# Algomorph/LevelSetFusion-Python

Hardware: AMD Instinct MI355X
Metric: voxel-warp-updates/sec (higher is better)
Workload: dtype f32

## Files before the change

include/lsf_hip.h:

```cpp
#ifndef LSF_HIP_H
#define LSF_HIP_H

#include <stdint.h>

#ifdef __cplusplus
extern "C" {
#endif

#define LSF_ABI_VERSION 4
#define LSF_MAX_KERNEL_TAPS 31

#define LSF_ERR_BAD_ARGUMENT (-1)
#define LSF_ERR_BAD_DIMS (-2)
#define LSF_ERR_KERNEL_TOO_LONG (-3)
#define LSF_ERR_RCCL_UNAVAILABLE (-4)
#define LSF_ERR_RCCL_FAILED (-5)
#define LSF_ERR_NOT_RESIDENT (-6)

typedef struct lsf_grid {
    int32_t dims;
    int32_t nz, ny, nx;
    int32_t z_begin, z_end;
    int32_t z_global_offset;
    int32_t y_global_offset;
// ... 146 lines not shown
int lsf_state_prepare(const float *live, const float *canonical, float *state_a, float *state_b,
                      const lsf_grid *grid, int32_t *scratch, int64_t *counts_out, void *stream);
int lsf_state_pack(const float *live, const float *warp_planar, float *state_a, float *state_b,
                   const lsf_grid *grid, void *stream);
int lsf_state_unpack(const float *state, float *live_out, float *warp_planar_out, float *warp_interleaved_out,
                     const lsf_grid *grid, void *stream);
int64_t lsf_state_finalize_scratch_elements(const lsf_grid *grid);
int lsf_state_finalize(const float *state, const float *canonical, float *live_out, float *warp_planar_out,
                       float *warp_interleaved_out, const lsf_grid *grid, float lower_threshold,
                       double *statistics16, double *scratch, void *stream);
int lsf_planar_finalize(const float *live, const float *warp_planar, const float *canonical, float *live_out,
                        float *warp_interleaved_out, const lsf_grid *grid, float lower_threshold,
                        double *statistics16, double *scratch, void *stream);

int lsf_state_finalize_listed(const float *state, const float *canonical, float *live_out, float *warp_interleaved_out,
                              const lsf_grid *grid, const int32_t *const *band_lists, const int64_t *band_counts,
                              int32_t n_lists, int64_t opposite_count, int64_t first_opposite, float lower_threshold,
                              double *statistics16, double *scratch, const int32_t *skip_flag,
                              const lsf_iteration_record *guard_records, int32_t guard_count, float guard_limit,
                              void *stream);
int lsf_slavcheva_state_iteration(const float *state_in, const float *canonical, float *state_out,
                                  const lsf_grid *grid, const lsf_slavcheva_params *params, const lsf_gate *gate,
                                  lsf_iteration_record *record, const int32_t *band_list, int64_t band_count,
                                  int32_t band_subset, void *stream);

int lsf_cumulative_warp_compose(const float *state, const float *psi_in, float *psi_out, const lsf_grid *grid,
                                const lsf_gate *gate, const int32_t *band_list, int64_t band_count, void *stream);

typedef struct lsf_band_box {
    int32_t origin;
    int32_t reserved;
    uint64_t mask;
} lsf_band_box;
int64_t lsf_band_boxes_scratch_elements(const lsf_grid *grid);
int lsf_band_boxes_count(const lsf_grid *grid, int32_t subset, const int32_t *prepare_scratch, int32_t *box_scratch,
                         int64_t *count_out, void *stream);
int lsf_band_boxes_fill(const lsf_grid *grid, int32_t subset, const int32_t *prepare_scratch, const int32_t *box_scratch,
                        lsf_band_box *boxes, void *stream);
int lsf_band_boxes_canonical(const float *canonical, const lsf_grid *grid, const lsf_band_box *boxes, int64_t box_count,
                             float *canonical_boxed, void *stream);
int lsf_slavcheva_state_iteration_boxes(const float *state_in, const float *canonical_boxed, float *state_out,
                                        const lsf_grid *grid, const lsf_slavcheva_params *params, const lsf_gate *gate,
                                        lsf_iteration_record *record, const lsf_band_box *boxes, int64_t box_count,
                                        void *stream);

typedef struct lsf_run_loop {
    int32_t min_iterations;
    int32_t max_iterations;
    float lower_threshold, upper_threshold;
    int32_t check_interval;
    int32_t reserved;
} lsf_run_loop;
typedef struct lsf_state_run {
    const float *live;
    const float *canonical;
    float *state[2];
    int32_t *prepare_scratch;
    int64_t *totals_device;
    int64_t *totals_host;
    lsf_grid grid;
    int32_t sparse_reach;
    int32_t second_state_late;
    int32_t *box_scratch;
    int32_t box_all;
    int32_t reserved;
} lsf_state_run;
typedef struct lsf_state_run_result {
    float *max_value;
    int64_t *argmax;
    double *energies3;
    uint8_t *executed;
    int32_t final_state;
    int32_t n_lists;
    int32_t reach_exceeded;
    int32_t compact_faces;
} lsf_state_run_result;
int lsf_state_run_begin(const lsf_state_run *run, void *stream);
int lsf_state_run_finish(const lsf_state_run *run, const lsf_slavcheva_params *params, int32_t *list_interior,
                         int32_t *list_boundary, lsf_band_box *boxes, float *box_canonical, lsf_iteration_record *records,
                         int32_t iterations, const lsf_run_loop *loop ,
                         float *live_out,
                         float lower_threshold, double *statistics16, double *finalize_scratch, int64_t *words_device,
                         int64_t *words_host, lsf_state_run_result *result, void *stream);

int lsf_sobolev_run_finish(const lsf_state_run *run, const lsf_slavcheva_params *params, const double *taps_host,
                           int32_t n_taps, int32_t *list_interior, int32_t *list_boundary, int32_t *list_all,
                           lsf_band_box *boxes, float *g4_a, float *g4_b, lsf_iteration_record *records, int32_t iterations,
                           const lsf_run_loop *loop, float *live_out, float lower_threshold, double *statistics16,
                           double *finalize_scratch, int64_t *words_device, int64_t *words_host,
                           lsf_state_run_result *result, void *stream);

int lsf_sobolev_state_gradient(const float *state, const float *canonical, float *g_raw4, const lsf_grid *grid,
                               const lsf_slavcheva_params *params, const lsf_gate *gate, lsf_iteration_record *record,
                               const int32_t *band_list, int64_t band_count, void *stream);
int lsf_sobolev_state_gradient_x(const float *state, const float *canonical, float *out4, const lsf_grid *grid,
                                 const lsf_slavcheva_params *params, const double *taps_host, int32_t n_taps,
                                 const lsf_gate *gate, lsf_iteration_record *record, const int32_t *band_list,
                                 int64_t band_count, int32_t out_bricks, void *stream);
int lsf_zero_listed4(float *field4, const lsf_grid *grid, const int32_t *band_list, int64_t band_count, int32_t bricks,
                     void *stream);
int lsf_convolve_axis_listed4(const float *in4, float *out4, const float *zero_mask_source4, const lsf_grid *grid,
                              int32_t axis, const double *taps_host, int32_t n_taps, const lsf_gate *gate,
                              const int32_t *band_list, int64_t band_count, void *stream);
int lsf_band_list_strip_major(const int32_t *band_list, int64_t band_count, const lsf_grid *grid, int32_t strips,
                              int32_t *out, int32_t *scratch, void *stream);
int lsf_sobolev_state_update(const float *in4, const float *zero_mask_source4, const float *state_in, float *state_out,
                             float *g_out4, const lsf_grid *grid, const lsf_slavcheva_params *params, int32_t axis,
                             const double *taps_host, int32_t n_taps, const lsf_gate *gate,
                             lsf_iteration_record *record, const int32_t *band_list, int64_t band_count,
                             int32_t first_list, void *stream);
int lsf_sobolev_state_update_boxes(const float *in4, const float *state_in, float *state_out, float *g_out4,
                                   const lsf_grid *grid, const lsf_slavcheva_params *params, const double *taps_host,
                                   int32_t n_taps, const lsf_gate *gate, lsf_iteration_record *record,
                                   const lsf_band_box *boxes, int64_t box_count, void *stream);

#define LSF_SLAB_LAUNCH 0
#define LSF_SLAB_EXCHANGE 1
#define LSF_SLAB_EXCHANGE_DEFERRED 2
#define LSF_SLAB_RESUME 3
typedef struct lsf_slab_comm lsf_slab_comm;
typedef struct lsf_slab_layout {
    int32_t nz, ny, nx;
    int32_t z_begin, z_end;
    int32_t halo;
    int32_t lo_rank, hi_rank;
} lsf_slab_layout;
typedef struct lsf_slab_part {
    lsf_grid grid;
    const int32_t *band_list[2];
    int64_t band_count[2];
    int32_t band_subset[2];
    int32_t n_lists;
    int32_t reserved;
} lsf_slab_part;
typedef struct lsf_slab_faces {
    const int32_t *send_list[2], *recv_list[2];
    float *send_msg[2], *recv_msg[2];
    int64_t send_count[2], recv_count[2];
} lsf_slab_faces;
int lsf_merge_sorted_runs(const int32_t *const *a, const int64_t *n_a, const int32_t *const *b, const int64_t *n_b,
                          int32_t *const *out, int32_t pairs, void *stream);
int lsf_slab_unique_id(const char *rccl_library_path, uint8_t *id_out128);
int lsf_slab_comm_create(const char *rccl_library_path, const uint8_t *id128, int32_t rank, int32_t world,
                         lsf_slab_comm **out);
int lsf_slab_comm_destroy(lsf_slab_comm *comm);
int lsf_slab_comm_info(lsf_slab_comm *comm, int32_t *rank_out, int32_t *nranks_out);
int lsf_slab_face_counts_begin(lsf_slab_comm *comm, const int64_t *counts4);
int lsf_slab_face_counts_end(lsf_slab_comm *comm, int64_t *table);
int lsf_slab_state_iteration(lsf_slab_comm *comm, const float *state_in, const float *canonical, float *state_out,
                             const lsf_slab_layout *layout, const lsf_slab_part *boundary_parts, int32_t n_boundary,
                             const lsf_slab_part *interior_parts, int32_t n_interior,
                             const lsf_slavcheva_params *params, const lsf_gate *gate, lsf_iteration_record *record,
                             int32_t exchange ,
                             const lsf_slab_faces *faces , void *stream);

#define LSF_SLAB_MAX_CUTS 72
typedef struct lsf_slab_run {
    lsf_state_run base;
    lsf_slab_layout layout;
    int32_t exchange_interval;
    int32_t n_cuts;
    int32_t cut_slices[LSF_SLAB_MAX_CUTS];
    int64_t cut_entries[2][LSF_SLAB_MAX_CUTS];
    int64_t out_index_entries;
    int64_t out_face_entries;
} lsf_slab_run;
// ... 483 lines not shown
```

levelsetfusion-python_amd/_lib.py:

```python
import ctypes
import os

import torch

from ._build import LIB_PATH

c_float_p = ctypes.c_void_p

MAX_KERNEL_TAPS = 31
ABI_VERSION = 4
HEADER_ABI_HASH = "88f9a6300475259d"

ERRORS = {-1: "LSF_ERR_BAD_ARGUMENT", -2: "LSF_ERR_BAD_DIMS", -3: "LSF_ERR_KERNEL_TOO_LONG",
          -4: "LSF_ERR_RCCL_UNAVAILABLE", -5: "LSF_ERR_RCCL_FAILED", -6: "LSF_ERR_NOT_RESIDENT"}

SMOOTHING_TIKHONOV, SMOOTHING_KILLING = 0, 1
DATA_BASIC, DATA_THRESHOLDED_FDM = 0, 2
ENERGY_NONE, ENERGY_DIRECT, ENERGY_VECTORIZED = 0, 1, 2
GATE_HIERARCHICAL, GATE_SLAVCHEVA, GATE_OPEN = 0, 1, 2


class Grid(ctypes.Structure):
    _fields_ = [("dims", ctypes.c_int32), ("nz", ctypes.c_int32), ("ny", ctypes.c_int32), ("nx", ctypes.c_int32),
                ("z_begin", ctypes.c_int32), ("z_end", ctypes.c_int32), ("z_global_offset", ctypes.c_int32),
                ("y_global_offset", ctypes.c_int32), ("energy_z_begin", ctypes.c_int32), ("energy_z_end", ctypes.c_int32),
                ("ny_global", ctypes.c_int32), ("energy_y_begin", ctypes.c_int32), ("energy_y_end", ctypes.c_int32)]


BAND_ALL, BAND_INTERIOR, BAND_BOUNDARY = 0, 1, 2
RECORD_SLOTS = 8


class RecordSlot(ctypes.Structure):
    _fields_ = [("max_packed", ctypes.c_uint64), ("data_energy", ctypes.c_double),
                ("smoothing_energy", ctypes.c_double), ("level_set_energy", ctypes.c_double),
                ("pad", ctypes.c_uint64 * 508)]


class IterationRecord(ctypes.Structure):
    _fields_ = [("slot", RecordSlot * RECORD_SLOTS)]


RECORD_BYTES = ctypes.sizeof(IterationRecord)
SLOT_WORDS = ctypes.sizeof(RecordSlot) // 8


class Gate(ctypes.Structure):
    _fields_ = [("prev_record", ctypes.c_void_p), ("mode", ctypes.c_int32), ("a", ctypes.c_float),
                ("b", ctypes.c_float)]


SLAB_LAUNCH, SLAB_EXCHANGE, SLAB_EXCHANGE_DEFERRED, SLAB_RESUME = 0, 1, 2, 3


class SlabLayoutC(ctypes.Structure):
    _fields_ = [("nz", ctypes.c_int32), ("ny", ctypes.c_int32), ("nx", ctypes.c_int32), ("z_begin", ctypes.c_int32),
                ("z_end", ctypes.c_int32), ("halo", ctypes.c_int32), ("lo_rank", ctypes.c_int32),
                ("hi_rank", ctypes.c_int32)]


class SlabPart(ctypes.Structure):
    _fields_ = [("grid", Grid), ("band_list", ctypes.c_void_p * 2), ("band_count", ctypes.c_int64 * 2),
                ("band_subset", ctypes.c_int32 * 2), ("n_lists", ctypes.c_int32), ("reserved", ctypes.c_int32)]


class SlabFaces(ctypes.Structure):
    _fields_ = [("send_list", ctypes.c_void_p * 2), ("recv_list", ctypes.c_void_p * 2),
                ("send_msg", ctypes.c_void_p * 2), ("recv_msg", ctypes.c_void_p * 2),
                ("send_count", ctypes.c_int64 * 2), ("recv_count", ctypes.c_int64 * 2)]


class BandBox(ctypes.Structure):
    _fields_ = [("origin", ctypes.c_int32), ("reserved", ctypes.c_int32), ("mask", ctypes.c_uint64)]


class StateRun(ctypes.Structure):
    _fields_ = [("live", ctypes.c_void_p), ("canonical", ctypes.c_void_p), ("state", ctypes.c_void_p * 2),
                ("prepare_scratch", ctypes.c_void_p), ("totals_device", ctypes.c_void_p),
                ("totals_host", ctypes.c_void_p), ("grid", Grid), ("sparse_reach", ctypes.c_int32),
                ("second_state_late", ctypes.c_int32), ("box_scratch", ctypes.c_void_p), ("box_all", ctypes.c_int32),
                ("reserved", ctypes.c_int32)]


TERM_DATA_BASIC, TERM_DATA_THRESHOLDED_FDM, TERM_TIKHONOV, TERM_TIKHONOV_LOCAL, TERM_KILLING, TERM_LEVEL_SET = range(6)
TERM_COPY_IF_ZERO, TERM_IGNORE_IF_ZERO, TERM_INTERLEAVED = 1, 2, 4
SELECT_ALL, SELECT_BAND, SELECT_LIST = 0, 1, 2
TERM_ENERGY_LOCAL, TERM_ENERGY_NP_GRADIENT = 0, 1


class TermParams(ctypes.Structure):
    _fields_ = [("isomorphic_enforcement_factor_f64", ctypes.c_double), ("isomorphic_enforcement_factor", ctypes.c_float),
                ("epsilon", ctypes.c_float), ("scaling_factor", ctypes.c_float), ("term", ctypes.c_int32),
                ("flags", ctypes.c_int32), ("reserved", ctypes.c_int32)]

# ... 218 lines not shown

class PointSdfParams(ctypes.Structure):
    _fields_ = [(n, ctypes.c_double) for n in ("fx", "fy", "cx", "cy", "depth_unit_ratio", "max_distance", "voxel_size",
                                               "offset_x", "offset_y", "offset_z", "narrow_band_width_voxels",
                                               "scale")] + \
               [(n, ctypes.c_int32) for n in ("depth", "height", "width", "image_height", "image_width", "depth_dtype",
                                              "levels")] + \
               [("iterations", ctypes.c_int32 * ICP_MAX_LEVELS), ("strides", ctypes.c_int32 * ICP_MAX_LEVELS),
                ("loss", ctypes.c_int32)]


POINT_SDF_COLOUR_SCRATCH_BYTES = 2 * ICP_MAX_BLOCKS * 35 * 8
_POINT_SDF_COLOUR_FIELDS = [(n, ctypes.c_double) for n in ("photometric_weight", "max_intensity_difference",
                                                           "intensity_scale")]


class PointSdfPhotometricParams(ctypes.Structure):
    _fields_ = PointSdfParams._fields_ + _POINT_SDF_COLOUR_FIELDS


class PointSdfPyramidParams(ctypes.Structure):
    _fields_ = PointSdfPhotometricParams._fields_ + [("pyramid_levels", ctypes.c_int32), ("reserved", ctypes.c_int32)]


class EwaParams(ctypes.Structure):
    _fields_ = [("covariance_camera_space", ctypes.c_double * 9), ("squared_radius_threshold", ctypes.c_double),
                ("intrinsic_matrix", ctypes.c_float * 9), ("method", ctypes.c_int32)]


_P = ctypes.POINTER
_vp, _i32, _i64, _f32 = ctypes.c_void_p, ctypes.c_int32, ctypes.c_int64, ctypes.c_float

PROTOTYPES = {
    "lsf_abi_version": (ctypes.c_int, []),
    "lsf_target_arch": (ctypes.c_char_p, []),
    "lsf_build_id": (ctypes.c_char_p, []),
    "lsf_abi_hash": (ctypes.c_char_p, []),
    "lsf_deinterleave": (ctypes.c_int, [_vp, _vp, _i64, _i32, _vp]),
    "lsf_interleave": (ctypes.c_int, [_vp, _vp, _i64, _i32, _vp]),
    "lsf_halo_copy": (ctypes.c_int, [_vp, _vp, _vp, _vp, _P(Grid), _i32, _i32, _i32, _i32, _i32, _vp]),
    "lsf_warp_field": (ctypes.c_int, [_vp, _vp, _vp, _P(Grid), _f32, _vp]),
    "lsf_warp_field_advanced": (ctypes.c_int, [_vp, _vp, _vp, _vp, _vp, _P(Grid), _i32, _vp]),
    "lsf_pack_live_gradient": (ctypes.c_int, [_vp, _vp, _P(Grid), _vp]),
    "lsf_restrict_mean": (ctypes.c_int, [_vp, _vp, _P(Grid), _i32, _vp]),
    "lsf_prolong_repeat": (ctypes.c_int, [_vp, _vp, _P(Grid), _vp]),
    "lsf_upsample2x_linear": (ctypes.c_int, [_vp, _vp, _P(Grid), _i32, _vp]),
    "lsf_downsample2x_linear": (ctypes.c_int, [_vp, _vp, _P(Grid), _i32, _vp]),
    "lsf_convolve_axis": (ctypes.c_int, [_vp, _vp, _vp, _P(Grid), _i32, _i32, _P(ctypes.c_double), _i32,
                                         _P(Gate), _vp]),
    "lsf_convolve_xy": (ctypes.c_int, [_vp, _vp, _P(Grid), _i32, _P(ctypes.c_double), _i32, _P(Gate), _vp]),
    "lsf_convolve_axis_update": (ctypes.c_int, [_vp, _vp, _vp, ctypes.c_float, _P(Grid), _i32, _i32, _P(ctypes.c_double),
                                                _i32, _P(Gate), _vp]),
    "lsf_convolve_xyz": (ctypes.c_int, [_vp, _vp, _vp, _f32, _P(Grid), _i32, _P(ctypes.c_double), _i32, _P(Gate),
                                        _vp]),
    "lsf_hier_iteration": (ctypes.c_int, [_vp, _vp, _vp, _vp, _vp, _P(Grid), _P(HierParams), _P(Gate), _vp, _vp]),
    "lsf_hier_update": (ctypes.c_int, [_vp, _vp, _P(Grid), _f32, _P(Gate), _vp, _vp]),
    "lsf_hier_level_run_2d": (ctypes.c_int, [_vp, _vp, _vp, _vp, _vp, _vp, _P(Grid), _P(HierParams), _P(ctypes.c_double),
                                            _i32, _vp, _i32, _i32, ctypes.c_float, _vp]),
    "lsf_slavcheva_gradient": (ctypes.c_int, [_vp, _vp, _vp, _vp, _P(Grid), _P(SlavchevaParams), _P(Gate), _vp,
                                              _vp, _i64, _vp]),
    "lsf_convolve_axis_listed": (ctypes.c_int, [_vp, _vp, _vp, _P(Grid), _i32, _i32, _P(ctypes.c_double), _i32,
                                                _P(Gate), _vp, _i64, _vp]),
    "lsf_state_prepare_scratch_elements": (ctypes.c_int64, [_P(Grid)]),
    "lsf_band_list_fill_prepared": (ctypes.c_int, [_P(Grid), _i32, _vp, _vp, _vp]),
    "lsf_state_prepare": (ctypes.c_int, [_vp, _vp, _vp, _vp, _P(Grid), _vp, _vp, _vp]),
    "lsf_state_pack": (ctypes.c_int, [_vp, _vp, _vp, _vp, _P(Grid), _vp]),
    "lsf_state_pack_needed": (ctypes.c_int, [_vp, _vp, _vp, _P(Grid), _vp, _i32, _i32, _vp]),
    "lsf_state_unpack": (ctypes.c_int, [_vp, _vp, _vp, _vp, _P(Grid), _vp]),
    "lsf_state_finalize_scratch_elements": (ctypes.c_int64, [_P(Grid)]),
    "lsf_state_finalize": (ctypes.c_int, [_vp, _vp, _vp, _vp, _vp, _P(Grid), _f32, _vp, _vp, _vp]),
    "lsf_planar_finalize": (ctypes.c_int, [_vp, _vp, _vp, _vp, _vp, _P(Grid), _f32, _vp, _vp, _vp]),
    "lsf_state_finalize_listed": (ctypes.c_int, [_vp, _vp, _vp, _vp, _P(Grid), _P(ctypes.c_void_p), _P(_i64), _i32,
                                                 _i64, _i64, _f32, _vp, _vp, _vp, _vp, _i32, _f32, _vp]),
    "lsf_slavcheva_state_iteration": (ctypes.c_int, [_vp, _vp, _vp, _P(Grid), _P(SlavchevaParams), _P(Gate), _vp,
                                                     _vp, _i64, _i32, _vp]),
    "lsf_cumulative_warp_compose": (ctypes.c_int, [_vp, _vp, _vp, _P(Grid), _P(Gate), _vp, _i64, _vp]),
    "lsf_band_boxes_scratch_elements": (ctypes.c_int64, [_P(Grid)]),
    "lsf_band_boxes_count": (ctypes.c_int, [_P(Grid), ctypes.c_int32, _vp, _vp, _vp, _vp]),
    "lsf_band_boxes_fill": (ctypes.c_int, [_P(Grid), ctypes.c_int32, _vp, _vp, _vp, _vp]),
    "lsf_band_boxes_canonical": (ctypes.c_int, [_vp, _P(Grid), _vp, ctypes.c_int64, _vp, _vp]),
    "lsf_slavcheva_state_iteration_boxes": (ctypes.c_int, [_vp, _vp, _vp, _P(Grid), _P(SlavchevaParams), _P(Gate), _vp, _vp,
                                                           _i64, _vp]),
    "lsf_state_run_begin": (ctypes.c_int, [_P(StateRun), _vp]),
    "lsf_state_run_finish": (ctypes.c_int, [_P(StateRun), _P(SlavchevaParams), _vp, _vp, _vp, _vp, _vp, _i32, _P(RunLoop), _vp,
                                            _f32, _vp, _vp, _vp, _vp, _P(StateRunResult), _vp]),
    "lsf_sobolev_run_finish": (ctypes.c_int, [_P(StateRun), _P(SlavchevaParams), _P(ctypes.c_double), _i32, _vp, _vp, _vp, _vp,
                                              _vp, _vp, _vp, _i32, _P(RunLoop), _vp, _f32, _vp, _vp, _vp, _vp,
                                              _P(StateRunResult), _vp]),
    "lsf_slab_run_begin": (ctypes.c_int, [_P(SlabRun), _vp]),
    "lsf_slab_run_finish": (ctypes.c_int, [_P(SlabRun), _vp, _P(SlavchevaParams), _vp, _vp, _vp, _vp, _vp, _i32, _vp, _vp, _vp,
                                           _P(StateRunResult), _vp]),
    "lsf_band_scratch_elements": (ctypes.c_int64, [_P(Grid)]),
    "lsf_band_count": (ctypes.c_int, [_vp, _vp, _P(Grid), _i32, _vp, _vp, _vp]),
    "lsf_band_list_fill": (ctypes.c_int, [_vp, _vp, _P(Grid), _i32, _vp, _vp, _vp]),
    "lsf_records_decode": (ctypes.c_int, [_vp, _i32, _i32, _i32, _vp, _vp, _vp, _vp]),
    "lsf_merge_sorted_runs": (ctypes.c_int, [_P(_vp), _P(_i64), _P(_vp), _P(_i64), _P(_vp), _i32, _vp]),
    "lsf_slab_unique_id": (ctypes.c_int, [ctypes.c_char_p, _vp]),
    "lsf_slab_comm_create": (ctypes.c_int, [ctypes.c_char_p, _vp, _i32, _i32, _P(_vp)]),
    "lsf_slab_comm_destroy": (ctypes.c_int, [_vp]),
    "lsf_slab_comm_info": (ctypes.c_int, [_vp, _P(_i32), _P(_i32)]),
    "lsf_slab_face_counts_begin": (ctypes.c_int, [_vp, _P(_i64)]),
    "lsf_slab_face_counts_end": (ctypes.c_int, [_vp, _P(_i64)]),
    "lsf_slab_state_iteration": (ctypes.c_int, [_vp, _vp, _vp, _vp, _P(SlabLayoutC), _P(SlabPart), _i32, _P(SlabPart),
                                                _i32, _P(SlavchevaParams), _P(Gate), _vp, _i32, _P(SlabFaces), _vp]),
    "lsf_slavcheva_filter_update_rewarp": (ctypes.c_int, [_vp, _vp, _vp, _vp, _vp, _vp, _P(Grid), _P(SlavchevaParams),
                                                          _i32, _P(ctypes.c_double), _i32, _P(Gate), _vp, _vp, _i64,
                                                          _vp]),
    "lsf_sobolev_state_gradient": (ctypes.c_int, [_vp, _vp, _vp, _P(Grid), _P(SlavchevaParams), _P(Gate), _vp, _vp, _i64,
                                                  _vp]),
    "lsf_band_list_strip_major": (ctypes.c_int, [_vp, _i64, _P(Grid), _i32, _vp, _vp, _vp]),
    "lsf_sobolev_state_gradient_x": (ctypes.c_int, [_vp, _vp, _vp, _P(Grid), _P(SlavchevaParams), _P(ctypes.c_double), _i32,
                                                    _P(Gate), _vp, _vp, _i64, _i32, _vp]),
    "lsf_zero_listed4": (ctypes.c_int, [_vp, _P(Grid), _vp, _i64, _i32, _vp]),
    "lsf_convolve_axis_listed4": (ctypes.c_int, [_vp, _vp, _vp, _P(Grid), _i32, _P(ctypes.c_double), _i32, _P(Gate), _vp,
                                                 _i64, _vp]),
    "lsf_sobolev_state_update": (ctypes.c_int, [_vp, _vp, _vp, _vp, _vp, _P(Grid), _P(SlavchevaParams), _i32,
                                                _P(ctypes.c_double), _i32, _P(Gate), _vp, _vp, _i64, _i32, _vp]),
    "lsf_sobolev_state_update_boxes": (ctypes.c_int, [_vp, _vp, _vp, _vp, _P(Grid), _P(SlavchevaParams),
                                                      _P(ctypes.c_double), _i32, _P(Gate), _vp, _vp, _i64, _vp]),
    "lsf_slavcheva_update_rewarp": (ctypes.c_int, [_vp, _vp, _vp, _vp, _vp, _P(Grid), _P(SlavchevaParams),
                                                   _P(Gate), _vp, _vp, _i64, _vp]),
    "lsf_term_gradient": (ctypes.c_int, [_vp, _vp, _vp, _vp, _vp, _vp, _vp, _vp, _vp, _P(Grid), _P(TermParams), _i32, _i32,
                                         _vp, _i64, _vp]),
    "lsf_warp_statistics": (ctypes.c_int, [_vp, _vp, _vp, _P(Grid), _f32, _vp, _vp]),
    "lsf_tsdf_difference_statistics": (ctypes.c_int, [_vp, _vp, _P(Grid), _vp, _vp]),
    "lsf_tsdf_generate_nearest": (ctypes.c_int, [_vp, _vp, _P(Grid), _P(TsdfParams), _vp]),
    "lsf_tsdf_generate_bilinear": (ctypes.c_int, [_vp, _vp, _P(Grid), _P(TsdfParams), _i32, _vp]),
    "lsf_tsdf_generate_ewa": (ctypes.c_int, [_vp, _vp, _P(Grid), _P(TsdfParams), _P(EwaParams), _vp]),
    "lsf_tsdf_generate_nearest_typed": (ctypes.c_int, [_vp, _i32, _vp, _P(Grid), _P(TsdfParams), _P(ctypes.c_double),
                                                       _P(ctypes.c_double), _vp]),
    "lsf_rigid_gradient": (ctypes.c_int, [_vp, _vp, _P(RigidParams), _vp]),
    "lsf_rigid_run": (ctypes.c_int, [_vp, _vp, _vp, _vp, _vp, _P(RigidParams), _vp]),
    "lsf_rigid3d_gradient": (ctypes.c_int, [_vp, _vp, _vp, _vp, _P(Rigid3dParams), _vp]),
    "lsf_rigid3d_run": (ctypes.c_int, [_vp, _vp, _vp, _vp, _vp, _P(Rigid3dParams), _vp]),
    "lsf_fusion_integrate_volume": (ctypes.c_int, [_vp, _vp, _vp, _vp, _vp, _P(FusionParams), _vp]),
    "lsf_fusion_integrate_depth": (ctypes.c_int, [_vp, _vp, _vp, _vp, _vp, _P(FusionParams), _vp]),
    "lsf_fusion_integrate_depth_weighted": (ctypes.c_int, [_vp, _vp, _vp, _vp, _vp, _vp, _P(FusionWeightedParams),
                                                           _vp]),
    "lsf_fusion_integrate_depth_colour": (ctypes.c_int, [_vp, _vp, _vp, _vp, _vp, _vp, _vp, _vp,
                                                         _P(FusionColourParams), _vp]),
    "lsf_fusion_integrate_depth_warped": (ctypes.c_int, [_vp, _vp, _vp, _vp, _vp, _vp, _vp, _vp, _vp,
                                                         _P(FusionWarpedParams), _vp]),
    "lsf_depth_confidence": (ctypes.c_int, [_vp, _vp, _vp, _P(DepthConfidenceParams), _vp]),
    "lsf_raycast": (ctypes.c_int, [_vp, _vp, _vp, _vp, _vp, _vp, _P(RaycastParams), _vp]),
    "lsf_raycast_colour": (ctypes.c_int, [_vp, _vp, _vp, _vp, _vp, _vp, _vp, _vp, _P(RaycastParams), _vp]),
    "lsf_mesh_count": (ctypes.c_int, [_vp, _vp, _vp, _vp, _vp, _vp, _P(MeshParams), _vp]),
    "lsf_mesh_emit": (ctypes.c_int, [_vp, _vp, _vp, _vp, _vp, _vp, _vp, _vp, _vp, _i64, _i64, _P(MeshParams), _vp]),
    "lsf_mesh_vertex_colours": (ctypes.c_int, [_vp, _vp, _vp, _vp, _vp, _i64, ctypes.c_int32, ctypes.c_int32,
                                               ctypes.c_int32, _P(MeshParams), _vp]),
    "lsf_volume_shift": (ctypes.c_int, [_vp, _vp, _vp, _vp, _vp, _vp, _P(VolumeShiftParams), _vp]),
    "lsf_icp_run": (ctypes.c_int, [_vp, _vp, _vp, _vp, _vp, _vp, _vp, _P(IcpParams), _vp]),
    "lsf_depth_pyramid": (ctypes.c_int, [_vp, _vp, _vp, _P(DepthPyramidParams), _vp]),
    "lsf_icp_run_pyramid": (ctypes.c_int, [_vp, _vp, _vp, _vp, _vp, _vp, _vp, _vp, _P(IcpPyramidParams), _vp]),
    "lsf_icp_run_photometric": (ctypes.c_int, [_vp, _vp, _vp, _vp, _vp, _vp, _vp, _vp, _vp, _vp,
                                               _P(IcpPhotometricParams), _vp]),
    "lsf_intensity_pyramid": (ctypes.c_int, [_vp, _vp, _P(IntensityPyramidParams), _vp]),
    "lsf_icp_run_pyramid_photometric": (ctypes.c_int, [_vp, _vp, _vp, _vp, _vp, _vp, _vp, _vp, _vp, _vp, _vp,
                                                       _P(IcpPyramidPhotometricParams), _vp]),
    "lsf_icp_run_robust": (ctypes.c_int, [_vp, _vp, _vp, _vp, _vp, _vp, _vp, _vp, _vp, _vp, _vp, _P(IcpRobustParams),
                                          _vp]),
    "lsf_icp_run_pyramid_robust": (ctypes.c_int, [_vp, _vp, _vp, _vp, _vp, _vp, _vp, _vp, _vp, _vp, _vp, _vp,
                                                  _P(IcpPyramidRobustParams), _vp]),
    "lsf_point_sdf_run": (ctypes.c_int, [_vp, _vp, _vp, _vp, _vp, _vp, _vp, _vp, _P(PointSdfParams), _vp]),
    "lsf_point_sdf_run_photometric": (ctypes.c_int, [_vp] * 11 + [_P(PointSdfPhotometricParams), _vp]),
    "lsf_point_sdf_run_pyramid": (ctypes.c_int, [_vp] * 11 + [_P(PointSdfPyramidParams), _vp]),
}
# ... 40 lines not shown
```

levelsetfusion-python_amd/csrc/lsf_device.h:

```cpp
#pragma once

#include <hip/hip_runtime.h>
#include <cstdlib>
#include <stdint.h>

#include "../../include/lsf_hip.h"

namespace lsf {

constexpr int kWave = 64;
constexpr int kBlock = 256;
constexpr int kCuBlock = 1024;
constexpr int kMaxBlockWaves = kCuBlock / kWave;

struct FastDiv {
    unsigned d, m, l;
};

__host__ inline FastDiv make_fast_div(unsigned d) {
    FastDiv f;
    f.d = d;
    f.l = 0;
    while ((1ull << f.l) < d) ++f.l;
    f.m = (unsigned)(((1ull << 32) * ((1ull << f.l) - d)) / d + 1ull);
// ... 203 lines not shown
        return x_begin + (g * cus + q) * group + (n - g * group);
    }
};

__device__ inline WaveWalk wave_list_walk(unsigned count, unsigned group) {
    const unsigned units = (count + kWave - 1) / kWave;
    const unsigned nb = gridDim.x, bid = blockIdx.x;
    WaveWalk w;
    w.group = group;
    if (nb % kXcds == 0) {
        const unsigned per_xcd = (units + kXcds - 1) / kXcds, xcd = bid % kXcds;
        w.cus = nb / kXcds;
        w.q = bid / kXcds;
        w.x_begin = xcd * per_xcd;
        w.x_end = w.x_begin + per_xcd < units ? w.x_begin + per_xcd : units;
    } else {
        w.cus = nb;
        w.q = bid;
        w.x_begin = 0u;
        w.x_end = units;
    }
    return w;
}

__host__ inline unsigned cu_list_blocks(unsigned count, unsigned cus) {
    const unsigned units = (count + kWave - 1) / kWave;
    unsigned blocks = (units + kMaxBlockWaves - 1) / kMaxBlockWaves;
    if (blocks < 1) blocks = 1;
    if (blocks > cus) blocks = cus;
    if (blocks > kXcds) blocks -= blocks % kXcds;
    return blocks;
}

template <class F>
__device__ inline void for_each_listed_voxel(const Grid& g, const int* __restrict__ list, unsigned count, F&& f) {
    const bool listed = list != nullptr;
    const Tiling t = make_tiling(g);
    const TileWalk w = tile_walk(t.total, g);
    const int lx = threadIdx.x & (kTileX - 1), ly = threadIdx.x / kTileX;
    unsigned first = w.q, step = w.step, end = w.count;
    if (listed) {
        const unsigned units = (count + kBlock - 1) / kBlock;
        const unsigned nb = gridDim.x, bid = blockIdx.x;
        if (nb % kXcds == 0) {
            const unsigned per_xcd = (units + kXcds - 1) / kXcds, xcd = bid % kXcds;
            first = xcd * per_xcd + bid / kXcds;
            step = nb / kXcds;
            end = (xcd + 1) * per_xcd < units ? (xcd + 1) * per_xcd : units;
        } else {
            first = bid; step = nb; end = units;
        }
    }
    for (unsigned u = first; u < end; u += step) {
        int x, y, z;
        bool inside;
        if (listed) {
            const unsigned k = u * kBlock + threadIdx.x;
            inside = k < count;
            const unsigned i = inside ? (unsigned)list[k] : 0u;
            const unsigned zy = fast_div(i, g.div_nx);
            x = (int)(i - zy * (unsigned)g.nx);
            z = (int)fast_div(zy, g.div_ny);
            y = (int)zy - z * g.ny;
        } else {
            const unsigned tile = tile_of(w, u);
            const unsigned rest = fast_div(tile, g.div_tiles_x);
            const int tx = (int)(tile - rest * (unsigned)t.tiles_x);
            const int tz = (int)fast_div(rest, g.div_tiles_y);
            const int ty = (int)rest - tz * t.tiles_y;
            x = tx * kTileX + lx; y = ty * g.tile_y + ly; z = g.z_begin + tz;
            inside = x < g.nx && y < g.ny;
        }
        if (inside) f(x, y, z);
    }
}

__host__ inline unsigned band_list_blocks(unsigned count, unsigned default_per_xcd = 256u) {
    const unsigned units = (count + kBlock - 1) / kBlock;
    if (units <= kXcds) return units < 1 ? 1 : units;
    const unsigned per_xcd = (units + kXcds - 1) / kXcds;
    const unsigned cap = default_per_xcd;
    const unsigned rounds = (per_xcd + cap - 1) / cap;
    return kXcds * ((per_xcd + rounds - 1) / rounds);
}


__device__ inline void decode_voxel(const Grid& g, unsigned i, int& x, int& y, int& z) {
    if (g.shift_x >= 0) {
        x = (int)(i & ((1u << g.shift_x) - 1u));
        const unsigned zy = i >> g.shift_x;
        y = (int)(zy & ((1u << g.shift_y) - 1u));
        z = (int)(zy >> g.shift_y);
    } else {
        const unsigned zy = fast_div(i, g.div_nx);
        x = (int)(i - zy * (unsigned)g.nx);
        z = (int)fast_div(zy, g.div_ny);
        y = (int)zy - z * g.ny;
    }
}

__device__ inline unsigned linear_index(const Grid& g, int x, int y, int z) {
    return (unsigned)(((long long)(z + g.z_global_offset) * g.ny_global + (y + g.y_global_offset)) * g.nx + x);
}

__device__ inline int vidx(const Grid& g, int x, int y, int z) {
    return (z * g.ny + y) * g.nx + x;
}

__device__ inline bool inside(const Grid& g, int x, int y, int z) {
    return (unsigned)x < (unsigned)g.nx && (unsigned)y < (unsigned)g.ny && (unsigned)z < (unsigned)g.nz;
}

__device__ inline float read_oob(const float* __restrict__ f, const Grid& g, int x, int y, int z, float oob) {
    return inside(g, x, y, z) ? f[vidx(g, x, y, z)] : oob;
}

__device__ inline float read_clamp(const float* __restrict__ f, const Grid& g, int x, int y, int z) {
    x = min(max(x, 0), g.nx - 1);
    y = min(max(y, 0), g.ny - 1);
    z = min(max(z, 0), g.nz - 1);
    return f[vidx(g, x, y, z)];
}

struct AxisTaps {
    int c0, c1;
    bool v0, v1;
    float r, i;
};

__device__ inline AxisTaps axis_taps(float p, int n, int global_offset) {
    AxisTaps t;
    const float f = floorf(p);
    t.r = p - f;
    t.i = 1.0f - t.r;
    const int b = (int)fminf(fmaxf(f - (float)global_offset, -2.0f), (float)n + 1.0f);
    t.v0 = (unsigned)b < (unsigned)n;
    t.v1 = (unsigned)(b + 1) < (unsigned)n;
    t.c0 = min(max(b, 0), n - 1);
    t.c1 = min(max(b + 1, 0), n - 1);
    return t;
}

template <int D>
__device__ inline float sample_linear_taps(const float* __restrict__ f, const Grid& g, const AxisTaps& ax,
                                           const AxisTaps& ay, const AxisTaps& az, float oob) {
    const int row0 = ay.c0 * g.nx, row1 = ay.c1 * g.nx;
    if (D == 2) {
        float v00 = f[row0 + ax.c0], v01 = f[row1 + ax.c0], v10 = f[row0 + ax.c1], v11 = f[row1 + ax.c1];
        v00 = (ax.v0 && ay.v0) ? v00 : oob;
        v01 = (ax.v0 && ay.v1) ? v01 : oob;
        v10 = (ax.v1 && ay.v0) ? v10 : oob;
        v11 = (ax.v1 && ay.v1) ? v11 : oob;
        const float i0 = v00 * ay.i + v01 * ay.r;
        const float i1 = v10 * ay.i + v11 * ay.r;
        return i0 * ax.i + i1 * ax.r;
    } else {
        const int slice = g.nx * g.ny;
        const int s0 = az.c0 * slice, s1 = az.c1 * slice;
        float c[2][2];
#pragma unroll
        for (int ox = 0; ox < 2; ++ox)
#pragma unroll
            for (int oy = 0; oy < 2; ++oy) {
                const int xy = (oy ? row1 : row0) + (ox ? ax.c1 : ax.c0);
                const bool vxy = (ox ? ax.v1 : ax.v0) && (oy ? ay.v1 : ay.v0);
                float a = f[s0 + xy], b = f[s1 + xy];
// ... 26 lines not shown
__device__ inline double shfl_down_f64(double v, int delta) {
    return __longlong_as_double((long long)shfl_down_u64((unsigned long long)__double_as_longlong(v), delta));
}

template <int CTRL>
__device__ inline unsigned long long dpp_u64(unsigned long long v) {
    const unsigned lo = (unsigned)__builtin_amdgcn_update_dpp(0, (int)(unsigned)v, CTRL, 0xf, 0xf, false);
    const unsigned hi = (unsigned)__builtin_amdgcn_update_dpp(0, (int)(unsigned)(v >> 32), CTRL, 0xf, 0xf, false);
    return ((unsigned long long)hi << 32) | lo;
}

__device__ inline unsigned long long broadcast_lane63_u64(unsigned long long v) {
    const unsigned lo = (unsigned)__builtin_amdgcn_readlane((int)(unsigned)v, 63);
    const unsigned hi = (unsigned)__builtin_amdgcn_readlane((int)(unsigned)(v >> 32), 63);
    return ((unsigned long long)hi << 32) | lo;
}

__device__ inline unsigned long long wave_max_u64(unsigned long long v) {
#define LSF_STEP(CTRL)                                   \
    {                                                    \
        const unsigned long long o = dpp_u64<CTRL>(v);   \
        v = o > v ? o : v;                               \
    }
    LSF_STEP(0xb1)
    LSF_STEP(0x4e)
    LSF_STEP(0x124)
    LSF_STEP(0x128)
    LSF_STEP(0x142)
    LSF_STEP(0x143)
#undef LSF_STEP
    return broadcast_lane63_u64(v);
}

__device__ inline double wave_sum_f64(double v) {
#define LSF_STEP(CTRL)                                                                                               \
    v += __longlong_as_double((long long)dpp_u64<CTRL>((unsigned long long)__double_as_longlong(v)));
    LSF_STEP(0xb1)
    LSF_STEP(0x4e)
    LSF_STEP(0x124)
    LSF_STEP(0x128)
    LSF_STEP(0x142)
    LSF_STEP(0x143)
#undef LSF_STEP
    return __longlong_as_double((long long)broadcast_lane63_u64((unsigned long long)__double_as_longlong(v)));
}

__device__ inline unsigned long long pack_max(float length, unsigned linear_index) {
    return ((unsigned long long)__float_as_uint(length) << 32) | (unsigned long long)(~linear_index);
}

__device__ inline float unpack_max_value(unsigned long long packed) { return __uint_as_float((unsigned)(packed >> 32)); }

template <int NS>
__device__ inline void block_reduce_commit(unsigned long long packed, const double (&sums)[NS > 0 ? NS : 1],
                                           unsigned long long* dst_max, double* const (&dst_sum)[NS > 0 ? NS : 1]) {
    __shared__ unsigned long long s_max[kMaxBlockWaves];
    __shared__ double s_sum[(NS > 0 ? NS : 1)][kMaxBlockWaves];
    const int lane = threadIdx.x & (kWave - 1), wave = threadIdx.x / kWave;
    const int n_waves = blockDim.x / kWave;
    unsigned long long m = wave_max_u64(packed);
    double s[NS > 0 ? NS : 1];
#pragma unroll
    for (int i = 0; i < NS; ++i) s[i] = wave_sum_f64(sums[i]);
    if (lane == 0) {
        s_max[wave] = m;
#pragma unroll
        for (int i = 0; i < NS; ++i) s_sum[i][wave] = s[i];
    }
    __syncthreads();
    if (wave == 0) {
        const unsigned long long mm = wave_max_u64(lane < n_waves ? s_max[lane] : 0ull);
        double t[NS > 0 ? NS : 1];
#pragma unroll
        for (int i = 0; i < NS; ++i) t[i] = wave_sum_f64(lane < n_waves ? s_sum[i][lane] : 0.0);
        if (lane == 0) {
            if (dst_max && mm != 0ull) atomicMax(dst_max, mm);
#pragma unroll
            for (int i = 0; i < NS; ++i)
                if (dst_sum[i] && t[i] != 0.0) atomicAdd(dst_sum[i], t[i]);
        }
    }
}

template <int NT>
struct TapsN {
    double k[NT];
};

template <bool FMA>
__device__ inline double mac(double acc, double k, double v) {
    return FMA ? __builtin_fma(k, v, acc) : acc + k * v;
}

static inline bool taps_are_float32(const double* taps, int n) {
    for (int j = 0; j < n; ++j)
        if (!((double)(float)taps[j] == taps[j])) return false;
    return true;
}

template <int D>
__device__ inline float vec_length(const float (&v)[3]) {
    float s = v[0] * v[0] + v[1] * v[1];
    if (D == 3) s = s + v[2] * v[2];
    return sqrtf(s);
}

__device__ inline float second_difference_f64(float am, float a0, float ap) {
    return (float)__builtin_fma(-2.0, (double)a0, (double)ap + (double)am);
}

__device__ inline bool gate_closed(const lsf_gate& gate) {
    if (!gate.prev_record || gate.mode == LSF_GATE_OPEN) return false;
    unsigned long long p = 0ull;
#pragma unroll
    for (int k = 0; k < LSF_RECORD_SLOTS; ++k) {
        const unsigned long long q = gate.prev_record->slot[k].max_packed;
        p = q > p ? q : p;
    }
    if (p == 0ull) return true;
    float m = unpack_max_value(p);
    if (gate.mode == LSF_GATE_HIERARCHICAL) return m < gate.a;
    return !(gate.a < m && m < gate.b);
}

__device__ inline lsf_record_slot* record_slot(lsf_iteration_record* r) {
    return &r->slot[blockIdx.x % LSF_RECORD_SLOTS];
}

__device__ inline unsigned long long* record_max(lsf_iteration_record* r) {
    return reinterpret_cast<unsigned long long*>(&record_slot(r)->max_packed);
}

__host__ inline lsf_gate gate_or_open(const lsf_gate* gate) {
    return gate ? *gate : lsf_gate{nullptr, 0, 0.0f, 0.0f};
}

inline bool overlaps(const void* a, size_t na, const void* b, size_t nb) {
    if (!a || !b || !na || !nb) return false;
    const uintptr_t x = (uintptr_t)a, y = (uintptr_t)b;
    return x < y + nb && y < x + na;
}

inline hipStream_t as_stream(void* s) { return reinterpret_cast<hipStream_t>(s); }

inline int launch_status() { return (int)hipGetLastError(); }

}
```

levelsetfusion-python_amd/csrc/lsf_slavcheva.hip:

```cpp
#include "lsf_device.h"

using namespace lsf;

#include "lsf_slavcheva_terms.h"

using namespace lsf::slav;

namespace {


template <int D, int SMOOTH, bool LEVELSET, int DATA, int ENERGY>
__device__ inline void voxel_gradient(const float* __restrict__ live, const float* __restrict__ canonical,
                                      const float* __restrict__ warp_prev, const Grid& g, const Params& p, int x,
                                      int y, int z, int i, float (&gv)[3], double (&en)[3]) {
    gv[0] = gv[1] = gv[2] = 0.0f;
    const float l = live[i], cn = canonical[i];
    if (fabsf(l) == 1.0f && fabsf(cn) == 1.0f) return;
    const bool interior = x > 0 && x < g.nx - 1 && y > 0 && y < g.ny - 1 && (D == 2 || (z > 0 && z < g.nz - 1));
    if (g.fast_ok && __all(interior)) {
        const NbhFast<D> n(live, warp_prev, g, x, y, z);
        band_voxel_gradient<D, SMOOTH, LEVELSET, DATA, ENERGY>(n, p, l, cn, gv, en);
    } else {
        const Nbh<D> n(live, warp_prev, g, x, y, z);
        band_voxel_gradient<D, SMOOTH, LEVELSET, DATA, ENERGY>(n, p, l, cn, gv, en);
// ... 300 lines not shown
    if (blockIdx.x >= arrays) {
        reduce_opposite(opposite, n, totals);
        return;
    }
    __shared__ int wave_total[1024 / kWave];
    int* __restrict__ sums = sums_base + (size_t)blockIdx.x * stride;
    const unsigned t = threadIdx.x, lane = t & (kWave - 1), wave = t / kWave;
    int carry = 0;
    for (unsigned base = 0; base < n; base += 4096u) {
        const unsigned i = base + 4u * t;
        int v[4];
#pragma unroll
        for (int k = 0; k < 4; ++k) v[k] = i + k < n ? sums[i + k] : 0;
        const int mine = v[0] + v[1] + v[2] + v[3];
        int inclusive = mine;
#pragma unroll
        for (int d = 1; d < kWave; d <<= 1) {
            const int up = __shfl_up(inclusive, d, kWave);
            if ((int)lane >= d) inclusive += up;
        }
        if (lane == kWave - 1) wave_total[wave] = inclusive;
        __syncthreads();
        int before = 0, tile = 0;
#pragma unroll
        for (int w = 0; w < 1024 / kWave; ++w) {
            const int x = wave_total[w];
            before += w < (int)wave ? x : 0;
            tile += x;
        }
        int run = carry + before + inclusive - mine;
#pragma unroll
        for (int k = 0; k < 4; ++k) {
            if (i + k < n) sums[i + k] = run;
            run += v[k];
        }
        carry += tile;
        __syncthreads();
    }
    if (t == 0) totals[blockIdx.x] = carry;
}

constexpr unsigned kScanTile = 4096u;

__global__ __launch_bounds__(1024) void band_tile_totals_kernel(const int* __restrict__ sums_base, unsigned n,
                                                                unsigned stride, const int* __restrict__ opposite,
                                                                int* __restrict__ tile_out, unsigned tiles) {
    __shared__ int s_sum[1024 / kWave], s_first[1024 / kWave];
    const unsigned tile = blockIdx.x, a = blockIdx.y, t = threadIdx.x;
    const unsigned i = tile * kScanTile + 4u * t;
    int sum = 0, first = 0x7fffffff;
    if (a < 2u) {
        const int* __restrict__ sums = sums_base + (size_t)a * stride;
#pragma unroll
        for (unsigned k = 0; k < 4u; ++k) sum += i + k < n ? sums[i + k] : 0;
    } else {
#pragma unroll
        for (unsigned k = 0; k < 4u; ++k)
            if (i + k < n) {
                sum += opposite[2 * (i + k)];
                first = min(first, opposite[2 * (i + k) + 1]);
            }
    }
    for (int d = kWave / 2; d > 0; d >>= 1) {
        sum += __shfl_down(sum, d, kWave);
        first = min(first, __shfl_down(first, d, kWave));
    }
    if ((t & (kWave - 1)) == 0) {
        s_sum[t / kWave] = sum;
        s_first[t / kWave] = first;
    }
    __syncthreads();
    if (t == 0) {
        for (int k = 1; k < 1024 / kWave; ++k) {
            sum += s_sum[k];
            first = min(first, s_first[k]);
        }
        tile_out[(size_t)a * tiles + tile] = sum;
        if (a == 2u) tile_out[(size_t)3 * tiles + tile] = first;
    }
}

__global__ __launch_bounds__(1024) void band_scan_tiles_kernel(int* __restrict__ sums_base, unsigned n, unsigned stride,
                                                               const int* __restrict__ tile_out, unsigned tiles,
                                                               long long* __restrict__ totals) {
    const unsigned tile = blockIdx.x, a = blockIdx.y, t = threadIdx.x, lane = t & (kWave - 1), wave = t / kWave;
    if (a == 2u) {
        if (tile == 0u && t == 0u) {
            long long sum = 0;
            int first = 0x7fffffff;
            for (unsigned k = 0; k < tiles; ++k) {
                sum += tile_out[(size_t)2 * tiles + k];
                first = min(first, tile_out[(size_t)3 * tiles + k]);
            }
            totals[2] = sum;
            totals[3] = first == 0x7fffffff ? -1 : first;
        }
        return;
    }
    __shared__ int wave_total[1024 / kWave];
    int* __restrict__ sums = sums_base + (size_t)a * stride;
    int carry = 0;
    for (unsigned k = 0; k < tile; ++k) carry += tile_out[(size_t)a * tiles + k];
    const unsigned i = tile * kScanTile + 4u * t;
    int v[4];
#pragma unroll
    for (int k = 0; k < 4; ++k) v[k] = i + k < n ? sums[i + k] : 0;
    const int mine = v[0] + v[1] + v[2] + v[3];
    int inclusive = mine;
#pragma unroll
    for (int d = 1; d < kWave; d <<= 1) {
        const int up = __shfl_up(inclusive, d, kWave);
        if ((int)lane >= d) inclusive += up;
    }
    if (lane == kWave - 1) wave_total[wave] = inclusive;
    __syncthreads();
    int before = 0, whole = 0;
#pragma unroll
    for (int w = 0; w < 1024 / kWave; ++w) {
        const int x = wave_total[w];
        before += w < (int)wave ? x : 0;
        whole += x;
    }
    int run = carry + before + inclusive - mine;
#pragma unroll
    for (int k = 0; k < 4; ++k) {
        if (i + k < n) sums[i + k] = run;
        run += v[k];
    }
    if (tile == tiles - 1u && t == 0u) totals[a] = (long long)carry + whole;
}

typedef float vf4 __attribute__((ext_vector_type(4)));

__global__ __launch_bounds__(kBlock) void state_prepare_kernel(const float* __restrict__ live,
                                                               const float* __restrict__ canonical,
                                                               vf4* __restrict__ a, vf4* __restrict__ b, unsigned n,
                                                               Grid g, int dims, int* __restrict__ sums_interior,
                                                               int* __restrict__ sums_boundary,
                                                               unsigned long long* __restrict__ masks,
                                                               int* __restrict__ opposite, int* __restrict__ nonempty) {
    __shared__ int part[4][16];
    const int t = threadIdx.x, wave = t / kWave, lane = t % kWave;
#pragma unroll
    for (int j = 0; j < 4; ++j) {
        const unsigned v = blockIdx.x * kBandChunk + j * kBlock + t;
        bool in_band = false, interior = false, opposed = false;
        if (v < n) {
            const float l = live[v], cn = canonical[v];
            in_band = !(fabsf(l) == 1.0f && fabsf(cn) == 1.0f);
            opposed = !in_band && l != cn;
            vf4 o;
            o.x = l; o.y = 0.0f; o.z = 0.0f; o.w = 0.0f;
            if (a) a[v] = o;
            if (b) b[v] = o;
            const unsigned zy = fast_div(v, g.div_nx);
            const int x = (int)(v - zy * (unsigned)g.nx);
            const int z = (int)fast_div(zy, g.div_ny);
            const int y = (int)zy - z * g.ny;
            interior = x > 0 && x < g.nx - 1 && y > 0 && y < g.ny - 1 && (dims == 2 || (z > 0 && z < g.nz - 1));
        }
        const unsigned long long mi = __ballot(in_band && interior), mb = __ballot(in_band && !interior);
        const unsigned long long mo = __ballot(opposed);
        if (lane == 0) {
            part[0][j * 4 + wave] = __popcll(mi);
            part[1][j * 4 + wave] = __popcll(mb);
            part[2][j * 4 + wave] = __popcll(mo);
            part[3][j * 4 + wave] = mo ? (int)(blockIdx.x * kBandChunk + j * kBlock + wave * kWave) + __ffsll((long long)mo) - 1
                                       : 0x7fffffff;
            masks[((size_t)blockIdx.x * 16 + j * 4 + wave) * 2 + 0] = mi;
            masks[((size_t)blockIdx.x * 16 + j * 4 + wave) * 2 + 1] = mb;
// ... 31 lines not shown
    return ((unsigned long long)hi << 32) | lo;
}

__global__ __launch_bounds__(kBlock) void state_prepare4_kernel(const vf4* __restrict__ live4,
                                                                const vf4* __restrict__ canonical4,
                                                                vf4* __restrict__ a, vf4* __restrict__ b, unsigned n,
                                                                unsigned chunks, Grid g, int dims,
                                                                int* __restrict__ sums_interior,
                                                                int* __restrict__ sums_boundary,
                                                                unsigned long long* __restrict__ masks,
                                                                int* __restrict__ opposite, int* __restrict__ nonempty) {
    __shared__ int part[kPrepareChunksPerBlock][4][16];
    const int t = threadIdx.x, wave = t / kWave, lane = t % kWave;
    const unsigned chunk0 = blockIdx.x * kPrepareChunksPerBlock;
    vf4 l[kPrepareChunksPerBlock], c[kPrepareChunksPerBlock];
#pragma unroll
    for (int k = 0; k < kPrepareChunksPerBlock; ++k) {
        const unsigned v = (chunk0 + k) * kBandChunk + 4u * t;
        const vf4 one = {1.0f, 1.0f, 1.0f, 1.0f};
        l[k] = v < n ? live4[v / 4] : one;
        c[k] = v < n ? canonical4[v / 4] : one;
    }
#pragma unroll
    for (int k = 0; k < kPrepareChunksPerBlock; ++k) {
        const unsigned chunk = chunk0 + k, v = chunk * kBandChunk + 4u * t;
        unsigned ni = 0u, nb = 0u, no = 0u;
        if (v < n) {
            const unsigned zy = fast_div(v, g.div_nx);
            const int x0 = (int)(v - zy * (unsigned)g.nx);
            const int z = (int)fast_div(zy, g.div_ny);
            const int y = (int)zy - z * g.ny;
            const bool row_inside = y > 0 && y < g.ny - 1 && (dims == 2 || (z > 0 && z < g.nz - 1));
            const float lv[4] = {l[k].x, l[k].y, l[k].z, l[k].w}, cv[4] = {c[k].x, c[k].y, c[k].z, c[k].w};
#pragma unroll
            for (int j = 0; j < 4; ++j) {
                const bool in_band = !(fabsf(lv[j]) == 1.0f && fabsf(cv[j]) == 1.0f);
                const bool interior = row_inside && x0 + j > 0 && x0 + j < g.nx - 1;
                ni |= (in_band && interior ? 1u : 0u) << j;
                nb |= (in_band && !interior ? 1u : 0u) << j;
                no |= (!in_band && lv[j] != cv[j] ? 1u : 0u) << j;
                vf4 o;
                o.x = lv[j]; o.y = 0.0f; o.z = 0.0f; o.w = 0.0f;
                if (a) a[v + j] = o;
                if (b) b[v + j] = o;
            }
        }
        const unsigned long long mi = row16_or(ni, lane), mb = row16_or(nb, lane), mo = row16_or(no, lane);
        if ((lane & 15) == 0 && chunk < chunks) {
            const int word = wave * 4 + lane / 16;
            part[k][0][word] = __popcll(mi);
            part[k][1][word] = __popcll(mb);
            part[k][2][word] = __popcll(mo);
            part[k][3][word] = mo ? (int)(chunk * kBandChunk + word * kWave) + __ffsll((long long)mo) - 1 : 0x7fffffff;
            masks[((size_t)chunk * 16 + word) * 2 + 0] = mi;
            masks[((size_t)chunk * 16 + word) * 2 + 1] = mb;
        }
    }
    __syncthreads();
    if (t < 4 * kPrepareChunksPerBlock) {
        const int k = t / 4, what = t % 4;
        const unsigned chunk = chunk0 + k;
        if (chunk < chunks) {
            if (what < 2) {
                int sum = 0;
                for (int w = 0; w < 16; ++w) sum += part[k][what][w];
                (what == 0 ? sums_interior : sums_boundary)[chunk] = sum;
            } else if (what == 2) {
                int sum = 0, first = 0x7fffffff;
                for (int w = 0; w < 16; ++w) {
                    sum += part[k][2][w];
                    first = min(first, part[k][3][w]);
                }
                opposite[2 * chunk] = sum;
                opposite[2 * chunk + 1] = first;
            } else {
                int any = 0;
                for (int w = 0; w < 16; ++w) any |= part[k][0][w] | part[k][1][w];
                nonempty[chunk] = any != 0;
            }
        }
    }
}

__global__ __launch_bounds__(kBlock) void chunk_needed_kernel(unsigned chunks, long long row, long long slice, int dims,
                                                              int reach, const int* __restrict__ nonempty,
                                                              int* __restrict__ needed) {
    const unsigned c = blockIdx.x * (kBlock / kWave) + threadIdx.x / kWave;
    if (c >= chunks) return;
    const int lane = threadIdx.x % kWave;
    const long long c0 = (long long)c * kBandChunk;
    const int span = 2 * reach + 1, zs = dims == 3 ? span : 1;
    bool hit = false;
    for (int k = lane; k < zs * span; k += kWave) {
        const int dy = k % span - reach, dz = dims == 3 ? k / span - reach : 0;
        const long long lo = c0 + dz * slice + dy * row - reach, hi = c0 + (long long)kBandChunk - 1 + dz * slice + dy * row + reach;
        long long first = lo >= 0 ? lo / kBandChunk : -((-lo + kBandChunk - 1) / kBandChunk);
        long long last = hi >= 0 ? hi / kBandChunk : -((-hi + kBandChunk - 1) / kBandChunk);
        first = first < 0 ? 0 : first;
        last = last >= (long long)chunks ? (long long)chunks - 1 : last;
        for (long long cand = first; cand <= last; ++cand) hit |= nonempty[cand] != 0;
    }
    const bool any = __any(hit);
    if (lane == 0) needed[c] = any ? 1 : 0;
}

constexpr int kPackChunks = 1;
__global__ __launch_bounds__(kBlock) void state_pack_needed_kernel(const float* __restrict__ live, vf4* __restrict__ a,
                                                                   vf4* __restrict__ b, unsigned n, unsigned chunks,
                                                                   const int* __restrict__ needed, int want) {
    const int t = threadIdx.x;
    int verdict[kPackChunks];
#pragma unroll
    for (int k = 0; k < kPackChunks; ++k) {
        const unsigned c = blockIdx.x * kPackChunks + k;
        verdict[k] = c < chunks ? needed[c] : -1;
    }
#pragma unroll
    for (int k = 0; k < kPackChunks; ++k) {
        if (verdict[k] != want) continue;
        const unsigned c = blockIdx.x * kPackChunks + k;
#pragma unroll
        for (int j = 0; j < 4; ++j) {
            const unsigned v = c * kBandChunk + j * kBlock + t;
            if (v < n) {
                vf4 o;
                o.x = live[v]; o.y = 0.0f; o.z = 0.0f; o.w = 0.0f;
                if (a) a[v] = o;
                if (b) b[v] = o;
            }
        }
    }
}



__global__ __launch_bounds__(kBlock) void band_fill_from_masks_kernel(const unsigned long long* __restrict__ masks,
                                                                      const int* __restrict__ block_sums, int which,
                                                                      int* __restrict__ list, unsigned chunks) {
    const int lane = threadIdx.x % kWave;
    const unsigned chunk = blockIdx.x * (kBlock / kWave) + threadIdx.x / kWave;
    if (chunk >= chunks) return;
    const unsigned long long mine = lane < 16 ? masks[((size_t)chunk * 16 + lane) * 2 + which] : 0ull;
    if (__ballot(mine != 0ull) == 0ull) return;
    int at = block_sums[chunk];
#pragma unroll
    for (int w = 0; w < 16; ++w) {
        const unsigned lo = (unsigned)__shfl((int)(unsigned)mine, w, kWave);
        const unsigned hi = (unsigned)__shfl((int)(unsigned)(mine >> 32), w, kWave);
        const unsigned long long m = ((unsigned long long)hi << 32) | lo;
        if ((m >> lane) & 1ull)
            list[at + __popcll(m & ((1ull << lane) - 1ull))] = (int)(chunk * kBandChunk + w * kWave + lane);
        at += __popcll(m);
    }
}

}

static inline bool band_subset_ok(int32_t subset) {
    return subset == LSF_BAND_ALL || subset == LSF_BAND_INTERIOR || subset == LSF_BAND_BOUNDARY;
}

extern "C" int lsf_slavcheva_gradient(const float* live, const float* canonical, const float* warp_prev_planar,
                                      float* g_out_planar, const lsf_grid* grid, const lsf_slavcheva_params* params,
                                      const lsf_gate* gate, lsf_iteration_record* record, const int32_t* band_list,
                                      int64_t band_count, void* stream) {
    if (int e = check_grid(grid)) return e;
    if (!live || !canonical || !warp_prev_planar || !params || !record || !g_out_planar ||
        g_out_planar == warp_prev_planar || (band_list && (band_count < 0 || band_count > 0x7fffffffll)))
        return LSF_ERR_BAD_ARGUMENT;
    Grid g = make_grid(grid);
    Tiling t = make_tiling(g);
    if (t.total == 0) return 0;
    LaunchArgs a{band_list ? band_list_blocks((unsigned)band_count) : launch_blocks(t.total), as_stream(stream), live,
                 canonical, warp_prev_planar, g_out_planar, g, make_params(params), gate_or_open(gate), record, band_list,
                 (unsigned)band_count};
    if (grid->dims == 2) pick_terms<2>(params, a);
    else pick_terms<3>(params, a);
    return launch_status();
}

extern "C" int lsf_slavcheva_update_rewarp(const float* live, const float* canonical, float* g_planar,
                                           float* warp_out_planar, float* live_out, const lsf_grid* grid,
                                           const lsf_slavcheva_params* params, const lsf_gate* gate,
                                           lsf_iteration_record* record, const int32_t* band_list, int64_t band_count,
                                           void* stream) {
    (void)canonical;
    if (int e = check_grid(grid)) return e;
    if (!live || !g_planar || !warp_out_planar || !live_out || live_out == live || !params || !record ||
        (band_list && (band_count < 0 || band_count > 0x7fffffffll)))
        return LSF_ERR_BAD_ARGUMENT;
    Grid g = make_grid(grid);
    Tiling t = make_tiling(g);
    if (t.total == 0) return 0;
    Params p = make_params(params);
    lsf_gate gt = gate_or_open(gate);
    const unsigned blocks = band_list ? band_list_blocks((unsigned)band_count) : launch_blocks(t.total);
    if (grid->dims == 2)
        hipLaunchKernelGGL(slavcheva_update_rewarp_kernel<2>, dim3(blocks), dim3(kBlock), 0, as_stream(stream), live,
// ... 137 lines not shown
        }
    return m;
}

template <bool FILL>
__global__ __launch_bounds__(kBlock) void band_boxes_kernel(const unsigned long long* __restrict__ masks, unsigned n_boxes,
                                                            int nbx, int nby, int nx, int ny, bool all,
                                                            int* __restrict__ group_sums, lsf_band_box* __restrict__ boxes) {
    __shared__ int wave_count[kBlock / kWave];
    const unsigned box = blockIdx.x * kBoxGroup + threadIdx.x;
    const int lane = threadIdx.x % kWave, wave = threadIdx.x / kWave;
    const unsigned long long m = box < n_boxes ? box_mask_of(masks, box, nbx, nby, nx, ny, all) : 0ull;
    const unsigned long long any = __ballot(m != 0ull);
    if (lane == 0) wave_count[wave] = __popcll(any);
    __syncthreads();
    if (!FILL) {
        if (threadIdx.x == 0) {
            int sum = 0;
            for (int k = 0; k < kBlock / kWave; ++k) sum += wave_count[k];
            group_sums[blockIdx.x] = sum;
        }
        return;
    }
    if (m == 0ull) return;
    int at = group_sums[blockIdx.x];
    for (int k = 0; k < wave; ++k) at += wave_count[k];
    at += __popcll(any & ((1ull << lane) - 1ull));
    const int bx = (int)(box % (unsigned)nbx), by = (int)((box / (unsigned)nbx) % (unsigned)nby);
    const int bz = (int)(box / ((unsigned)nbx * (unsigned)nby));
    lsf_band_box b;
    b.origin = ((4 * bz) * ny + 4 * by) * nx + 4 * bx;
    b.reserved = 0;
    b.mask = m;
    boxes[at] = b;
}

inline bool boxes_ok(const lsf_grid* g) {
    return g->dims == 3 && g->nx % 4 == 0 && g->ny % 4 == 0 && g->nz % 4 == 0 && g->z_begin == 0 && g->z_end == g->nz &&
           (long long)g->nx * g->ny * g->nz <= 0x0fffffffll;
}
}

extern "C" int64_t lsf_band_boxes_scratch_elements(const lsf_grid* grid) {
    if (check_grid(grid) || !boxes_ok(grid)) return 0;
    const long long n_boxes = (long long)grid->nx * grid->ny * grid->nz / 64;
    return (n_boxes + kBoxGroup - 1) / kBoxGroup + 1;
}

extern "C" int lsf_band_boxes_count(const lsf_grid* grid, int32_t subset, const int32_t* prepare_scratch,
                                    int32_t* box_scratch, int64_t* count_out, void* stream) {
    if (int e = check_grid(grid)) return e;
    if (!boxes_ok(grid)) return LSF_ERR_BAD_DIMS;
    if (!prepare_scratch || !box_scratch || !count_out || (subset != LSF_BAND_INTERIOR && subset != LSF_BAND_ALL))
        return LSF_ERR_BAD_ARGUMENT;
    unsigned first, n, chunks;
    band_range(grid, first, n, chunks);
    const unsigned n_boxes = n / 64, groups = (n_boxes + kBoxGroup - 1) / kBoxGroup;
    hipStream_t s = as_stream(stream);
    hipLaunchKernelGGL(band_boxes_kernel<false>, dim3(groups), dim3(kBlock), 0, s,
                       prepare_masks(const_cast<int32_t*>(prepare_scratch), chunks), n_boxes, grid->nx / 4, grid->ny / 4,
                       grid->nx, grid->ny, subset == LSF_BAND_ALL, box_scratch, (lsf_band_box*)nullptr);
    hipLaunchKernelGGL(band_scan_kernel, dim3(1), dim3(1024), 0, s, box_scratch, groups, 0u, 1u, (long long*)count_out,
                       (const int*)nullptr);
    return launch_status();
}

extern "C" int lsf_band_boxes_fill(const lsf_grid* grid, int32_t subset, const int32_t* prepare_scratch,
                                   const int32_t* box_scratch, lsf_band_box* boxes, void* stream) {
    if (int e = check_grid(grid)) return e;
    if (!boxes_ok(grid)) return LSF_ERR_BAD_DIMS;
    if (!prepare_scratch || !box_scratch || !boxes || (subset != LSF_BAND_INTERIOR && subset != LSF_BAND_ALL))
        return LSF_ERR_BAD_ARGUMENT;
    unsigned first, n, chunks;
    band_range(grid, first, n, chunks);
    const unsigned n_boxes = n / 64, groups = (n_boxes + kBoxGroup - 1) / kBoxGroup;
    hipLaunchKernelGGL(band_boxes_kernel<true>, dim3(groups), dim3(kBlock), 0, as_stream(stream),
                       prepare_masks(const_cast<int32_t*>(prepare_scratch), chunks), n_boxes, grid->nx / 4, grid->ny / 4,
                       grid->nx, grid->ny, subset == LSF_BAND_ALL, const_cast<int32_t*>(box_scratch), boxes);
    return launch_status();
}

extern "C" int lsf_state_prepare(const float* live, const float* canonical, float* state_a, float* state_b,
                                 const lsf_grid* grid, int32_t* scratch, int64_t* counts_out, void* stream) {
    if (int e = check_grid(grid, true)) return e;
    if (!live || !canonical || (!state_a && state_b) || !scratch || !counts_out) return LSF_ERR_BAD_ARGUMENT;
    if (grid->z_begin != 0 || grid->z_end != grid->nz) return LSF_ERR_BAD_ARGUMENT;
    unsigned first, n, chunks;
    band_range(grid, first, n, chunks);
    hipStream_t s = as_stream(stream);
    int* sums_interior = scratch;
    int* sums_boundary = scratch + (chunks + 1);
    const bool wide = grid->nx % 4 == 0 && ((uintptr_t)live | (uintptr_t)canonical) % 16 == 0;
    if (wide)
        hipLaunchKernelGGL(state_prepare4_kernel, dim3((chunks + kPrepareChunksPerBlock - 1) / kPrepareChunksPerBlock),
                           dim3(kBlock), 0, s, reinterpret_cast<const vf4*>(live), reinterpret_cast<const vf4*>(canonical),
                           reinterpret_cast<vf4*>(state_a), reinterpret_cast<vf4*>(state_b), n, chunks, make_grid(grid),
                           grid->dims, sums_interior, sums_boundary, prepare_masks(scratch, chunks),
                           prepare_opposite(scratch, chunks), prepare_nonempty(scratch, chunks));
    else
        hipLaunchKernelGGL(state_prepare_kernel, dim3(chunks), dim3(kBlock), 0, s, live, canonical,
                           reinterpret_cast<vf4*>(state_a), reinterpret_cast<vf4*>(state_b), n, make_grid(grid), grid->dims,
                           sums_interior, sums_boundary, prepare_masks(scratch, chunks), prepare_opposite(scratch, chunks),
                           prepare_nonempty(scratch, chunks));
    const unsigned tiles = prepare_scan_tiles(chunks) > 0u ? prepare_scan_tiles(chunks) : 1u;
    hipLaunchKernelGGL(band_tile_totals_kernel, dim3(tiles, 3), dim3(1024), 0, s, scratch, chunks, chunks + 1,
                       (const int*)prepare_opposite(scratch, chunks), prepare_tile_totals(scratch, chunks), tiles);
    hipLaunchKernelGGL(band_scan_tiles_kernel, dim3(tiles, 3), dim3(1024), 0, s, scratch, chunks, chunks + 1,
                       (const int*)prepare_tile_totals(scratch, chunks), tiles, (long long*)counts_out);
    return launch_status();
}

extern "C" int lsf_state_pack_needed(const float* live, float* state_a, float* state_b, const lsf_grid* grid,
                                     int32_t* scratch, int32_t reach, int32_t invert, void* stream) {
    if (int e = check_grid(grid, true)) return e;
    if (!live || (!state_a && !state_b) || !scratch || reach < 1 || reach > 8) return LSF_ERR_BAD_ARGUMENT;
    if (grid->z_begin != 0 || grid->z_end != grid->nz) return LSF_ERR_BAD_ARGUMENT;
    unsigned first, n, chunks;
    band_range(grid, first, n, chunks);
    if (!invert)
        hipLaunchKernelGGL(chunk_needed_kernel, dim3((chunks + kBlock / kWave - 1) / (kBlock / kWave)), dim3(kBlock), 0, as_stream(stream),
                           chunks, (long long)grid->nx, (long long)grid->nx * grid->ny, grid->dims, reach,
                           prepare_nonempty(scratch, chunks), prepare_needed(scratch, chunks));
    hipLaunchKernelGGL(state_pack_needed_kernel, dim3((chunks + kPackChunks - 1) / kPackChunks), dim3(kBlock), 0,
                       as_stream(stream), live, reinterpret_cast<vf4*>(state_a), reinterpret_cast<vf4*>(state_b), n, chunks,
                       prepare_needed(scratch, chunks), invert ? 0 : 1);
    return launch_status();
}

extern "C" int lsf_band_list_fill(const float* live, const float* canonical, const lsf_grid* grid, int32_t subset,
                                  const int32_t* scratch, int32_t* list, void* stream) {
    if (int e = check_grid(grid)) return e;
    if (!live || !canonical || !scratch || !list || !band_subset_ok(subset)) return LSF_ERR_BAD_ARGUMENT;
    unsigned first, n, chunks;
    if (!band_range(grid, first, n, chunks)) return 0;
    hipLaunchKernelGGL(band_list_kernel<true>, dim3(chunks), dim3(kBlock), 0, as_stream(stream), live, canonical, first, n,
                       make_grid(grid), grid->dims, subset, const_cast<int32_t*>(scratch), list);
    return launch_status();
}
```

levelsetfusion-python_amd/csrc/lsf_slavcheva_box.hip:

```cpp
#include "lsf_slavcheva_state_taps.h"

using namespace lsf;
using namespace lsf::slav;

namespace {

constexpr int kBoxEdge = 4, kShellEdge = kBoxEdge + 2, kShell = kShellEdge * kShellEdge * kShellEdge;
constexpr int kShellLoads = (kShell + kWave - 1) / kWave;
#ifndef LSF_BOX_WAVES
#define LSF_BOX_WAVES 12
#endif
constexpr int kBoxWaves = LSF_BOX_WAVES, kBoxThreads = kBoxWaves * kWave;
constexpr int kImage = kShellLoads * kWave + kWave / 4;

struct NbhStateLds : TapsBase<3> {
    __device__ inline void load(const vf4* __restrict__ image, int centre) {
#pragma unroll
        for (int dz = -1; dz <= 1; ++dz)
#pragma unroll
            for (int dy = -1; dy <= 1; ++dy)
#pragma unroll
                for (int dx = -1; dx <= 1; ++dx) {
                    if ((dx != 0) + (dy != 0) + (dz != 0) > 2) continue;
                    this->t[dz + 1][dy + 1][dx + 1] = image[centre + (dz * kShellEdge + dy) * kShellEdge + dx];
                }
    }
};

__device__ inline bool rewarp_from_image(const TapsBase<3>& n, const vf4* __restrict__ image, int centre, const Grid& g,
                                         int x, int y, int z, const float (&wv)[3], bool active, Rewarp& rw) {
    const NearFar ax((float)x, wv[0]), ay((float)(y + g.y_global_offset), wv[1]), az((float)(z + g.z_global_offset), wv[2]);
    const unsigned lowest = min(min((unsigned)x, (unsigned)y), (unsigned)z);
    if (!__all(!active || (ax.near && ay.near && az.near && lowest >= 2u))) return false;
    const int ci = centre + (ax.below ? -1 : 1) + (ay.below ? -kShellEdge : kShellEdge) +
                   (az.below ? -kShellEdge * kShellEdge : kShellEdge * kShellEdge);
    rw.corner = image[ci].x;
    auto L = [&](int dz, int dy, int dx) { return n.t[dz + 1][dy + 1][dx + 1].x; };
    auto pick2 = [&](bool b, float m, float p) { return b ? m : p; };
    const float t000 = L(0, 0, 0);
    const float t100 = pick2(az.below, L(-1, 0, 0), L(1, 0, 0));
    const float t010 = pick2(ay.below, L(0, -1, 0), L(0, 1, 0));
    const float t001 = pick2(ax.below, L(0, 0, -1), L(0, 0, 1));
    const float t110 = pick2(az.below, pick2(ay.below, L(-1, -1, 0), L(-1, 1, 0)), pick2(ay.below, L(1, -1, 0), L(1, 1, 0)));
    const float t101 = pick2(az.below, pick2(ax.below, L(-1, 0, -1), L(-1, 0, 1)), pick2(ax.below, L(1, 0, -1), L(1, 0, 1)));
    const float t011 = pick2(ay.below, pick2(ax.below, L(0, -1, -1), L(0, -1, 1)), pick2(ax.below, L(0, 1, -1), L(0, 1, 1)));
    const float c00 = t000 * az.wn + t100 * az.wf;
    const float c10 = t010 * az.wn + t110 * az.wf;
    const float c01 = t001 * az.wn + t101 * az.wf;
    const float iy0 = c00 * ay.wn + c10 * ay.wf;
    rw.P = t011 * az.wn;
    rw.Q = c01 * ay.wn;
    rw.R = iy0 * ax.wn;
    rw.wfz = az.wf;
    rw.wfy = ay.wf;
    rw.wfx = ax.wf;
    rw.lerp = true;
    return true;
}

template <int SMOOTH, bool LEVELSET, int DATA, int ENERGY>
__global__ __launch_bounds__(kBoxThreads) __attribute__((amdgpu_waves_per_eu(kBoxWaves / 4, kBoxWaves / 4)))
void slavcheva_state_box_kernel(const vf4* __restrict__ state_in, const float* __restrict__ canonical_boxed,
                                vf4* __restrict__ state_out, Grid g, Params p, lsf_gate gate, lsf_iteration_record* record,
                                const lsf_band_box* __restrict__ boxes, unsigned box_count) {
    g.y_global_offset = 0;
    g.ny_global = g.ny;
    g.y_cut = 0;
    if (gate_closed(gate)) return;
    extern __shared__ vf4 lds[];
    __shared__ unsigned s_next_unit;
    __shared__ int s_goff[kWave][kShellLoads];
    const unsigned waves = blockDim.x / kWave, wave = threadIdx.x / kWave, lane = threadIdx.x & (kWave - 1);
    vf4* const images = lds + wave * (2 * kImage);
    const int sy = g.nx, sz = g.nx * g.ny;
    const int last_voxel = g.nz * sz - 1;
    if (wave == 0) {
#pragma unroll
        for (int j = 0; j < kShellLoads; ++j) {
            int k = (int)lane + kWave * j;
            k = k < kShell ? k : kShell - 1;
            s_goff[lane][j] = (k / (kShellEdge * kShellEdge)) * sz + ((k / kShellEdge) % kShellEdge) * sy + k % kShellEdge;
        }
    }
    const int lx = lane & 3, ly = (lane >> 2) & 3, lz = lane >> 4;
    const int centre = ((lz + 1) * kShellEdge + ly + 1) * kShellEdge + lx + 1;
    const int voxel_off = lz * sz + ly * sy + lx;

    unsigned long long best = 0ull;
    double en[3] = {0.0, 0.0, 0.0};
    const WaveWalk w = wave_list_walk(box_count * kWave, g.list_group);
    if (threadIdx.x == 0) s_next_unit = 2u * waves;
    __syncthreads();
    auto grab = [&]() {
        unsigned v = 0u;
        if (lane == 0) v = atomicAdd(&s_next_unit, 1u);
        return w.unit((unsigned)__builtin_amdgcn_readfirstlane((int)v));
    };
    auto header = [&](unsigned unit, bool& listed) {
        listed = unit < w.x_end && unit < box_count;
        return boxes[unit < box_count ? unit : box_count - 1u];
    };
    auto stage = [&](int origin, unsigned unit, vf4* image) {
        __builtin_amdgcn_global_load_lds((const __attribute__((address_space(1))) void*)(
                                             canonical_boxed + (size_t)(unit < box_count ? unit : box_count - 1u) * kWave + lane),
                                         (__attribute__((address_space(3))) void*)(image + kShellLoads * kWave), 4, 0, 0);
        const int corner = origin - 1 - sy - sz;
        int goff[kShellLoads];
#pragma unroll
        for (int j = 0; j < kShellLoads; ++j) goff[j] = s_goff[lane][j];
#pragma unroll
        for (int j = 0; j < kShellLoads; ++j) {
            int v = corner + goff[j];
            v = v < 0 ? 0 : (v > last_voxel ? last_voxel : v);
            __builtin_amdgcn_global_load_lds((const __attribute__((address_space(1))) void*)(state_in + v),
                                             (__attribute__((address_space(3))) void*)(image + j * kWave), 16, 0, 0);
        }
    };
    auto new_state = [&](const Deferred& d) {
        float v = d.rw.value();
        float wv[3] = {d.wv[0], d.wv[1], d.wv[2]};
        if (1.0f - fabsf(v) < 1e-6f) {
            v = v > 0.0f ? 1.0f : (v < 0.0f ? -1.0f : v);
            wv[0] = wv[1] = wv[2] = 0.0f;
        }
        vf4 o;
        o.x = v; o.y = wv[0]; o.z = wv[1]; o.w = wv[2];
        return o;
    };
    const __amdgpu_buffer_rsrc_t out_rsrc = __builtin_amdgcn_make_buffer_rsrc(
        state_out, 0, (int)((unsigned)(last_voxel + 1) * 16u), 0x00020000);
    auto store = [&](const vf4& o, int i) {
        const int offset = i < 0 ? (int)0xfffffff0u : i * 16;
        if (g.list_store_nt) __builtin_amdgcn_raw_buffer_store_b128(__builtin_bit_cast(vu4, o), out_rsrc, offset, 0, 2);
        else __builtin_amdgcn_raw_buffer_store_b128(__builtin_bit_cast(vu4, o), out_rsrc, offset, 0, 0);
    };

    unsigned u = box_count ? w.unit(wave) : w.x_end, u1 = w.unit(wave + waves);
    bool in0 = false, in1 = false, in2 = false;
    lsf_band_box b0 = {0, 0, 0ull}, b1 = b0;
    int parity = 0;
    if (u < w.x_end) {
        b0 = header(u, in0);
        b1 = header(u1, in1);
        stage(b0.origin, u, images);
    }
    while (u < w.x_end) {
        asm volatile("s_waitcnt vmcnt(0)" ::: "memory");
        const unsigned u2 = grab();
        const lsf_band_box b2 = header(u2, in2);
        const vf4* image = images + parity * kImage;
        const float cn = reinterpret_cast<const float*>(image + kShellLoads * kWave)[lane];
        stage(b1.origin, u1, images + (parity ^ 1) * kImage);
        __builtin_amdgcn_sched_barrier(0);
        NbhStateLds n;
        n.load(image, centre);
        const unsigned i = (unsigned)(b0.origin + voxel_off);
        const bool listed = in0 && ((b0.mask >> lane) & 1ull);
        int x0, y0, z0;
        decode_voxel(g, (unsigned)b0.origin, x0, y0, z0);
        const int x = x0 + lx, y = y0 + ly, z = z0 + lz;
        Deferred d;
        d.i = listed ? (int)i : -1;
        const float l = n.t[1][1][1].x;
        const bool in_band = listed && !(fabsf(l) == 1.0f && fabsf(cn) == 1.0f);
        float gv[3] = {0.0f, 0.0f, 0.0f};
        double e[3] = {0.0, 0.0, 0.0};
        band_voxel_gradient_taps<SMOOTH, LEVELSET, DATA, ENERGY>(n, p, l, cn, gv, e);
        const bool counted = in_band && z >= g.e_begin && z < g.e_end;
#pragma unroll
        for (int c = 0; c < 3; ++c) {
            d.wv[c] = in_band ? (-gv[c]) * p.rate : 0.0f;
            en[c] += counted ? e[c] : 0.0;
        }
        const float len = vec_length<3>(d.wv);
        const bool moved = !(d.wv[0] == 0.0f && d.wv[1] == 0.0f && d.wv[2] == 0.0f);
        if (!rewarp_from_image(n, image, centre, g, x, y, z, d.wv, listed, d.rw)) {
            d.rw.lerp = false;
            d.rw.R = state_gather<3>(state_in, g, (float)x + d.wv[0], (float)y + d.wv[1], (float)(z + g.z_global_offset) + d.wv[2]);
        }
        if (!moved) {
            d.rw.lerp = false;
            d.rw.R = l;
        }
        const unsigned long long q = listed ? pack_max(len, i + g.index_offset) : 0ull;
        best = q > best ? q : best;
        store(new_state(d), d.i);
        u = u1; u1 = u2;
        b0 = b1; b1 = b2;
        in0 = in1; in1 = in2;
        parity ^= 1;
    }
    asm volatile("s_waitcnt vmcnt(0)" ::: "memory");
    if (blockIdx.x == 0 && threadIdx.x == 0) {
        const unsigned long long q = pack_max(0.0f, linear_index(g, 0, 0, g.z_begin));
        best = q > best ? q : best;
    }
    double* dst[3] = {ENERGY != LSF_ENERGY_NONE ? &record_slot(record)->data_energy : nullptr,
                      ENERGY != LSF_ENERGY_NONE ? &record_slot(record)->smoothing_energy : nullptr,
                      ENERGY != LSF_ENERGY_NONE ? &record_slot(record)->level_set_energy : nullptr};
    block_reduce_commit<3>(best, en, record_max(record), dst);
}

struct BoxLaunch {
    unsigned blocks;
    hipStream_t s;
    const vf4* state_in;
    const float* canonical;
    vf4* state_out;
    Grid g;
    Params p;
    lsf_gate gate;
    lsf_iteration_record* record;
    const lsf_band_box* boxes;
    unsigned box_count;
};

constexpr size_t kBoxLdsBytes = (size_t)kBoxWaves * 2 * kImage * sizeof(vf4);

template <int SMOOTH, bool LEVELSET, int DATA, int ENERGY>
int launch_box(const BoxLaunch& a) {
    auto kernel = slavcheva_state_box_kernel<SMOOTH, LEVELSET, DATA, ENERGY>;
    static bool configured[64] = {false};
    int dev = 0;
    if (hipGetDevice(&dev) != hipSuccess || dev < 0 || dev >= 64) return (int)hipGetLastError();
    if (!configured[dev]) {
        if (hipFuncSetAttribute(reinterpret_cast<const void*>(kernel), hipFuncAttributeMaxDynamicSharedMemorySize,
                                (int)kBoxLdsBytes) != hipSuccess)
            return (int)hipGetLastError();
        configured[dev] = true;
    }
    hipLaunchKernelGGL(kernel, dim3(a.blocks), dim3(kBoxThreads), kBoxLdsBytes, a.s, a.state_in, a.canonical, a.state_out, a.g,
                       a.p, a.gate, a.record, a.boxes, a.box_count);
    return 0;
}

template <int SMOOTH, bool LEVELSET, int DATA>
int pick_box_energy(int energy, const BoxLaunch& a) {
    switch (energy) {
        case LSF_ENERGY_DIRECT: return launch_box<SMOOTH, LEVELSET, DATA, LSF_ENERGY_DIRECT>(a);
        case LSF_ENERGY_VECTORIZED: return launch_box<SMOOTH, LEVELSET, DATA, LSF_ENERGY_VECTORIZED>(a);
        default: return launch_box<SMOOTH, LEVELSET, DATA, LSF_ENERGY_NONE>(a);
    }
}

Params box_params(const lsf_slavcheva_params* q) {
    Params p;
    p.lambda64 = q->isomorphic_enforcement_factor_f64;
    p.rate = q->rate;
    p.w_data = q->data_term_weight;
    p.w_smooth = q->smoothing_term_weight;
    p.w_level_set = q->level_set_term_weight;
    p.lambda32 = q->isomorphic_enforcement_factor;
    p.killing_c1 = q->killing_c1;
    p.zero_gradient_on_snap = q->zero_gradient_on_snap;
    return p;
}

inline unsigned box_compute_units() {
    static int cached[64] = {0};
    int dev = 0;
    if (hipGetDevice(&dev) != hipSuccess || dev < 0 || dev >= 64) return 256u;
    if (!cached[dev]) {
        int n = 0;
        if (hipDeviceGetAttribute(&n, hipDeviceAttributeMultiprocessorCount, dev) != hipSuccess || n <= 0) n = 256;
        cached[dev] = n;
    }
    return (unsigned)cached[dev];
}

}

__global__ __launch_bounds__(kBlock) void box_canonical_kernel(const float* __restrict__ canonical,
                                                               const lsf_band_box* __restrict__ boxes, unsigned box_count,
                                                               int sy, int sz, float* __restrict__ out) {
    const unsigned b = blockIdx.x * (kBlock / kWave) + threadIdx.x / kWave, lane = threadIdx.x & (kWave - 1);
    if (b >= box_count) return;
    const int lx = lane & 3, ly = (lane >> 2) & 3, lz = lane >> 4;
    out[(size_t)b * kWave + lane] = canonical[boxes[b].origin + lz * sz + ly * sy + lx];
}

extern "C" int lsf_band_boxes_canonical(const float* canonical, const lsf_grid* grid, const lsf_band_box* boxes,
                                        int64_t box_count, float* canonical_boxed, void* stream) {
    if (int e = check_grid(grid)) return e;
    if (!canonical || !boxes || !canonical_boxed || box_count < 0 || box_count > 0x3ffffffll) return LSF_ERR_BAD_ARGUMENT;
    if (grid->dims != 3 || grid->nx % kBoxEdge || grid->ny % kBoxEdge || grid->nz % kBoxEdge ||
        (long long)grid->nx * grid->ny * grid->nz > 0x0fffffffll)
        return LSF_ERR_BAD_DIMS;
    if (box_count == 0) return 0;
    hipLaunchKernelGGL(box_canonical_kernel, dim3((unsigned)((box_count + kBlock / kWave - 1) / (kBlock / kWave))), dim3(kBlock),
                       0, as_stream(stream), canonical, boxes, (unsigned)box_count, grid->nx, grid->nx * grid->ny, canonical_boxed);
    return launch_status();
}

extern "C" int lsf_slavcheva_state_iteration_boxes(const float* state_in, const float* canonical_boxed, float* state_out,
                                                   const lsf_grid* grid, const lsf_slavcheva_params* params,
                                                   const lsf_gate* gate, lsf_iteration_record* record,
                                                   const lsf_band_box* boxes, int64_t box_count, void* stream) {
    if (int e = check_grid(grid)) return e;
    if (!state_in || !canonical_boxed || !state_out || state_out == state_in || !params || !record || !boxes || box_count < 0 ||
        box_count > 0x3ffffffll)
        return LSF_ERR_BAD_ARGUMENT;
    if (grid->dims != 3 || grid->nx % kBoxEdge || grid->ny % kBoxEdge || grid->nz % kBoxEdge ||
        (long long)grid->nx * grid->ny * grid->nz > 0x0fffffffll)
        return LSF_ERR_BAD_DIMS;
    if (box_count == 0) return 0;
    Grid g = make_grid(grid, 4);
    g.list_store_nt = box_count * 64ll * 32ll > 200ll * 1000 * 1000 * 5 / 4;
    BoxLaunch a{cu_list_blocks((unsigned)box_count * kWave, box_compute_units()), as_stream(stream),
                reinterpret_cast<const vf4*>(state_in), canonical_boxed, reinterpret_cast<vf4*>(state_out), g, box_params(params),
                gate_or_open(gate), record, boxes, (unsigned)box_count};
    const bool killing = params->smoothing_method == LSF_SMOOTHING_KILLING;
    const bool ls = params->level_set_enabled != 0;
    const bool fdm = params->data_method == LSF_DATA_THRESHOLDED_FDM;
    const int e = params->energy_mode;
    int status;
#define LSF_BOX(S, L, DM) status = pick_box_energy<S, L, DM>(e, a)
    if (killing) {
        if (ls) { if (fdm) LSF_BOX(LSF_SMOOTHING_KILLING, true, LSF_DATA_THRESHOLDED_FDM); else LSF_BOX(LSF_SMOOTHING_KILLING, true, LSF_DATA_BASIC); }
        else    { if (fdm) LSF_BOX(LSF_SMOOTHING_KILLING, false, LSF_DATA_THRESHOLDED_FDM); else LSF_BOX(LSF_SMOOTHING_KILLING, false, LSF_DATA_BASIC); }
    } else {
        if (ls) { if (fdm) LSF_BOX(LSF_SMOOTHING_TIKHONOV, true, LSF_DATA_THRESHOLDED_FDM); else LSF_BOX(LSF_SMOOTHING_TIKHONOV, true, LSF_DATA_BASIC); }
        else    { if (fdm) LSF_BOX(LSF_SMOOTHING_TIKHONOV, false, LSF_DATA_THRESHOLDED_FDM); else LSF_BOX(LSF_SMOOTHING_TIKHONOV, false, LSF_DATA_BASIC); }
    }
#undef LSF_BOX
    return status ? status : launch_status();
}
```

levelsetfusion-python_amd/csrc/lsf_slavcheva_run.hip:

```cpp
#include "lsf_device.h"

#include <cstring>

using namespace lsf;

namespace {

__global__ __launch_bounds__(kBlock) void records_used_words_kernel(const long long* __restrict__ records,
                                                                    const long long* __restrict__ statistics16,
                                                                    long long* __restrict__ out, int n_slots, int tail) {
    const int k = blockIdx.x * kBlock + threadIdx.x;
    if (k < n_slots * 4) out[k] = records[(long long)(k >> 2) * (sizeof(lsf_record_slot) / 8) + (k & 3)];
    else if (tail && k < n_slots * 4 + 16) out[k] = statistics16 ? statistics16[k - n_slots * 4] : 0ll;
}

inline hipEvent_t thread_event() {
    thread_local hipEvent_t events[64] = {};
    int dev = 0;
    if (hipGetDevice(&dev) != hipSuccess || dev < 0 || dev >= 64) return nullptr;
    if (!events[dev] && hipEventCreateWithFlags(&events[dev], hipEventDisableTiming) != hipSuccess) events[dev] = nullptr;
    return events[dev];
}

inline bool run_ok(const lsf_state_run* r) {
    return r && r->live && r->canonical && r->state[0] && r->state[1] && r->state[0] != r->state[1] && r->prepare_scratch &&
           r->totals_device && r->totals_host && r->sparse_reach >= 0 && r->sparse_reach <= 8;
}

}

extern "C" int lsf_state_run_begin(const lsf_state_run* run, void* stream) {
    if (!run_ok(run)) return LSF_ERR_BAD_ARGUMENT;
    const lsf_grid* g = &run->grid;
    if (int e = check_grid(g)) return e;
    if (g->z_begin != 0 || g->z_end != g->nz) return LSF_ERR_BAD_ARGUMENT;
    hipStream_t s = as_stream(stream);
    const bool sparse = run->sparse_reach > 0;
    float* b_in_pass = (sparse || run->second_state_late) ? nullptr : run->state[1];
    if (int e = lsf_state_prepare(run->live, run->canonical, sparse ? nullptr : run->state[0], b_in_pass, g,
                                  run->prepare_scratch, run->totals_device, stream))
        return e;
    if (run->box_scratch) {
        if (int e = lsf_band_boxes_count(g, run->box_all ? LSF_BAND_ALL : LSF_BAND_INTERIOR, run->prepare_scratch, run->box_scratch,
                                         run->totals_device + 4, stream))
            return e;
    } else if (hipMemsetAsync(run->totals_device + 4, 0, sizeof(int64_t), s) != hipSuccess) {
        return (int)hipGetLastError();
    }
    if (hipMemcpyAsync(run->totals_host, run->totals_device, 5 * sizeof(int64_t), hipMemcpyDeviceToHost, s) != hipSuccess)
        return (int)hipGetLastError();
    hipEvent_t sizes = thread_event();
    if (!sizes) return (int)hipGetLastError();
    int status = 0;
    if (hipEventRecord(sizes, s) != hipSuccess) status = (int)hipGetLastError();
    if (!status && sparse)
        status = lsf_state_pack_needed(run->live, run->state[0], run->state[1], g, run->prepare_scratch, run->sparse_reach, 0,
                                       stream);
    else if (!status && run->second_state_late)
        status = lsf_state_pack(run->live, nullptr, run->state[1], nullptr, g, stream);
    if (!status && hipEventSynchronize(sizes) != hipSuccess) status = (int)hipGetLastError();
    return status;
}

extern "C" int lsf_state_run_finish(const lsf_state_run* run, const lsf_slavcheva_params* params, int32_t* list_interior,
                                    int32_t* list_boundary, lsf_band_box* boxes, float* box_canonical,
                                    lsf_iteration_record* records, int32_t iterations, const lsf_run_loop* loop,
                                    float* live_out, float lower_threshold, double* statistics16,
                                    double* finalize_scratch, int64_t* words_device, int64_t* words_host,
                                    lsf_state_run_result* result, void* stream) {
    if (!run_ok(run) || !params || !records || iterations < 1 || !live_out || !words_device || !words_host || !result ||
        (statistics16 && !finalize_scratch) || !result->max_value || !result->argmax ||
        !result->energies3 || !result->executed)
        return LSF_ERR_BAD_ARGUMENT;
    if (loop && (loop->min_iterations < 1 || loop->check_interval < 1 ||
                 (loop->max_iterations > loop->min_iterations ? loop->max_iterations : loop->min_iterations) != iterations))
        return LSF_ERR_BAD_ARGUMENT;
    if (run->box_all && boxes) return LSF_ERR_BAD_ARGUMENT;
    const lsf_grid* g = &run->grid;
    if (int e = check_grid(g)) return e;
    const int64_t n_interior = run->totals_host[0], n_boundary = run->totals_host[1];
    if (n_interior < 0 || n_boundary < 0 || n_interior > 0x7fffffffll || n_boundary > 0x7fffffffll ||
        (n_interior && !list_interior) || (n_boundary && !list_boundary))
        return LSF_ERR_BAD_ARGUMENT;
    hipStream_t s = as_stream(stream);
    const int32_t* lists[2];
    int64_t counts[2];
    int32_t subsets[2];
    int n_lists = 0;
    if (n_interior) {
        if (int e = lsf_band_list_fill_prepared(g, LSF_BAND_INTERIOR, run->prepare_scratch, list_interior, stream)) return e;
        lists[n_lists] = list_interior; counts[n_lists] = n_interior; subsets[n_lists++] = LSF_BAND_INTERIOR;
    }
    if (n_boundary || !n_lists) {
        if (n_boundary)
            if (int e = lsf_band_list_fill_prepared(g, LSF_BAND_BOUNDARY, run->prepare_scratch, list_boundary, stream)) return e;
        lists[n_lists] = n_boundary ? list_boundary : reinterpret_cast<const int32_t*>(run->prepare_scratch);
        counts[n_lists] = n_boundary; subsets[n_lists++] = LSF_BAND_BOUNDARY;
    }
    const int64_t n_boxes = boxes && run->box_scratch ? run->totals_host[4] : 0;
    if (n_boxes > 0) {
        if (!box_canonical) return LSF_ERR_BAD_ARGUMENT;
        if (int e = lsf_band_boxes_fill(g, LSF_BAND_INTERIOR, run->prepare_scratch, run->box_scratch, boxes, stream)) return e;
        if (int e = lsf_band_boxes_canonical(run->canonical, g, boxes, n_boxes, box_canonical, stream)) return e;
    }
    const bool sparse = run->sparse_reach > 0;
    const int n_slots = iterations * LSF_RECORD_SLOTS;
    const bool fixed = !loop || loop->min_iterations >= iterations;
    int32_t it = 0, n_exec = fixed ? iterations : 0;
    while (it < iterations) {
        const int32_t batch = fixed ? iterations : (loop->check_interval < iterations - it ? loop->check_interval : iterations - it);
        for (int32_t i = it; i < it + batch; ++i) {
            lsf_gate gate_i{records + (i > 0 ? i - 1 : 0), LSF_GATE_SLAVCHEVA, loop ? loop->lower_threshold : 0.0f,
                            loop ? loop->upper_threshold : 0.0f};
            const lsf_gate* gate = (fixed || i < loop->min_iterations) ? nullptr : &gate_i;
            for (int k = 0; k < n_lists; ++k) {
                int e;
                if (n_boxes > 0 && subsets[k] == LSF_BAND_INTERIOR)
                    e = lsf_slavcheva_state_iteration_boxes(run->state[i % 2], box_canonical, run->state[(i + 1) % 2], g, params,
                                                            gate, records + i, boxes, n_boxes, stream);
                else
                    e = lsf_slavcheva_state_iteration(run->state[i % 2], run->canonical, run->state[(i + 1) % 2], g, params,
                                                      gate, records + i, lists[k], counts[k], subsets[k], stream);
                if (e) return e;
            }
        }
        it += batch;
        if (fixed) break;
        const int first_slot = (it - batch) * LSF_RECORD_SLOTS, batch_slots = batch * LSF_RECORD_SLOTS;
        hipLaunchKernelGGL(records_used_words_kernel, dim3((batch_slots * 4 + kBlock - 1) / kBlock), dim3(kBlock), 0, s,
                           reinterpret_cast<const long long*>(records + (it - batch)), nullptr,
                           reinterpret_cast<long long*>(words_device) + (size_t)first_slot * 4, batch_slots, 0);
        if (int e = launch_status()) return e;
        if (hipMemcpyAsync(words_host + (size_t)first_slot * 4, words_device + (size_t)first_slot * 4,
                           (size_t)batch_slots * 4 * sizeof(int64_t), hipMemcpyDeviceToHost, s) != hipSuccess)
            return (int)hipGetLastError();
        if (hipStreamSynchronize(s) != hipSuccess) return (int)hipGetLastError();
        if (int e = lsf_records_decode(words_host, it, LSF_RECORD_SLOTS, 4, result->max_value, result->argmax,
                                       result->energies3, result->executed))
            return e;
        n_exec = 0;
        while (n_exec < it && result->executed[n_exec]) ++n_exec;
        if (n_exec < it) break;
        const float m = result->max_value[n_exec - 1];
        if (n_exec >= loop->min_iterations && !(loop->lower_threshold < m && m < loop->upper_threshold)) break;
    }
    const float* final_state = run->state[n_exec % 2];
    int64_t listed_counts[2] = {0, 0};
    const int32_t* listed[2] = {nullptr, nullptr};
    int n_listed = 0;
    for (int k = 0; k < n_lists; ++k)
        if (counts[k]) { listed[n_listed] = lists[k]; listed_counts[n_listed++] = counts[k]; }
    if (int e = lsf_state_finalize_listed(final_state, run->canonical, live_out, nullptr, g, listed, listed_counts, n_listed,
                                          run->totals_host[2], run->totals_host[3], lower_threshold, statistics16,
                                          finalize_scratch, nullptr, sparse ? records : nullptr, sparse ? iterations : 0,
                                          (float)run->sparse_reach, stream))
        return e;
    hipLaunchKernelGGL(records_used_words_kernel, dim3((n_slots * 4 + 16 + kBlock - 1) / kBlock), dim3(kBlock), 0, s,
                       reinterpret_cast<const long long*>(records), reinterpret_cast<const long long*>(statistics16),
                       reinterpret_cast<long long*>(words_device), n_slots, 1);
    if (int e = launch_status()) return e;
    if (hipMemcpyAsync(words_host, words_device, ((size_t)n_slots * 4 + 16) * sizeof(int64_t), hipMemcpyDeviceToHost, s) !=
        hipSuccess)
        return (int)hipGetLastError();
    if (hipStreamSynchronize(s) != hipSuccess) return (int)hipGetLastError();
    if (int e = lsf_records_decode(words_host, iterations, LSF_RECORD_SLOTS, 4, result->max_value, result->argmax,
                                   result->energies3, result->executed))
        return e;
    result->final_state = n_exec % 2;
    result->n_lists = n_lists;
    result->reach_exceeded = 0;
    result->compact_faces = -1;
    for (int32_t i = 0; i < iterations && sparse; ++i)
        if (result->executed[i] && !(result->max_value[i] < (float)run->sparse_reach)) result->reach_exceeded = 1;
    return 0;
}

extern "C" int lsf_sobolev_run_finish(const lsf_state_run* run, const lsf_slavcheva_params* params, const double* taps_host,
                                      int32_t n_taps, int32_t* list_interior, int32_t* list_boundary, int32_t* list_all,
                                      lsf_band_box* boxes, float* g4_a, float* g4_b, lsf_iteration_record* records,
                                      int32_t iterations, const lsf_run_loop* loop, float* live_out, float lower_threshold,
                                      double* statistics16, double* finalize_scratch, int64_t* words_device,
                                      int64_t* words_host, lsf_state_run_result* result, void* stream) {
    if (!run_ok(run) || !run->box_scratch || !run->box_all || !params || !taps_host || !boxes || !g4_a || !g4_b ||
        g4_a == g4_b || !records || iterations < 1 || !live_out || !words_device || !words_host || !result ||
        (statistics16 && !finalize_scratch) || !result->max_value || !result->argmax || !result->energies3 ||
        !result->executed)
        return LSF_ERR_BAD_ARGUMENT;
    if (loop && (loop->min_iterations < 1 || loop->check_interval < 1 ||
                 (loop->max_iterations > loop->min_iterations ? loop->max_iterations : loop->min_iterations) != iterations))
        return LSF_ERR_BAD_ARGUMENT;
    const lsf_grid* g = &run->grid;
    if (int e = check_grid(g)) return e;
    if (g->dims != 3) return LSF_ERR_BAD_DIMS;
    const int64_t n_interior = run->totals_host[0], n_boundary = run->totals_host[1], n_boxes = run->totals_host[4];
    if (n_interior < 0 || n_boundary < 0 || n_boxes < 0 || n_interior + n_boundary > 0x7fffffffll ||
        (n_interior && !list_interior) || (n_boundary && !list_boundary) || (n_interior && n_boundary && !list_all))
        return LSF_ERR_BAD_ARGUMENT;
    hipStream_t s = as_stream(stream);
    if (n_interior)
        if (int e = lsf_band_list_fill_prepared(g, LSF_BAND_INTERIOR, run->prepare_scratch, list_interior, stream)) return e;
    if (n_boundary)
        if (int e = lsf_band_list_fill_prepared(g, LSF_BAND_BOUNDARY, run->prepare_scratch, list_boundary, stream)) return e;
    const int32_t* all = n_interior ? list_interior : list_boundary;
    const int64_t n_all = n_interior + n_boundary;
    if (n_interior && n_boundary) {
        const int32_t* a[1] = {list_interior};
        const int32_t* b[1] = {list_boundary};
        int32_t* out[1] = {list_all};
        const int64_t na[1] = {n_interior}, nb[1] = {n_boundary};
        if (int e = lsf_merge_sorted_runs(a, na, b, nb, out, 1, stream)) return e;
        all = list_all;
    }
    if (n_boxes > 0)
        if (int e = lsf_band_boxes_fill(g, LSF_BAND_ALL, run->prepare_scratch, run->box_scratch, boxes, stream)) return e;
    const bool sparse = run->sparse_reach > 0;
    const int n_slots = iterations * LSF_RECORD_SLOTS;
    const bool fixed = !loop || loop->min_iterations >= iterations;
    int32_t it = 0, n_exec = fixed ? iterations : 0;
    while (it < iterations) {
        const int32_t batch = fixed ? iterations : (loop->check_interval < iterations - it ? loop->check_interval : iterations - it);
        for (int32_t i = it; i < it + batch; ++i) {
            lsf_gate gate_i{records + (i > 0 ? i - 1 : 0), LSF_GATE_SLAVCHEVA, loop ? loop->lower_threshold : 0.0f,
                            loop ? loop->upper_threshold : 0.0f};
            const lsf_gate* gate = (fixed || i < loop->min_iterations) ? nullptr : &gate_i;
            const float* s_in = run->state[i % 2];
            float* s_out = run->state[(i + 1) % 2];
            if (n_all)
                if (int e = lsf_sobolev_state_gradient_x(s_in, run->canonical, g4_a, g, params, taps_host, n_taps, gate,
                                                         records + i, all, n_all, 1, stream))
                    return e;
            float* g_out = (!fixed || i == iterations - 1) ? g4_b : nullptr;
            if (int e = lsf_sobolev_state_update_boxes(g4_a, s_in, s_out, g_out, g, params, taps_host, n_taps, gate, records + i,
                                                       boxes, n_boxes, stream))
                return e;
        }
        it += batch;
        if (fixed) break;
        const int first_slot = (it - batch) * LSF_RECORD_SLOTS, batch_slots = batch * LSF_RECORD_SLOTS;
        hipLaunchKernelGGL(records_used_words_kernel, dim3((batch_slots * 4 + kBlock - 1) / kBlock), dim3(kBlock), 0, s,
                           reinterpret_cast<const long long*>(records + (it - batch)), nullptr,
                           reinterpret_cast<long long*>(words_device) + (size_t)first_slot * 4, batch_slots, 0);
        if (int e = launch_status()) return e;
        if (hipMemcpyAsync(words_host + (size_t)first_slot * 4, words_device + (size_t)first_slot * 4,
                           (size_t)batch_slots * 4 * sizeof(int64_t), hipMemcpyDeviceToHost, s) != hipSuccess)
            return (int)hipGetLastError();
        if (hipStreamSynchronize(s) != hipSuccess) return (int)hipGetLastError();
        if (int e = lsf_records_decode(words_host, it, LSF_RECORD_SLOTS, 4, result->max_value, result->argmax,
                                       result->energies3, result->executed))
            return e;
        n_exec = 0;
        while (n_exec < it && result->executed[n_exec]) ++n_exec;
        if (n_exec < it) break;
        const float m = result->max_value[n_exec - 1];
        if (n_exec >= loop->min_iterations && !(loop->lower_threshold < m && m < loop->upper_threshold)) break;
    }
    const int32_t* listed[2] = {nullptr, nullptr};
    int64_t listed_counts[2] = {0, 0};
    int n_listed = 0;
    if (n_interior) { listed[n_listed] = list_interior; listed_counts[n_listed++] = n_interior; }
    if (n_boundary) { listed[n_listed] = list_boundary; listed_counts[n_listed++] = n_boundary; }
    if (int e = lsf_state_finalize_listed(run->state[n_exec % 2], run->canonical, live_out, nullptr, g, listed, listed_counts,
                                          n_listed, run->totals_host[2], run->totals_host[3], lower_threshold, statistics16,
                                          finalize_scratch, nullptr, sparse ? records : nullptr, sparse ? iterations : 0,
                                          (float)run->sparse_reach, stream))
        return e;
    hipLaunchKernelGGL(records_used_words_kernel, dim3((n_slots * 4 + 16 + kBlock - 1) / kBlock), dim3(kBlock), 0, s,
                       reinterpret_cast<const long long*>(records), reinterpret_cast<const long long*>(statistics16),
                       reinterpret_cast<long long*>(words_device), n_slots, 1);
    if (int e = launch_status()) return e;
    if (hipMemcpyAsync(words_host, words_device, ((size_t)n_slots * 4 + 16) * sizeof(int64_t), hipMemcpyDeviceToHost, s) !=
        hipSuccess)
        return (int)hipGetLastError();
    if (hipStreamSynchronize(s) != hipSuccess) return (int)hipGetLastError();
    if (int e = lsf_records_decode(words_host, iterations, LSF_RECORD_SLOTS, 4, result->max_value, result->argmax,
                                   result->energies3, result->executed))
        return e;
    result->final_state = n_exec % 2;
    result->n_lists = n_listed;
    result->reach_exceeded = 0;
    result->compact_faces = -1;
    for (int32_t i = 0; i < iterations && sparse; ++i)
        if (result->executed[i] && !(result->max_value[i] < (float)run->sparse_reach)) result->reach_exceeded = 1;
    return 0;
}
```

levelsetfusion-python_amd/csrc/lsf_slavcheva_state.hip:

```cpp
#include "lsf_slavcheva_state_taps.h"

using namespace lsf;
using namespace lsf::slav;

namespace {

#ifdef LSF_STATE_TRACE
__device__ unsigned long long* g_state_trace = nullptr;
__device__ unsigned long long* g_state_waves = nullptr;
constexpr unsigned kTraceBlocks = 64, kTraceUnits = 16, kTraceStamps = 8;
#define LSF_TRACE(slot)                                                                                               \
    do {                                                                                                              \
        if (trace_row && (threadIdx.x & 63) == 0) trace_row[slot] = __builtin_readcyclecounter();                     \
    } while (0)
#else
#define LSF_TRACE(slot) do {} while (0)
#endif

constexpr int kWalkDense = 0, kWalkList = 1, kWalkListInterior = 2, kWalkListYCut = 3, kWalkListInteriorYCut = 4;
constexpr int walk_of(int walk_code) {
    return walk_code == kWalkListYCut ? kWalkList : (walk_code == kWalkListInteriorYCut ? kWalkListInterior : walk_code);
}

template <int D, int SMOOTH, bool LEVELSET, int DATA, int ENERGY, int WALK_CODE>
__global__ __launch_bounds__(walk_of(WALK_CODE) == kWalkListInterior ? kCuBlock : kBlock)
__attribute__((amdgpu_waves_per_eu(walk_of(WALK_CODE) == kWalkList ? 3 : 4, 4)))
void slavcheva_state_kernel(const vf4* __restrict__ state_in,
                                                                 const float* __restrict__ canonical,
                                                                 vf4* __restrict__ state_out, Grid g, Params p,
                                                                 lsf_gate gate, lsf_iteration_record* record,
                                                                 const int* __restrict__ band_list,
                                                                 unsigned band_count) {
    constexpr int WALK = walk_of(WALK_CODE);
    if (WALK_CODE == WALK) {
        g.y_global_offset = 0;
        g.ny_global = g.ny;
        g.ey_begin = -0x7fffffff - 1;
        g.ey_end = 0x7fffffff;
        g.y_cut = 0;
    }
#ifdef LSF_STATE_TRACE
    unsigned long long* wave_row = (g_state_waves && WALK == kWalkListInterior)
                                       ? g_state_waves + ((unsigned long long)blockIdx.x * kMaxBlockWaves + threadIdx.x / 64) * 8 : nullptr;
    if (wave_row && (threadIdx.x & 63) == 0) wave_row[0] = __builtin_amdgcn_s_memrealtime();
#endif
    if (gate_closed(gate)) return;
    unsigned long long best = 0ull;
    double en[3] = {0.0, 0.0, 0.0};
    auto finish = [&](const Deferred& d) {
        if (d.i < 0) return;
        float v = d.rw.value();
        float wv[3] = {d.wv[0], d.wv[1], d.wv[2]};
        if (1.0f - fabsf(v) < 1e-6f) {
            v = v > 0.0f ? 1.0f : (v < 0.0f ? -1.0f : v);
            wv[0] = wv[1] = wv[2] = 0.0f;
        }
        vf4 o;
        o.x = v; o.y = wv[0]; o.z = wv[1]; o.w = wv[2];
        if (WALK == kWalkDense) __builtin_nontemporal_store(o, &state_out[d.i]);
        else if (g.list_store_nt) __builtin_nontemporal_store(o, &state_out[d.i]);
        else state_out[d.i] = o;
    };
    auto voxel = [&](int x, int y, int z, int i, const vf4& sc, float cn) {
        Deferred d;
        d.i = i;
        const float l = sc.x;
        float gv[3] = {0.0f, 0.0f, 0.0f};
        const bool in_band = !(fabsf(l) == 1.0f && fabsf(cn) == 1.0f);
        d.rw.lerp = false;
        d.rw.R = l;
        d.rw.P = d.rw.Q = d.rw.wfz = d.rw.wfy = d.rw.wfx = d.rw.corner = 0.0f;
        bool from_taps = false;
        if (in_band) {
            double e[3] = {0.0, 0.0, 0.0};
            const bool interior = x > 0 && x < g.nx - 1 && y > 0 && y < g.ny - 1 && (D == 2 || (z > 0 && z < g.nz - 1));
            if (g.wide_ok && __all(interior) && wave_span_ok(g, i)) {
                NbhStateFast<D> n;
                n.load(state_in, g, (unsigned)i, sc, !g.fast_ok);
                band_voxel_gradient<D, SMOOTH, LEVELSET, DATA, ENERGY>(n, p, l, cn, gv, e);
                float w_now[3] = {0.0f, 0.0f, 0.0f};
#pragma unroll
                for (int c = 0; c < D; ++c) w_now[c] = (-gv[c]) * p.rate;
                if (g.fast_ok) from_taps = rewarp_from_taps<D, true>(n, state_in, g, i, x, y, z, w_now, d.rw);
                else from_taps = rewarp_from_taps<D, false>(n, state_in, g, i, x, y, z, w_now, d.rw);
            } else {
                const NbhState<D> n(state_in, g, x, y, z, sc);
                band_voxel_gradient<D, SMOOTH, LEVELSET, DATA, ENERGY>(n, p, l, cn, gv, e);
            }
            if (z >= g.e_begin && z < g.e_end && y >= g.ey_begin && y < g.ey_end) {
                en[0] += e[0];
                en[1] += e[1];
                en[2] += e[2];
            }
        }
#pragma unroll
        for (int c = 0; c < 3; ++c) d.wv[c] = c < D ? (-gv[c]) * p.rate : 0.0f;
        const float len = vec_length<D>(d.wv);
        const bool moved = !(d.wv[0] == 0.0f && d.wv[1] == 0.0f && d.wv[2] == 0.0f);
        if (!moved) {
            d.rw.lerp = false;
            d.rw.R = l;
        } else if (!from_taps) {
            const float px = (float)x + d.wv[0], py = (float)(y + g.y_global_offset) + d.wv[1];
            const float pz = D == 3 ? (float)(z + g.z_global_offset) + d.wv[2] : 0.0f;
            d.rw.lerp = false;
            d.rw.R = state_gather<D>(state_in, g, px, py, pz);
        }
        const unsigned long long q = pack_max(len, linear_index(g, x, y, z));
        best = q > best ? q : best;
        return d;
    };
#ifdef LSF_STATE_TRACE
    unsigned long long* trace_row = nullptr;
    unsigned trace_unit = 0u;
#endif
// ... 57 lines not shown
            return (unsigned)band_list[k < band_count ? k : band_count - 1u];
        };
        __shared__ unsigned s_next_unit;
        if (WALK == kWalkListInterior) {
            if (threadIdx.x == 0) s_next_unit = 2u * waves;
            __syncthreads();
        }
        unsigned n_last = wave + waves;
        auto grab = [&]() {
            if (WALK != kWalkListInterior) return w.unit(n_last += waves);
            unsigned v = 0u;
            if ((threadIdx.x & (kWave - 1)) == 0) v = atomicAdd(&s_next_unit, 1u);
            return w.unit((unsigned)__builtin_amdgcn_readfirstlane((int)v));
        };
        unsigned u = band_count ? w.unit(wave) : w.x_end, u1 = w.unit(wave + waves), u2 = 0u;
        bool in0 = false, in1 = false, in2 = false;
        unsigned i0 = 0u, i1 = 0u;
        vf4 s0 = {0.0f, 0.0f, 0.0f, 0.0f};
        float c0 = 0.0f;
        if (u < w.x_end) {
            i0 = entry(u, in0);
            i1 = entry(u1, in1);
            s0 = state_in[i0];
            c0 = canonical[i0];
        }
        Deferred pending = nothing;
#ifdef LSF_STATE_TRACE
        if (wave_row && (threadIdx.x & 63) == 0) {
            wave_row[1] = __builtin_amdgcn_s_memrealtime();
            wave_row[4] = __builtin_readcyclecounter();
        }
#endif
        while (u < w.x_end) {
            u2 = grab();
            const vf4 s1 = state_in[i1];
            const float c1 = canonical[i1];
            const unsigned i2 = entry(u2, in2);
            if (WALK == kWalkListInterior) {
#ifdef LSF_STATE_TRACE
                const unsigned nth = trace_unit++;
                trace_row = (g_state_trace && blockIdx.x < kTraceBlocks && nth < kTraceUnits)
                                ? g_state_trace + ((((unsigned long long)blockIdx.x * kMaxBlockWaves + threadIdx.x / 64) * kTraceUnits + nth) * kTraceStamps)
                                : nullptr;
                if (trace_row && (threadIdx.x & 63) == 0) {
                    trace_row[6] = __builtin_amdgcn_s_getreg((4 << 0) | (0 << 6) | (31 << 11));
                    trace_row[7] = __builtin_amdgcn_s_getreg((20 << 0) | (0 << 6) | (31 << 11));
                }
#endif
                pending = interior_voxel(i0, s0, c0, in0, pending);
                LSF_TRACE(5);
#ifdef LSF_STATE_NO_DEFER
                finish(pending);
                pending = nothing;
#endif
            } else if (in0) {
                const unsigned zy = fast_div(i0, g.div_nx);
                const int x = (int)(i0 - zy * (unsigned)g.nx);
                const int z = (int)fast_div(zy, g.div_ny);
                const int y = (int)zy - z * g.ny;
                finish(voxel(x, y, z, (int)i0, s0, c0));
            }
            u = u1;
            u1 = u2;
            i0 = i1; in0 = in1; s0 = s1; c0 = c1;
            i1 = i2; in1 = in2;
        }
        finish(pending);
#ifdef LSF_STATE_TRACE
        if (wave_row && (threadIdx.x & 63) == 0) {
            wave_row[2] = __builtin_amdgcn_s_memrealtime();
            wave_row[5] = __builtin_readcyclecounter();
            wave_row[6] = __builtin_amdgcn_s_getreg((4 << 0) | (0 << 6) | (31 << 11));
            wave_row[7] = __builtin_amdgcn_s_getreg((20 << 0) | (0 << 6) | (31 << 11));
        }
#endif
        if (blockIdx.x == 0 && threadIdx.x == 0) {
            const unsigned long long q = pack_max(0.0f, linear_index(g, 0, 0, g.z_begin));
            best = q > best ? q : best;
        }
    }
    double* dst[3] = {ENERGY != LSF_ENERGY_NONE ? &record_slot(record)->data_energy : nullptr,
                      ENERGY != LSF_ENERGY_NONE ? &record_slot(record)->smoothing_energy : nullptr,
                      ENERGY != LSF_ENERGY_NONE ? &record_slot(record)->level_set_energy : nullptr};
    block_reduce_commit<3>(best, en, record_max(record), dst);
#ifdef LSF_STATE_TRACE
    if (wave_row && (threadIdx.x & 63) == 0) wave_row[3] = __builtin_amdgcn_s_memrealtime();
#endif
}

__global__ __launch_bounds__(kBlock) void state_pack_kernel(const float* __restrict__ live,
                                                            const float* __restrict__ warp, vf4* __restrict__ a,
                                                            vf4* __restrict__ b, long long first, long long n,
                                                            long long plane, int dims) {
    for (long long k = blockIdx.x * (long long)kBlock + threadIdx.x; k < n; k += (long long)gridDim.x * kBlock) {
        const long long i = first + k;
        vf4 o;
        o.x = live[i];
        o.y = warp ? warp[i] : 0.0f;
        o.z = warp ? warp[plane + i] : 0.0f;
        o.w = (warp && dims == 3) ? warp[2 * plane + i] : 0.0f;
        a[i] = o;
        if (b) b[i] = o;
    }
}

__global__ __launch_bounds__(kBlock) void state_unpack_kernel(const vf4* __restrict__ s, float* __restrict__ live,
                                                              float* __restrict__ planar,
                                                              float* __restrict__ interleaved, long long first,
                                                              long long n, long long plane, int dims) {
    for (long long k = blockIdx.x * (long long)kBlock + threadIdx.x; k < n; k += (long long)gridDim.x * kBlock) {
        const long long i = first + k;
        const vf4 v = s[i];
        if (live) live[i] = v.x;
        if (planar) {
            planar[i] = v.y;
            planar[plane + i] = v.z;
            if (dims == 3) planar[2 * plane + i] = v.w;
        }
        if (interleaved) {
            interleaved[i * dims] = v.y;
            interleaved[i * dims + 1] = v.z;
            if (dims == 3) interleaved[i * dims + 2] = v.w;
        }
    }
}

constexpr int kFinalizeWords = 12;

struct FinalizeAccumulator {
    unsigned long long best_w = 0ull, best_d = 0ull;
    double sums[6] = {0.0, 0.0, 0.0, 0.0, 0.0, 0.0};
    double mn = __longlong_as_double(0x7ff0000000000000ll);

    __device__ inline void add(const vf4& v, float cn, unsigned lin, int dims, float lo) {
        if (!(fabsf(v.x) == 1.0f && fabsf(cn) == 1.0f)) {
            const float wv[3] = {v.y, v.z, v.w};
            const float len = dims == 3 ? vec_length<3>(wv) : vec_length<2>(wv);
            const unsigned long long p = pack_max(len, lin);
            best_w = p > best_w ? p : best_w;
            sums[0] += 1.0;
            sums[1] += len > lo ? 1.0 : 0.0;
            sums[2] += (double)len;
            sums[3] += (double)len * (double)len;
        }
        const double d = fabs((double)cn - (double)v.x);
        const unsigned long long q = pack_max((float)d, lin);
        best_d = q > best_d ? q : best_d;
        sums[4] += d;
        sums[5] += d * d;
        mn = fmin(mn, d);
    }

    __device__ inline void store_row(double* __restrict__ row) {
        __shared__ unsigned long long s_w[kBlock / kWave], s_d[kBlock / kWave];
        __shared__ double s_mn[kBlock / kWave], s_sum[6][kBlock / kWave];
        const int lane = threadIdx.x & (kWave - 1), wave = threadIdx.x / kWave;
        best_w = wave_max_u64(best_w);
        best_d = wave_max_u64(best_d);
        for (int dl = kWave / 2; dl > 0; dl >>= 1) mn = fmin(mn, shfl_down_f64(mn, dl));
#pragma unroll
        for (int j = 0; j < 6; ++j) sums[j] = wave_sum_f64(sums[j]);
        if (lane == 0) {
            s_w[wave] = best_w; s_d[wave] = best_d; s_mn[wave] = mn;
#pragma unroll
            for (int j = 0; j < 6; ++j) s_sum[j][wave] = sums[j];
        }
        __syncthreads();
// ... 13 lines not shown
                double t = 0.0;
                for (int k = 0; k < kBlock / kWave; ++k) t += s_sum[j][k];
                row[3 + j] = t;
            }
        }
    }
};

__global__ __launch_bounds__(kBlock) void state_finalize_kernel(const vf4* __restrict__ s,
                                                                const float* __restrict__ src_live,
                                                                const float* __restrict__ src_warp,
                                                                const float* __restrict__ canonical,
                                                                float* __restrict__ live, float* __restrict__ planar,
                                                                float* __restrict__ interleaved, long long first,
                                                                long long n, long long plane, int dims,
                                                                long long index_offset, float lo,
                                                                double* __restrict__ scratch) {
    FinalizeAccumulator acc;
    for (long long k = blockIdx.x * (long long)kBlock + threadIdx.x; k < n; k += (long long)gridDim.x * kBlock) {
        const long long i = first + k;
        vf4 v;
        if (s) {
            v = s[i];
        } else {
            v.x = src_live[i];
            v.y = src_warp[i];
            v.z = src_warp[plane + i];
            v.w = dims == 3 ? src_warp[2 * plane + i] : 0.0f;
        }
        if (live) live[i] = v.x;
        if (planar) {
            planar[i] = v.y;
            planar[plane + i] = v.z;
            if (dims == 3) planar[2 * plane + i] = v.w;
        }
        if (interleaved) {
            interleaved[i * dims] = v.y;
            interleaved[i * dims + 1] = v.z;
            if (dims == 3) interleaved[i * dims + 2] = v.w;
        }
        if (scratch) acc.add(v, canonical[i], (unsigned)(i + index_offset), dims, lo);
    }
    if (scratch) acc.store_row(scratch + (long long)blockIdx.x * kFinalizeWords);
}

__global__ __launch_bounds__(kBlock) void state_finalize_list_kernel(const vf4* __restrict__ s,
                                                                     const float* __restrict__ canonical,
                                                                     float* __restrict__ live,
                                                                     float* __restrict__ interleaved,
                                                                     const int* __restrict__ list, unsigned count,
                                                                     int dims, long long index_offset, float lo,
                                                                     double* __restrict__ scratch,
                                                                     const int* __restrict__ skip_flag,
                                                                     const lsf_iteration_record* __restrict__ guard_records,
                                                                     unsigned guard_count, float guard_limit) {
    if (skip_flag && *skip_flag != 0) return;
    if (guard_records) {
        bool bad = false;
        for (unsigned k = threadIdx.x; k < guard_count * LSF_RECORD_SLOTS; k += kBlock) {
            const unsigned long long p = guard_records[k / LSF_RECORD_SLOTS].slot[k % LSF_RECORD_SLOTS].max_packed;
            if (p != 0ull) bad |= !(unpack_max_value(p) < guard_limit);
        }
        if (__syncthreads_or(bad)) return;
    }
    FinalizeAccumulator acc;
    for (unsigned k = blockIdx.x * kBlock + threadIdx.x; k < count; k += gridDim.x * kBlock) {
        const long long i = list[k];
        const vf4 v = s[i];
        if (live) live[i] = v.x;
        if (interleaved) {
            interleaved[i * dims] = v.y;
            interleaved[i * dims + 1] = v.z;
            if (dims == 3) interleaved[i * dims + 2] = v.w;
        }
        if (scratch) acc.add(v, canonical[i], (unsigned)(i + index_offset), dims, lo);
    }
    if (scratch) acc.store_row(scratch + (long long)blockIdx.x * kFinalizeWords);
}

__global__ __launch_bounds__(kBlock) void state_finalize_combine_kernel(const double* __restrict__ scratch,
                                                                        unsigned rows, double voxels,
                                                                        double* __restrict__ out16, double unlisted,
                                                                        double opposite, long long first_opposite,
                                                                        long long first_voxel) {
    unsigned long long best_w = 0ull, best_d = 0ull;
    double sums[6] = {0.0, 0.0, 0.0, 0.0, 0.0, 0.0};
    double mn = __longlong_as_double(0x7ff0000000000000ll);
    for (unsigned r = threadIdx.x; r < rows; r += kBlock) {
        const double* row = scratch + (long long)r * kFinalizeWords;
        const unsigned long long w = (unsigned long long)__double_as_longlong(row[0]);
        const unsigned long long d = (unsigned long long)__double_as_longlong(row[1]);
        best_w = w > best_w ? w : best_w;
        best_d = d > best_d ? d : best_d;
        mn = fmin(mn, row[2]);
#pragma unroll
        for (int j = 0; j < 6; ++j) sums[j] += row[3 + j];
    }
    __shared__ unsigned long long s_w[kBlock / kWave], s_d[kBlock / kWave];
    __shared__ double s_mn[kBlock / kWave], s_sum[6][kBlock / kWave];
    const int lane = threadIdx.x & (kWave - 1), wave = threadIdx.x / kWave;
    best_w = wave_max_u64(best_w);
    best_d = wave_max_u64(best_d);
    for (int dl = kWave / 2; dl > 0; dl >>= 1) mn = fmin(mn, shfl_down_f64(mn, dl));
#pragma unroll
    for (int j = 0; j < 6; ++j) sums[j] = wave_sum_f64(sums[j]);
    if (lane == 0) {
        s_w[wave] = best_w; s_d[wave] = best_d; s_mn[wave] = mn;
#pragma unroll
        for (int j = 0; j < 6; ++j) s_sum[j][wave] = sums[j];
    }
    __syncthreads();
    if (threadIdx.x != 0) return;
    unsigned long long w = 0ull, d = 0ull;
    double m = s_mn[0], t[6] = {0.0, 0.0, 0.0, 0.0, 0.0, 0.0};
    for (int k = 0; k < kBlock / kWave; ++k) {
        w = s_w[k] > w ? s_w[k] : w;
        d = s_d[k] > d ? s_d[k] : d;
        m = fmin(m, s_mn[k]);
#pragma unroll
        for (int j = 0; j < 6; ++j) t[j] += s_sum[j][k];
    }
    if (unlisted > opposite) m = fmin(m, 0.0);
    if (opposite > 0.0) {
        m = fmin(m, 2.0);
        const unsigned long long q = pack_max(2.0f, (unsigned)first_opposite);
        d = q > d ? q : d;
        t[4] += 2.0 * opposite;
        t[5] += 4.0 * opposite;
    }
    if (unlisted > 0.0 && (d >> 32) == 0ull) d = pack_max(0.0f, (unsigned)first_voxel);
    out16[0] = t[0]; out16[1] = t[1];
    out16[2] = w ? (double)unpack_max_value(w) : 0.0;
    out16[3] = t[2]; out16[4] = t[3];
    out16[5] = w ? (double)(~(unsigned)w) : -1.0;
    out16[6] = 0.0; out16[7] = 0.0;
    out16[8] = voxels; out16[9] = m;
    out16[10] = d ? (double)unpack_max_value(d) : 0.0;
    out16[11] = t[4]; out16[12] = t[5];
    out16[13] = d ? (double)(~(unsigned)d) : -1.0;
    out16[14] = 0.0; out16[15] = 0.0;
}

struct LaunchArgs {
    unsigned blocks, threads;
    hipStream_t s;
    const vf4* state_in;
    const float* canonical;
    vf4* state_out;
    Grid g;
    Params p;
    lsf_gate gate;
    lsf_iteration_record* record;
    const int* band_list;
    unsigned band_count;
};

template <int D, int SMOOTH, bool LEVELSET, int DATA, int ENERGY, int WALK>
void launch_one(const LaunchArgs& a) {
    if constexpr (D == 3 && (WALK == kWalkList || WALK == kWalkListInterior)) {
        if (a.g.y_cut) {
            hipLaunchKernelGGL((slavcheva_state_kernel<D, SMOOTH, LEVELSET, DATA, ENERGY,
                                                       WALK == kWalkList ? kWalkListYCut : kWalkListInteriorYCut>),
                               dim3(a.blocks), dim3(a.threads), 0, a.s, a.state_in, a.canonical, a.state_out, a.g, a.p, a.gate,
                               a.record, a.band_list, a.band_count);
            return;
        }
    }
    hipLaunchKernelGGL((slavcheva_state_kernel<D, SMOOTH, LEVELSET, DATA, ENERGY, WALK>), dim3(a.blocks),
                       dim3(a.threads), 0, a.s, a.state_in, a.canonical, a.state_out, a.g, a.p, a.gate,
                       a.record, a.band_list, a.band_count);
}

template <int D, int SMOOTH, bool LEVELSET, int DATA, int WALK>
void pick_energy(int energy, const LaunchArgs& a) {
    switch (energy) {
        case LSF_ENERGY_DIRECT: launch_one<D, SMOOTH, LEVELSET, DATA, LSF_ENERGY_DIRECT, WALK>(a); break;
        case LSF_ENERGY_VECTORIZED: launch_one<D, SMOOTH, LEVELSET, DATA, LSF_ENERGY_VECTORIZED, WALK>(a); break;
        default: launch_one<D, SMOOTH, LEVELSET, DATA, LSF_ENERGY_NONE, WALK>(a); break;
    }
}

template <int D, int WALK>
void pick_terms(const lsf_slavcheva_params* q, const LaunchArgs& a) {
    const bool killing = q->smoothing_method == LSF_SMOOTHING_KILLING;
    const bool ls = q->level_set_enabled != 0;
    const bool fdm = q->data_method == LSF_DATA_THRESHOLDED_FDM;
    const int e = q->energy_mode;
#define LSF_PICK(S, L, DM) pick_energy<D, S, L, DM, WALK>(e, a)
    if (killing) {
        if (ls) { if (fdm) LSF_PICK(LSF_SMOOTHING_KILLING, true, LSF_DATA_THRESHOLDED_FDM); else LSF_PICK(LSF_SMOOTHING_KILLING, true, LSF_DATA_BASIC); }
        else    { if (fdm) LSF_PICK(LSF_SMOOTHING_KILLING, false, LSF_DATA_THRESHOLDED_FDM); else LSF_PICK(LSF_SMOOTHING_KILLING, false, LSF_DATA_BASIC); }
    } else {
        if (ls) { if (fdm) LSF_PICK(LSF_SMOOTHING_TIKHONOV, true, LSF_DATA_THRESHOLDED_FDM); else LSF_PICK(LSF_SMOOTHING_TIKHONOV, true, LSF_DATA_BASIC); }
        else    { if (fdm) LSF_PICK(LSF_SMOOTHING_TIKHONOV, false, LSF_DATA_THRESHOLDED_FDM); else LSF_PICK(LSF_SMOOTHING_TIKHONOV, false, LSF_DATA_BASIC); }
    }
#undef LSF_PICK
}

Params make_params(const lsf_slavcheva_params* q) {
    Params p;
    p.lambda64 = q->isomorphic_enforcement_factor_f64;
    p.rate = q->rate;
    p.w_data = q->data_term_weight;
    p.w_smooth = q->smoothing_term_weight;
    p.w_level_set = q->level_set_term_weight;
    p.lambda32 = q->isomorphic_enforcement_factor;
    p.killing_c1 = q->killing_c1;
    p.zero_gradient_on_snap = q->zero_gradient_on_snap;
    return p;
}

inline unsigned compute_units() {
    static int cached[64] = {0};
    int dev = 0;
    if (hipGetDevice(&dev) != hipSuccess || dev < 0 || dev >= 64) return 256u;
    if (!cached[dev]) {
        int n = 0;
        if (hipDeviceGetAttribute(&n, hipDeviceAttributeMultiprocessorCount, dev) != hipSuccess || n <= 0) n = 256;
        cached[dev] = n;
    }
    return (unsigned)cached[dev];
}

inline bool range_of(const lsf_grid* grid, long long& first, long long& n) {
    const long long slice = (long long)grid->ny * grid->nx;
    first = slice * grid->z_begin;
    n = slice * (grid->z_end - grid->z_begin);
    return n > 0;
}

inline unsigned stream_blocks(long long n, long long cap = 8192) {
    const long long want = (n + kBlock - 1) / kBlock;
    return (unsigned)(want < cap ? want : cap);
}

inline unsigned finalize_blocks(long long n) { return stream_blocks(n, 2048); }

}

#ifdef LSF_STATE_TRACE
extern "C" int lsf_debug_set_state_trace(void* units, void* waves) {
    if (int e = (int)hipMemcpyToSymbol(HIP_SYMBOL(g_state_trace), &units, sizeof(units))) return e;
    return (int)hipMemcpyToSymbol(HIP_SYMBOL(g_state_waves), &waves, sizeof(waves));
}
#endif

extern "C" int lsf_state_pack(const float* live, const float* warp_planar, float* state_a, float* state_b,
                              const lsf_grid* grid, void* stream) {
    if (int e = check_grid(grid, true)) return e;
    if (!live || !state_a) return LSF_ERR_BAD_ARGUMENT;
    long long first, n;
    if (!range_of(grid, first, n)) return 0;
    hipLaunchKernelGGL(state_pack_kernel, dim3(stream_blocks(n)), dim3(kBlock), 0, as_stream(stream), live, warp_planar,
                       reinterpret_cast<vf4*>(state_a), reinterpret_cast<vf4*>(state_b), first, n,
                       (long long)grid->nz * grid->ny * grid->nx, grid->dims);
    return launch_status();
}

extern "C" int lsf_state_unpack(const float* state, float* live_out, float* warp_planar_out,
                                float* warp_interleaved_out, const lsf_grid* grid, void* stream) {
    if (int e = check_grid(grid, true)) return e;
    if (!state) return LSF_ERR_BAD_ARGUMENT;
    long long first, n;
    if (!range_of(grid, first, n)) return 0;
    hipLaunchKernelGGL(state_unpack_kernel, dim3(stream_blocks(n)), dim3(kBlock), 0, as_stream(stream),
                       reinterpret_cast<const vf4*>(state), live_out, warp_planar_out, warp_interleaved_out, first, n,
                       (long long)grid->nz * grid->ny * grid->nx, grid->dims);
    return launch_status();
}

extern "C" int64_t lsf_state_finalize_scratch_elements(const lsf_grid* grid) {
    if (check_grid(grid, true)) return 0;
    long long first, n;
    range_of(grid, first, n);
    return (int64_t)finalize_blocks(n > 0 ? n : 1) * kFinalizeWords;
}

extern "C" int lsf_state_finalize(const float* state, const float* canonical, float* live_out,
                                  float* warp_planar_out, float* warp_interleaved_out, const lsf_grid* grid,
                                  float lower_threshold, double* statistics16, double* scratch, void* stream) {
    if (int e = check_grid(grid, true)) return e;
    if (!state || (statistics16 && (!canonical || !scratch))) return LSF_ERR_BAD_ARGUMENT;
    if (statistics16 && grid_is_y_cut(grid)) return LSF_ERR_BAD_ARGUMENT;
    long long first, n;
    if (!range_of(grid, first, n)) return statistics16 ? LSF_ERR_BAD_ARGUMENT : 0;
    const unsigned blocks = finalize_blocks(n);
    const long long slice = (long long)grid->ny * grid->nx;
    hipLaunchKernelGGL(state_finalize_kernel, dim3(blocks), dim3(kBlock), 0, as_stream(stream),
                       reinterpret_cast<const vf4*>(state), (const float*)nullptr, (const float*)nullptr, canonical,
                       live_out, warp_planar_out, warp_interleaved_out, first, n, (long long)grid->nz * slice, grid->dims,
                       slice * grid->z_global_offset, lower_threshold, statistics16 ? scratch : (double*)nullptr);
    if (statistics16)
        hipLaunchKernelGGL(state_finalize_combine_kernel, dim3(1), dim3(kBlock), 0, as_stream(stream), scratch, blocks,
                           (double)n, statistics16, 0.0, 0.0, 0ll, 0ll);
    return launch_status();
}

extern "C" int lsf_planar_finalize(const float* live, const float* warp_planar, const float* canonical, float* live_out,
                                   float* warp_interleaved_out, const lsf_grid* grid, float lower_threshold,
                                   double* statistics16, double* scratch, void* stream) {
    if (int e = check_grid(grid)) return e;
    if (!live || !warp_planar || live_out == live || (statistics16 && (!canonical || !scratch)))
        return LSF_ERR_BAD_ARGUMENT;
    long long first, n;
    if (!range_of(grid, first, n)) return statistics16 ? LSF_ERR_BAD_ARGUMENT : 0;
    const unsigned blocks = finalize_blocks(n);
    const long long slice = (long long)grid->ny * grid->nx;
    hipLaunchKernelGGL(state_finalize_kernel, dim3(blocks), dim3(kBlock), 0, as_stream(stream), (const vf4*)nullptr, live,
                       warp_planar, canonical, live_out, (float*)nullptr, warp_interleaved_out, first, n,
                       (long long)grid->nz * slice, grid->dims, slice * grid->z_global_offset, lower_threshold,
                       statistics16 ? scratch : (double*)nullptr);
    if (statistics16)
        hipLaunchKernelGGL(state_finalize_combine_kernel, dim3(1), dim3(kBlock), 0, as_stream(stream), scratch, blocks,
                           (double)n, statistics16, 0.0, 0.0, 0ll, 0ll);
    return launch_status();
}

extern "C" int lsf_state_finalize_listed(const float* state, const float* canonical, float* live_out,
                                         float* warp_interleaved_out, const lsf_grid* grid,
                                         const int32_t* const* band_lists, const int64_t* band_counts, int32_t n_lists,
                                         int64_t opposite_count, int64_t first_opposite, float lower_threshold,
                                         double* statistics16, double* scratch, const int32_t* skip_flag,
                                         const lsf_iteration_record* guard_records, int32_t guard_count, float guard_limit,
                                         void* stream) {
    if (int e = check_grid(grid, true)) return e;
    if (statistics16 && grid_is_y_cut(grid)) return LSF_ERR_BAD_ARGUMENT;
    if (!state || n_lists < 0 || n_lists > 2 || (n_lists && (!band_lists || !band_counts)) ||
        (statistics16 && (!canonical || !scratch)) || grid->z_begin != 0 || grid->z_end != grid->nz)
        return LSF_ERR_BAD_ARGUMENT;
    long long first, n;
    if (!range_of(grid, first, n)) return statistics16 ? LSF_ERR_BAD_ARGUMENT : 0;
    unsigned rows = 0;
    long long listed = 0;
    for (int32_t k = 0; k < n_lists; ++k)
        if (band_counts[k] < 0 || band_counts[k] > 0x7fffffffll || (band_counts[k] && !band_lists[k])) return LSF_ERR_BAD_ARGUMENT;
    for (int32_t k = 0; k < n_lists; ++k) {
        if (band_counts[k] == 0) continue;
        const unsigned blocks = finalize_blocks(band_counts[k]);
        hipLaunchKernelGGL(state_finalize_list_kernel, dim3(blocks), dim3(kBlock), 0, as_stream(stream),
                           reinterpret_cast<const vf4*>(state), canonical, live_out, warp_interleaved_out, band_lists[k],
                           (unsigned)band_counts[k], grid->dims, (long long)grid->ny * grid->nx * grid->z_global_offset,
                           lower_threshold, statistics16 ? scratch + (long long)rows * kFinalizeWords : (double*)nullptr,
                           skip_flag, guard_records, (unsigned)(guard_records && guard_count > 0 ? guard_count : 0), guard_limit);
        rows += blocks;
        listed += band_counts[k];
    }
    if (statistics16) {
        const long long first_voxel = (long long)grid->ny * grid->nx * grid->z_global_offset;
        hipLaunchKernelGGL(state_finalize_combine_kernel, dim3(1), dim3(kBlock), 0, as_stream(stream), scratch, rows,
                           (double)n, statistics16, (double)(n - listed), (double)opposite_count,
                           (long long)first_opposite + first_voxel, first_voxel);
    }
    return launch_status();
}

extern "C" int lsf_slavcheva_state_iteration(const float* state_in, const float* canonical, float* state_out,
                                             const lsf_grid* grid, const lsf_slavcheva_params* params,
                                             const lsf_gate* gate, lsf_iteration_record* record,
                                             const int32_t* band_list, int64_t band_count, int32_t band_subset,
                                             void* stream) {
    if (int e = check_grid(grid, true)) return e;
    if (!state_in || !canonical || !state_out || state_out == state_in || !params || !record)
        return LSF_ERR_BAD_ARGUMENT;
    if (grid_is_y_cut(grid) && (!band_list || grid->dims != 3)) return LSF_ERR_BAD_ARGUMENT;
    const int tile_y = 4;
    Grid g = make_grid(grid, tile_y);
    g.fast_ok = g.plane * 16 < 0xffffffffll;
    g.wide_ok = 16ll * (2ll * grid->nx * grid->ny + 2ll * grid->nx + 3) < 0x7fffffffll;
    Tiling t = make_tiling(g);
    if (t.total == 0) return 0;
    const bool listed = band_list != nullptr;
    if (listed && (band_count < 0 || band_count > 0x7fffffffll ||
                   !(band_subset == LSF_BAND_ALL || band_subset == LSF_BAND_INTERIOR || band_subset == LSF_BAND_BOUNDARY)))
        return LSF_ERR_BAD_ARGUMENT;
    const bool all_interior = listed && band_subset == LSF_BAND_INTERIOR && g.fast_ok;
    const unsigned blocks = all_interior ? cu_list_blocks((unsigned)band_count, compute_units())
                            : listed     ? band_list_blocks((unsigned)band_count, 128u)
                                         : launch_blocks(t.total, blocks_per_xcd());
#ifdef LSF_LIST_THREADS
    const unsigned list_threads = LSF_LIST_THREADS;
#else
    const unsigned list_threads = kCuBlock;
#endif
#ifdef LSF_LIST_GROUP
    g.list_group = LSF_LIST_GROUP;
#endif
    g.list_store_nt = listed && band_count * 32ll > 200ll * 1000 * 1000;
    LaunchArgs a{blocks, all_interior ? list_threads : (unsigned)(kTileX * tile_y), as_stream(stream), reinterpret_cast<const vf4*>(state_in), canonical,
                 reinterpret_cast<vf4*>(state_out), g, make_params(params), gate_or_open(gate), record, band_list,
                 (unsigned)band_count};
    if (grid->dims == 2) {
        if (all_interior) pick_terms<2, kWalkListInterior>(params, a);
        else if (listed) pick_terms<2, kWalkList>(params, a);
        else pick_terms<2, kWalkDense>(params, a);
    } else {
        if (all_interior) pick_terms<3, kWalkListInterior>(params, a);
        else if (listed) pick_terms<3, kWalkList>(params, a);
        else pick_terms<3, kWalkDense>(params, a);
    }
    return launch_status();
}
```

levelsetfusion-python_amd/engine_options.py:

```python
import os
import types

SLAVCHEVA_DEFAULTS = dict(
    use_band_list=True,
    library_run=True,
    box_walk=None,
    sobolev_boxes=True,
    sparse_reach=None,
    sparse_min_voxels=None,
    box_walk_min_band_bytes=100 * 1000 * 1000,
    box_walk_min_voxels=1 << 25,
)

HIERARCHICAL_DEFAULTS = dict(
    use_graphs=True,
    graph_max_voxels=1 << 21,
    fused_filter=True,
    fused_filter_min_voxels=1 << 23,
    defer_maximum=True,
    blocked_levels=True,
)


def apply(engine, defaults, options):
    options = dict(options or {})
    unknown = sorted(set(options) - set(defaults))
    if unknown:
        raise TypeError("unknown engine option(s) %s (known: %s)" % (", ".join(unknown), ", ".join(sorted(defaults))))
    for name, value in defaults.items():
        setattr(engine, name, options.get(name, value))
    if "sparse_reach" in defaults:
        if engine.sparse_reach is None:
            engine.sparse_reach = int(os.environ.get("LSF_SPARSE_REACH", "2"))
        if engine.sparse_min_voxels is None:
            engine.sparse_min_voxels = int(os.environ.get("LSF_SPARSE_MIN_VOXELS", str(1 << 21)))


def new_call_report():
    return types.SimpleNamespace(sparse_states=False, box_walk=False, sobolev_boxes=False, library_run=False,
                                 blocked_levels=0)
```

levelsetfusion-python_amd/engine_run.py:

```python
import ctypes

import numpy as np
import torch

from . import _lib, device as dev
from .engine_common import _Counted
from .engine_outcome import _RunLog, _RunOutcome


class _SparseStateExceeded(Exception):
    """a call whose ping-pong states were initialised near the band only (dev.StatePrepare(sparse_reach=...)) met a warp
    update that can read beyond that; nothing of the caller's has been modified (SlavchevaEngine.optimize repeats the
    call on fully initialised states and keeps doing so for this optimizer)"""


class _RunGradient:

    def __init__(self, g4):
        self._g4 = g4

    def final_gradient_planar(self, dims):
        return self._g4[..., :dims].movedim(-1, 0).contiguous()


class RunMixin:

    def _optimize_run(self, live, canonical, grid, finalize, sobolev=False):
        live_out, lower_threshold, statistics = finalize
        iterations = max(self.min_iterations, self.max_iterations)
        loop = None
        if self.min_iterations < iterations:
            loop = _lib.RunLoop(self.min_iterations, self.max_iterations, self.lo, self.hi, self.check_interval, 0)
        device = live.device
        n = dev.n_voxels(grid)
        whole = dev.full_range(grid)
        sparse = (self.sparse_reach > 0 and n >= self.sparse_min_voxels and not self.sparse_disabled)
        self.last_call.sparse_states = sparse
        self.last_call.library_run = True
        usable = (live_out is not None and live_out.is_cuda and live_out.dtype == torch.float32
                  and live_out.is_contiguous() and tuple(live_out.shape) == tuple(live.shape))
        target = live_out if usable else torch.empty_like(live)
        if target is not live:
            target.copy_(live)
        states = [torch.empty(tuple(live.shape) + (4,), dtype=torch.float32, device=device) for _ in range(2)]
        scratch = torch.empty(int(_lib.lib.lsf_state_prepare_scratch_elements(ctypes.byref(whole))), dtype=torch.int32,
                              device=device)
        totals = torch.empty(5, dtype=torch.int64, device=device)
        totals_host = dev.pinned_scratch("run totals", 5, torch.int64)
        run = _lib.StateRun()
        run.live, run.canonical = dev._ptr(live, n, "live"), dev._ptr(canonical, n, "canonical")
        run.state[0], run.state[1] = states[0].data_ptr(), states[1].data_ptr()
        run.prepare_scratch, run.totals_device, run.totals_host = scratch.data_ptr(), totals.data_ptr(), totals_host.data_ptr()
        run.grid = whole
        run.sparse_reach = self.sparse_reach if sparse else 0
        run.second_state_late = int(not sparse and n <= dev.StatePrepare.SPLIT_MAX_VOXELS)
        count_boxes = sobolev or (dev.boxes_ok(whole) and (self.box_walk is True or
                                                           (self.box_walk is None and n >= self.box_walk_min_voxels)))
        run.box_all = int(sobolev)
        box_scratch = None
        if count_boxes:
            box_scratch = torch.empty(int(_lib.lib.lsf_band_boxes_scratch_elements(ctypes.byref(whole))),
                                      dtype=torch.int32, device=device)
            run.box_scratch = box_scratch.data_ptr()
        stream = dev.stream_ptr()
        _lib.check(_lib.lib.lsf_state_run_begin(ctypes.byref(run), stream), "lsf_state_run_begin")
        n_interior, n_boundary, opposite, first_opposite, n_boxes = totals_host.tolist()
        lists = torch.empty(max(n_interior + n_boundary, 1), dtype=torch.int32, device=device)
        boxes = box_canonical = None
        if sobolev:
            boxes = torch.empty((max(n_boxes, 1), 2), dtype=torch.int64, device=device)
            list_all = torch.empty(max(n_interior + n_boundary, 1), dtype=torch.int32, device=device) \
                if n_interior and n_boundary else None
            g4 = self._sobolev_gradient_buffers(live, whole, lists, n_interior + n_boundary)
            taps = np.ascontiguousarray(np.asarray(self.sobolev_kernel, dtype=np.float64))
            self.last_call.sobolev_boxes = True
        elif n_boxes and (self.box_walk is True or 32 * n_interior > self.box_walk_min_band_bytes):
            boxes = torch.empty((n_boxes, 2), dtype=torch.int64, device=device)
            box_canonical = torch.empty(n_boxes * dev.BOX_EDGE ** 3, dtype=torch.float32, device=device)
        self.last_call.box_walk = boxes is not None and not sobolev
        records = dev.new_records(iterations, device)
        n_words = iterations * _lib.RECORD_SLOTS * dev.USED_SLOT_WORDS
        words = torch.empty(n_words + 16, dtype=torch.int64, device=device)
        words_host = dev.pinned_scratch("run records", words.numel(), torch.int64)
        stats = stats_scratch = None
        if statistics:
            stats = torch.empty(16, dtype=torch.float64, device=device)
            stats_scratch = torch.empty(2 * int(_lib.lib.lsf_state_finalize_scratch_elements(ctypes.byref(whole))),
                                        dtype=torch.float64, device=device)
        max_value, argmax = np.empty(iterations, np.float32), np.empty(iterations, np.int64)
        energies, executed = np.empty((iterations, 3), np.float64), np.empty(iterations, np.bool_)
        result = _lib.StateRunResult(max_value.ctypes.data, argmax.ctypes.data, energies.ctypes.data, executed.ctypes.data)
        none = ctypes.c_void_p(0)
        p_lists = lists.data_ptr()
        bands = []
        if n_interior:
            bands.append(dev.BandList(lists[:n_interior], n_interior, _lib.BAND_INTERIOR))
        if n_boundary or not bands:
            bands.append(dev.BandList(lists[n_interior:] if n_boundary else lists[:1], n_boundary, _lib.BAND_BOUNDARY))
        f = _Counted(sum(b.count for b in bands))
        f.bands, f.records, f.boxes = bands, records, (boxes, box_canonical)
        outcome = _RunOutcome(grid, canonical, None, target, bands, None)
        weights = tuple(self.weights)
        if sobolev:
            f.keep = (g4, list_all, taps)
            self._sobolev_band = f
            _lib.check(_lib.lib.lsf_sobolev_run_finish(
                ctypes.byref(run), ctypes.byref(self.params), taps.ctypes.data_as(ctypes.POINTER(ctypes.c_double)),
                int(taps.size), ctypes.c_void_p(p_lists), ctypes.c_void_p(p_lists + 4 * n_interior),
                ctypes.c_void_p(list_all.data_ptr() if list_all is not None else 0), ctypes.c_void_p(boxes.data_ptr()),
                ctypes.c_void_p(g4[0].data_ptr()), ctypes.c_void_p(g4[1].data_ptr()), ctypes.c_void_p(records.data_ptr()),
                iterations, ctypes.byref(loop) if loop is not None else None, dev._ptr(target, n, "live_out"),
                float(lower_threshold), ctypes.c_void_p(stats.data_ptr()) if statistics else none,
                ctypes.c_void_p(stats_scratch.data_ptr()) if statistics else none, ctypes.c_void_p(words.data_ptr()),
                ctypes.c_void_p(words_host.data_ptr()), ctypes.byref(result), stream), "lsf_sobolev_run_finish")
        else:
            self._run_finish(run, p_lists, n_interior, boxes, box_canonical, records, iterations, loop, target, n,
                             lower_threshold, stats, stats_scratch, statistics, words, words_host, result, stream)
        return self._after_run(result, executed, iterations, f, max_value, argmax, energies, weights, states, canonical, grid,
                               bands, outcome, statistics, words_host, n_words, g4[1] if sobolev else None)

    def _sobolev_gradient_buffers(self, live, whole, lists, n_listed):
        key = (tuple(live.shape), live.device)
        cache = getattr(self, "_g4_cache", None)
        if cache is not None and cache[0] == key:
            _, g4, old_lists, old_n = cache
            for t, bricks in ((g4[0], 1), (g4[1], 0)):
                _lib.check(_lib.lib.lsf_zero_listed4(ctypes.c_void_p(t.data_ptr()), ctypes.byref(whole),
                                                     ctypes.c_void_p(old_lists.data_ptr()), old_n, bricks, dev.stream_ptr()),
                           "lsf_zero_listed4")
        else:
            self._g4_cache = None
            g4 = [torch.zeros(tuple(live.shape) + (4,), dtype=torch.float32, device=live.device) for _ in range(2)]
        self._g4_cache = (key, g4, lists, int(n_listed))
        return g4

    def _run_finish(self, run, p_lists, n_interior, boxes, box_canonical, records, iterations, loop, target, n,
                    lower_threshold, stats, stats_scratch, statistics, words, words_host, result, stream):
        none = ctypes.c_void_p(0)
        _lib.check(_lib.lib.lsf_state_run_finish(
            ctypes.byref(run), ctypes.byref(self.params), ctypes.c_void_p(p_lists),
            ctypes.c_void_p(p_lists + 4 * n_interior), ctypes.c_void_p(boxes.data_ptr() if boxes is not None else 0),
            ctypes.c_void_p(box_canonical.data_ptr() if boxes is not None else 0),
            ctypes.c_void_p(records.data_ptr()), iterations, ctypes.byref(loop) if loop is not None else None,
            dev._ptr(target, n, "live_out"), float(lower_threshold),
            ctypes.c_void_p(stats.data_ptr()) if statistics else none,
            ctypes.c_void_p(stats_scratch.data_ptr()) if statistics else none, ctypes.c_void_p(words.data_ptr()),
            ctypes.c_void_p(words_host.data_ptr()), ctypes.byref(result), stream), "lsf_state_run_finish")

    def _after_run(self, result, executed, iterations, f, max_value, argmax, energies, weights, states, canonical, grid, bands,
                   outcome, statistics, words_host, n_words, sobolev_gradient):
        if result.reach_exceeded:
            raise _SparseStateExceeded()
        n_exec = iterations if executed.all() else int(executed.sum())
        self._fast = f
        self.iteration_count = n_exec
        self.log = _RunLog(max_value[:n_exec], argmax[:n_exec], energies[:n_exec], weights)
        if sobolev_gradient is not None:
            self._gradient_state = ("float4", _RunGradient(sobolev_gradient), grid.dims)
        else:
            self._gradient_state = ("recompute_listed", states[(n_exec - 1) % 2], canonical, grid, bands)
        outcome.state = states[n_exec % 2]
        if statistics:
            outcome._raw = words_host[n_words:].numpy().view(np.float64).copy()
        return outcome
```

Measured before the change: 521.1 billion.

## Write per-wave reduction rows instead of atomic record commits; fuse chunk-needed into pack

Iteration kernels can now store per-wave max/energy partials into a row buffer instead of doing a block reduction with atomic commits to the iteration record. The rows are reduced later, presumably in the finish stage. The aim is to cut global atomic contention and block-level synchronisation in each iteration. Separately, the chunk-needed computation is fused into the pack kernel, which removes one launch. The fifth count is also zeroed inside the scan kernel, saving a memset. In exchange the change adds a scratch buffer and an extra reduction pass.

```diff
diff --git a/include/lsf_hip.h b/include/lsf_hip.h
--- a/include/lsf_hip.h
+++ b/include/lsf_hip.h
@@ -252,6 +252,13 @@
                          float *live_out,
                          float lower_threshold, double *statistics16, double *finalize_scratch, int64_t *words_device,
                          int64_t *words_host, lsf_state_run_result *result, void *stream);
+int lsf_state_run_finish_rows(const lsf_state_run *run, const lsf_slavcheva_params *params, int32_t *list_interior,
+                              int32_t *list_boundary, lsf_band_box *boxes, float *box_canonical,
+                              lsf_iteration_record *records, int32_t iterations, const lsf_run_loop *loop, float *live_out,
+                              float lower_threshold, double *statistics16, double *finalize_scratch, int64_t *words_device,
+                              int64_t *words_host, lsf_state_run_result *result, int64_t *record_rows,
+                              int64_t record_rows_elements, int32_t *rows_taken, void *stream);
+int64_t lsf_state_run_rows_elements(const lsf_grid *grid, int32_t iterations, int32_t n_lists);
 
 int lsf_sobolev_run_finish(const lsf_state_run *run, const lsf_slavcheva_params *params, const double *taps_host,
                            int32_t n_taps, int32_t *list_interior, int32_t *list_boundary, int32_t *list_all,
diff --git a/levelsetfusion-python_amd/_lib.py b/levelsetfusion-python_amd/_lib.py
--- a/levelsetfusion-python_amd/_lib.py
+++ b/levelsetfusion-python_amd/_lib.py
@@ -9,7 +9,7 @@
 
 MAX_KERNEL_TAPS = 31
 ABI_VERSION = 4
-HEADER_ABI_HASH = "88f9a6300475259d"
+HEADER_ABI_HASH = "e7f8790ad697fe6d"
 
 ERRORS = {-1: "LSF_ERR_BAD_ARGUMENT", -2: "LSF_ERR_BAD_DIMS", -3: "LSF_ERR_KERNEL_TOO_LONG",
           -4: "LSF_ERR_RCCL_UNAVAILABLE", -5: "LSF_ERR_RCCL_FAILED", -6: "LSF_ERR_NOT_RESIDENT"}
@@ -394,6 +394,10 @@
     "lsf_slavcheva_state_iteration_boxes": (ctypes.c_int, [_vp, _vp, _vp, _P(Grid), _P(SlavchevaParams), _P(Gate), _vp, _vp,
                                                            _i64, _vp]),
     "lsf_state_run_begin": (ctypes.c_int, [_P(StateRun), _vp]),
+    "lsf_state_run_finish_rows": (ctypes.c_int, [_P(StateRun), _P(SlavchevaParams), _vp, _vp, _vp, _vp, _vp, _i32, _P(RunLoop),
+                                                 _vp, _f32, _vp, _vp, _vp, _vp, _P(StateRunResult), _vp, ctypes.c_int64,
+                                                 _P(ctypes.c_int32), _vp]),
+    "lsf_state_run_rows_elements": (ctypes.c_int64, [_P(Grid), _i32, _i32]),
     "lsf_state_run_finish": (ctypes.c_int, [_P(StateRun), _P(SlavchevaParams), _vp, _vp, _vp, _vp, _vp, _i32, _P(RunLoop), _vp,
                                             _f32, _vp, _vp, _vp, _vp, _P(StateRunResult), _vp]),
     "lsf_sobolev_run_finish": (ctypes.c_int, [_P(StateRun), _P(SlavchevaParams), _P(ctypes.c_double), _i32, _vp, _vp, _vp, _vp,
diff --git a/levelsetfusion-python_amd/csrc/lsf_device.h b/levelsetfusion-python_amd/csrc/lsf_device.h
--- a/levelsetfusion-python_amd/csrc/lsf_device.h
+++ b/levelsetfusion-python_amd/csrc/lsf_device.h
@@ -309,6 +309,13 @@
     const unsigned cap = default_per_xcd;
     const unsigned rounds = (per_xcd + cap - 1) / cap;
     return kXcds * ((per_xcd + rounds - 1) / rounds);
+}
+
+__host__ inline unsigned band_list_blocks_max(unsigned count, unsigned default_per_xcd = 256u) {
+    const unsigned units = (count + kBlock - 1) / kBlock;
+    if (units <= kXcds) return units < 1 ? 1 : units;
+    const unsigned per_xcd = (units + kXcds - 1) / kXcds;
+    return kXcds * (per_xcd < default_per_xcd ? per_xcd : default_per_xcd);
 }
 
 
@@ -501,6 +508,22 @@
     }
 }
 
+struct alignas(32) RecordRow {
+    unsigned long long max_packed;
+    double data, smoothing, level_set;
+};
+
+__device__ inline void wave_reduce_store_row(unsigned long long packed, const double (&sums)[3], RecordRow* __restrict__ rows) {
+    RecordRow r;
+    r.max_packed = wave_max_u64(packed);
+    r.data = wave_sum_f64(sums[0]);
+    r.smoothing = wave_sum_f64(sums[1]);
+    r.level_set = wave_sum_f64(sums[2]);
+    if ((threadIdx.x & (kWave - 1)) == 0) rows[blockIdx.x * (blockDim.x / kWave) + threadIdx.x / kWave] = r;
+}
+
+__host__ inline unsigned launch_rows(unsigned blocks, unsigned threads) { return blocks * (threads / kWave); }
+
 template <int NT>
 struct TapsN {
     double k[NT];
@@ -564,4 +587,24 @@
 
 inline int launch_status() { return (int)hipGetLastError(); }
 
-}
+int state_iteration_launch(const float* state_in, const float* canonical, float* state_out, const lsf_grid* grid,
+                           const lsf_slavcheva_params* params, const lsf_gate* gate, lsf_iteration_record* record,
+                           const int32_t* band_list, int64_t band_count, int32_t band_subset, RecordRow* rows,
+                           unsigned rows_capacity, unsigned* rows_written, void* stream);
+int state_iteration_boxes_launch(const float* state_in, const float* canonical_boxed, float* state_out, const lsf_grid* grid,
+                                 const lsf_slavcheva_params* params, const lsf_gate* gate, lsf_iteration_record* record,
+                                 const lsf_band_box* boxes, int64_t box_count, RecordRow* rows, unsigned rows_capacity,
+                                 unsigned* rows_written, void* stream);
+int state_prepare_launch(const float* live, const float* canonical, float* state_a, float* state_b, const lsf_grid* grid,
+                         int32_t* scratch, int64_t* counts_out, bool zero_fifth, void* stream);
+unsigned state_iteration_rows_max(const lsf_grid* grid);
+unsigned state_iteration_boxes_rows_max(const lsf_grid* grid);
+int state_finalize_listed_launch(const float* state, const float* canonical, float* live_out, float* warp_interleaved_out,
+                                 const lsf_grid* grid, const int32_t* const* band_lists, const int64_t* band_counts,
+                                 int32_t n_lists, int64_t opposite_count, int64_t first_opposite, float lower_threshold,
+                                 double* statistics16, double* scratch, const int32_t* skip_flag,
+                                 const lsf_iteration_record* guard_records, int32_t guard_count, float guard_limit,
+                                 const lsf_iteration_record* word_records, int32_t n_word_slots, int64_t* words_out,
+                                 void* stream);
+
+}
diff --git a/levelsetfusion-python_amd/csrc/lsf_slavcheva.hip b/levelsetfusion-python_amd/csrc/lsf_slavcheva.hip
--- a/levelsetfusion-python_amd/csrc/lsf_slavcheva.hip
+++ b/levelsetfusion-python_amd/csrc/lsf_slavcheva.hip
@@ -406,10 +406,11 @@
 
 __global__ __launch_bounds__(1024) void band_scan_tiles_kernel(int* __restrict__ sums_base, unsigned n, unsigned stride,
                                                                const int* __restrict__ tile_out, unsigned tiles,
-                                                               long long* __restrict__ totals) {
+                                                               long long* __restrict__ totals, int zero_fifth) {
     const unsigned tile = blockIdx.x, a = blockIdx.y, t = threadIdx.x, lane = t & (kWave - 1), wave = t / kWave;
     if (a == 2u) {
         if (tile == 0u && t == 0u) {
+            if (zero_fifth) totals[4] = 0;
             long long sum = 0;
             int first = 0x7fffffff;
             for (unsigned k = 0; k < tiles; ++k) {
@@ -607,11 +608,8 @@
     }
 }
 
-__global__ __launch_bounds__(kBlock) void chunk_needed_kernel(unsigned chunks, long long row, long long slice, int dims,
-                                                              int reach, const int* __restrict__ nonempty,
-                                                              int* __restrict__ needed) {
-    const unsigned c = blockIdx.x * (kBlock / kWave) + threadIdx.x / kWave;
-    if (c >= chunks) return;
+__device__ inline bool chunk_is_needed(unsigned c, unsigned chunks, long long row, long long slice, int dims, int reach,
+                                       const int* __restrict__ nonempty) {
     const int lane = threadIdx.x % kWave;
     const long long c0 = (long long)c * kBandChunk;
     const int span = 2 * reach + 1, zs = dims == 3 ? span : 1;
@@ -625,20 +623,35 @@
         last = last >= (long long)chunks ? (long long)chunks - 1 : last;
         for (long long cand = first; cand <= last; ++cand) hit |= nonempty[cand] != 0;
     }
-    const bool any = __any(hit);
-    if (lane == 0) needed[c] = any ? 1 : 0;
+    return __any(hit);
 }
 
 constexpr int kPackChunks = 1;
+static_assert(kPackChunks <= kBlock / kWave, "a wave per chunk of the block forms the verdicts");
 __global__ __launch_bounds__(kBlock) void state_pack_needed_kernel(const float* __restrict__ live, vf4* __restrict__ a,
                                                                    vf4* __restrict__ b, unsigned n, unsigned chunks,
-                                                                   const int* __restrict__ needed, int want) {
+                                                                   int* __restrict__ needed, int want, int reach,
+                                                                   long long row, long long slice, int dims,
+                                                                   const int* __restrict__ nonempty) {
     const int t = threadIdx.x;
+    __shared__ int s_verdict[kPackChunks];
+    if (reach > 0) {
+        const int k = t / kWave;
+        const unsigned c = blockIdx.x * kPackChunks + k;
+        if (k < kPackChunks && c < chunks) {
+            const int any = chunk_is_needed(c, chunks, row, slice, dims, reach, nonempty) ? 1 : 0;
+            if (t % kWave == 0) {
+                needed[c] = any;
+                s_verdict[k] = any;
+            }
+        }
+        __syncthreads();
+    }
     int verdict[kPackChunks];
 #pragma unroll
     for (int k = 0; k < kPackChunks; ++k) {
         const unsigned c = blockIdx.x * kPackChunks + k;
-        verdict[k] = c < chunks ? needed[c] : -1;
+        verdict[k] = c < chunks ? (reach > 0 ? s_verdict[k] : needed[c]) : -1;
     }
 #pragma unroll
     for (int k = 0; k < kPackChunks; ++k) {
@@ -942,6 +955,11 @@
 
 extern "C" int lsf_state_prepare(const float* live, const float* canonical, float* state_a, float* state_b,
                                  const lsf_grid* grid, int32_t* scratch, int64_t* counts_out, void* stream) {
+    return state_prepare_launch(live, canonical, state_a, state_b, grid, scratch, counts_out, false, stream);
+}
+
+int lsf::state_prepare_launch(const float* live, const float* canonical, float* state_a, float* state_b, const lsf_grid* grid,
+                              int32_t* scratch, int64_t* counts_out, bool zero_fifth, void* stream) {
     if (int e = check_grid(grid, true)) return e;
     if (!live || !canonical || (!state_a && state_b) || !scratch || !counts_out) return LSF_ERR_BAD_ARGUMENT;
     if (grid->z_begin != 0 || grid->z_end != grid->nz) return LSF_ERR_BAD_ARGUMENT;
@@ -966,7 +984,7 @@
     hipLaunchKernelGGL(band_tile_totals_kernel, dim3(tiles, 3), dim3(1024), 0, s, scratch, chunks, chunks + 1,
                        (const int*)prepare_opposite(scratch, chunks), prepare_tile_totals(scratch, chunks), tiles);
     hipLaunchKernelGGL(band_scan_tiles_kernel, dim3(tiles, 3), dim3(1024), 0, s, scratch, chunks, chunks + 1,
-                       (const int*)prepare_tile_totals(scratch, chunks), tiles, (long long*)counts_out);
+                       (const int*)prepare_tile_totals(scratch, chunks), tiles, (long long*)counts_out, zero_fifth ? 1 : 0);
     return launch_status();
 }
 
@@ -977,13 +995,10 @@
     if (grid->z_begin != 0 || grid->z_end != grid->nz) return LSF_ERR_BAD_ARGUMENT;
     unsigned first, n, chunks;
     band_range(grid, first, n, chunks);
-    if (!invert)
-        hipLaunchKernelGGL(chunk_needed_kernel, dim3((chunks + kBlock / kWave - 1) / (kBlock / kWave)), dim3(kBlock), 0, as_stream(stream),
-                           chunks, (long long)grid->nx, (long long)grid->nx * grid->ny, grid->dims, reach,
-                           prepare_nonempty(scratch, chunks), prepare_needed(scratch, chunks));
     hipLaunchKernelGGL(state_pack_needed_kernel, dim3((chunks + kPackChunks - 1) / kPackChunks), dim3(kBlock), 0,
                        as_stream(stream), live, reinterpret_cast<vf4*>(state_a), reinterpret_cast<vf4*>(state_b), n, chunks,
-                       prepare_needed(scratch, chunks), invert ? 0 : 1);
+                       prepare_needed(scratch, chunks), invert ? 0 : 1, invert ? 0 : (int)reach, (long long)grid->nx,
+                       (long long)grid->nx * grid->ny, grid->dims, (const int*)prepare_nonempty(scratch, chunks));
     return launch_status();
 }
 
diff --git a/levelsetfusion-python_amd/csrc/lsf_slavcheva_box.hip b/levelsetfusion-python_amd/csrc/lsf_slavcheva_box.hip
--- a/levelsetfusion-python_amd/csrc/lsf_slavcheva_box.hip
+++ b/levelsetfusion-python_amd/csrc/lsf_slavcheva_box.hip
@@ -62,7 +62,7 @@
 __global__ __launch_bounds__(kBoxThreads) __attribute__((amdgpu_waves_per_eu(kBoxWaves / 4, kBoxWaves / 4)))
 void slavcheva_state_box_kernel(const vf4* __restrict__ state_in, const float* __restrict__ canonical_boxed,
                                 vf4* __restrict__ state_out, Grid g, Params p, lsf_gate gate, lsf_iteration_record* record,
-                                const lsf_band_box* __restrict__ boxes, unsigned box_count) {
+                                const lsf_band_box* __restrict__ boxes, unsigned box_count, RecordRow* __restrict__ rows) {
     g.y_global_offset = 0;
     g.ny_global = g.ny;
     g.y_cut = 0;
@@ -198,7 +198,8 @@
     double* dst[3] = {ENERGY != LSF_ENERGY_NONE ? &record_slot(record)->data_energy : nullptr,
                       ENERGY != LSF_ENERGY_NONE ? &record_slot(record)->smoothing_energy : nullptr,
                       ENERGY != LSF_ENERGY_NONE ? &record_slot(record)->level_set_energy : nullptr};
-    block_reduce_commit<3>(best, en, record_max(record), dst);
+    if (rows) wave_reduce_store_row(best, en, rows);
+    else block_reduce_commit<3>(best, en, record_max(record), dst);
 }
 
 struct BoxLaunch {
@@ -213,6 +214,7 @@
     lsf_iteration_record* record;
     const lsf_band_box* boxes;
     unsigned box_count;
+    RecordRow* rows;
 };
 
 constexpr size_t kBoxLdsBytes = (size_t)kBoxWaves * 2 * kImage * sizeof(vf4);
@@ -230,7 +232,7 @@
         configured[dev] = true;
     }
     hipLaunchKernelGGL(kernel, dim3(a.blocks), dim3(kBoxThreads), kBoxLdsBytes, a.s, a.state_in, a.canonical, a.state_out, a.g,
-                       a.p, a.gate, a.record, a.boxes, a.box_count);
+                       a.p, a.gate, a.record, a.boxes, a.box_count, a.rows);
     return 0;
 }
 
@@ -296,6 +298,21 @@
                                                    const lsf_grid* grid, const lsf_slavcheva_params* params,
                                                    const lsf_gate* gate, lsf_iteration_record* record,
                                                    const lsf_band_box* boxes, int64_t box_count, void* stream) {
+    return state_iteration_boxes_launch(state_in, canonical_boxed, state_out, grid, params, gate, record, boxes, box_count,
+                                        nullptr, 0u, nullptr, stream);
+}
+
+unsigned lsf::state_iteration_boxes_rows_max(const lsf_grid* grid) {
+    const long long n = (long long)grid->nz * grid->ny * grid->nx;
+    const unsigned count = (unsigned)(n < 0x0fffffffll ? n : 0x0fffffffll);
+    return launch_rows(cu_list_blocks(count, box_compute_units()), kBoxThreads);
+}
+
+int lsf::state_iteration_boxes_launch(const float* state_in, const float* canonical_boxed, float* state_out,
+                                      const lsf_grid* grid, const lsf_slavcheva_params* params, const lsf_gate* gate,
+                                      lsf_iteration_record* record, const lsf_band_box* boxes, int64_t box_count,
+                                      RecordRow* rows, unsigned rows_capacity, unsigned* rows_written, void* stream) {
+    if (rows_written) *rows_written = 0u;
     if (int e = check_grid(grid)) return e;
     if (!state_in || !canonical_boxed || !state_out || state_out == state_in || !params || !record || !boxes || box_count < 0 ||
         box_count > 0x3ffffffll)
@@ -306,9 +323,14 @@
     if (box_count == 0) return 0;
     Grid g = make_grid(grid, 4);
     g.list_store_nt = box_count * 64ll * 32ll > 200ll * 1000 * 1000 * 5 / 4;
-    BoxLaunch a{cu_list_blocks((unsigned)box_count * kWave, box_compute_units()), as_stream(stream),
-                reinterpret_cast<const vf4*>(state_in), canonical_boxed, reinterpret_cast<vf4*>(state_out), g, box_params(params),
-                gate_or_open(gate), record, boxes, (unsigned)box_count};
+    const unsigned blocks = cu_list_blocks((unsigned)box_count * kWave, box_compute_units());
+    if (rows) {
+        if (gate || launch_rows(blocks, kBoxThreads) > rows_capacity) return LSF_ERR_BAD_ARGUMENT;
+        if (rows_written) *rows_written = launch_rows(blocks, kBoxThreads);
+    }
+    BoxLaunch a{blocks, as_stream(stream), reinterpret_cast<const vf4*>(state_in), canonical_boxed,
+                reinterpret_cast<vf4*>(state_out), g, box_params(params), gate_or_open(gate), record, boxes,
+                (unsigned)box_count, rows};
     const bool killing = params->smoothing_method == LSF_SMOOTHING_KILLING;
     const bool ls = params->level_set_enabled != 0;
     const bool fdm = params->data_method == LSF_DATA_THRESHOLDED_FDM;
diff --git a/levelsetfusion-python_amd/csrc/lsf_slavcheva_run.hip b/levelsetfusion-python_amd/csrc/lsf_slavcheva_run.hip
--- a/levelsetfusion-python_amd/csrc/lsf_slavcheva_run.hip
+++ b/levelsetfusion-python_amd/csrc/lsf_slavcheva_run.hip
@@ -14,6 +14,57 @@
     else if (tail && k < n_slots * 4 + 16) out[k] = statistics16 ? statistics16[k - n_slots * 4] : 0ll;
 }
 
+__global__ __launch_bounds__(kBlock) void records_from_rows_kernel(const RecordRow* __restrict__ rows,
+                                                                   unsigned rows_per_iteration,
+                                                                   lsf_iteration_record* __restrict__ records) {
+    const RecordRow* mine = rows + (size_t)blockIdx.x * rows_per_iteration;
+    unsigned long long best = 0ull;
+    double sums[3] = {0.0, 0.0, 0.0};
+    for (unsigned r = threadIdx.x; r < rows_per_iteration; r += kBlock) {
+        const RecordRow row = mine[r];
+        best = row.max_packed > best ? row.max_packed : best;
+        sums[0] += row.data;
+        sums[1] += row.smoothing;
+        sums[2] += row.level_set;
+    }
+    __shared__ unsigned long long s_max[kBlock / kWave];
+    __shared__ double s_sum[3][kBlock / kWave];
+    const int lane = threadIdx.x & (kWave - 1), wave = threadIdx.x / kWave;
+    best = wave_max_u64(best);
+#pragma unroll
+    for (int j = 0; j < 3; ++j) sums[j] = wave_sum_f64(sums[j]);
+    if (lane == 0) {
+        s_max[wave] = best;
+#pragma unroll
+        for (int j = 0; j < 3; ++j) s_sum[j][wave] = sums[j];
+    }
+    __syncthreads();
+    lsf_iteration_record* record = records + blockIdx.x;
+    if (threadIdx.x == 0) {
+        unsigned long long m = 0ull;
+        double t[3] = {0.0, 0.0, 0.0};
+        for (int k = 0; k < kBlock / kWave; ++k) {
+            m = s_max[k] > m ? s_max[k] : m;
+#pragma unroll
+            for (int j = 0; j < 3; ++j) t[j] += s_sum[j][k];
+        }
+        record->slot[0].max_packed = m;
+        record->slot[0].data_energy = t[0];
+        record->slot[0].smoothing_energy = t[1];
+        record->slot[0].level_set_energy = t[2];
+    } else if (threadIdx.x < LSF_RECORD_SLOTS) {
+        record->slot[threadIdx.x].max_packed = 0ull;
+        record->slot[threadIdx.x].data_energy = 0.0;
+        record->slot[threadIdx.x].smoothing_energy = 0.0;
+        record->slot[threadIdx.x].level_set_energy = 0.0;
+    }
+}
+
+inline int64_t rows_per_iteration_max(const lsf_grid* g, int32_t n_lists) {
+    const unsigned list = state_iteration_rows_max(g), boxes = state_iteration_boxes_rows_max(g);
+    return (int64_t)(list > boxes ? list : boxes) + (n_lists > 1 ? (int64_t)list : 0);
+}
+
 inline hipEvent_t thread_event() {
     thread_local hipEvent_t events[64] = {};
     int dev = 0;
@@ -27,6 +78,29 @@
            r->totals_device && r->totals_host && r->sparse_reach >= 0 && r->sparse_reach <= 8;
 }
 
+inline int finalize_and_gather_words(const float* final_state, const float* canonical, float* live_out, const lsf_grid* g,
+                                     const int32_t* const* listed, const int64_t* listed_counts, int n_listed,
+                                     int64_t opposite_count, int64_t first_opposite, float lower_threshold,
+                                     double* statistics16, double* finalize_scratch, const lsf_iteration_record* guard_records,
+                                     int32_t guard_count, float guard_limit, const lsf_iteration_record* records, int n_slots,
+                                     int64_t* words_device, hipStream_t s) {
+    if (int e = state_finalize_listed_launch(final_state, canonical, live_out, nullptr, g, listed, listed_counts, n_listed,
+                                             opposite_count, first_opposite, lower_threshold, statistics16, finalize_scratch,
+                                             nullptr, guard_records, guard_count, guard_limit, statistics16 ? records : nullptr,
+                                             statistics16 ? n_slots : 0, statistics16 ? words_device : nullptr, s))
+        return e;
+    if (statistics16) return 0;
+    hipLaunchKernelGGL(records_used_words_kernel, dim3((n_slots * 4 + 16 + kBlock - 1) / kBlock), dim3(kBlock), 0, s,
+                       reinterpret_cast<const long long*>(records), (const long long*)nullptr,
+                       reinterpret_cast<long long*>(words_device), n_slots, 1);
+    return launch_status();
+}
+
+}
+
+extern "C" int64_t lsf_state_run_rows_elements(const lsf_grid* grid, int32_t iterations, int32_t n_lists) {
+    if (check_grid(grid) || iterations < 1 || n_lists < 1 || n_lists > 2) return 0;
+    return rows_per_iteration_max(grid, n_lists) * iterations * (int64_t)(sizeof(RecordRow) / sizeof(int64_t));
 }
 
 extern "C" int lsf_state_run_begin(const lsf_state_run* run, void* stream) {
@@ -37,16 +111,13 @@
     hipStream_t s = as_stream(stream);
     const bool sparse = run->sparse_reach > 0;
     float* b_in_pass = (sparse || run->second_state_late) ? nullptr : run->state[1];
-    if (int e = lsf_state_prepare(run->live, run->canonical, sparse ? nullptr : run->state[0], b_in_pass, g,
-                                  run->prepare_scratch, run->totals_device, stream))
-        return e;
-    if (run->box_scratch) {
+    if (int e = state_prepare_launch(run->live, run->canonical, sparse ? nullptr : run->state[0], b_in_pass, g,
+                                     run->prepare_scratch, run->totals_device, !run->box_scratch, stream))
+        return e;
+    if (run->box_scratch)
         if (int e = lsf_band_boxes_count(g, run->box_all ? LSF_BAND_ALL : LSF_BAND_INTERIOR, run->prepare_scratch, run->box_scratch,
                                          run->totals_device + 4, stream))
             return e;
-    } else if (hipMemsetAsync(run->totals_device + 4, 0, sizeof(int64_t), s) != hipSuccess) {
-        return (int)hipGetLastError();
-    }
     if (hipMemcpyAsync(run->totals_host, run->totals_device, 5 * sizeof(int64_t), hipMemcpyDeviceToHost, s) != hipSuccess)
         return (int)hipGetLastError();
     hipEvent_t sizes = thread_event();
@@ -68,6 +139,21 @@
                                     float* live_out, float lower_threshold, double* statistics16,
                                     double* finalize_scratch, int64_t* words_device, int64_t* words_host,
                                     lsf_state_run_result* result, void* stream) {
+    return lsf_state_run_finish_rows(run, params, list_interior, list_boundary, boxes, box_canonical, records, iterations, loop,
+                                     live_out, lower_threshold, statistics16, finalize_scratch, words_device, words_host,
+                                     result, nullptr, 0, nullptr, stream);
+}
+
+extern "C" int lsf_state_run_finish_rows(const lsf_state_run* run, const lsf_slavcheva_params* params, int32_t* list_interior,
+                                         int32_t* list_boundary, lsf_band_box* boxes, float* box_canonical,
+                                         lsf_iteration_record* records, int32_t iterations, const lsf_run_loop* loop,
+                                         float* live_out, float lower_threshold, double* statistics16,
+                                         double* finalize_scratch, int64_t* words_device, int64_t* words_host,
+                                         lsf_state_run_result* result, int64_t* record_rows, int64_t record_rows_elements,
+                                         int32_t* rows_taken, void* stream) {
+    if (rows_taken) *rows_taken = 0;
+    if (record_rows && (record_rows_elements <= 0 || (reinterpret_cast<uintptr_t>(record_rows) & 31u) != 0))
+        return LSF_ERR_BAD_ARGUMENT;
     if (!run_ok(run) || !params || !records || iterations < 1 || !live_out || !words_device || !words_host || !result ||
         (statistics16 && !finalize_scratch) || !result->max_value || !result->argmax ||
         !result->energies3 || !result->executed)
@@ -81,6 +167,12 @@
     const int64_t n_interior = run->totals_host[0], n_boundary = run->totals_host[1];
     if (n_interior < 0 || n_boundary < 0 || n_interior > 0x7fffffffll || n_boundary > 0x7fffffffll ||
         (n_interior && !list_interior) || (n_boundary && !list_boundary))
+        return LSF_ERR_BAD_ARGUMENT;
+    const bool fixed = !loop || loop->min_iterations >= iterations;
+    RecordRow* const rows = fixed ? reinterpret_cast<RecordRow*>(record_rows) : nullptr;
+    const int64_t rows_capacity = rows ? record_rows_elements / (int64_t)(sizeof(RecordRow) / sizeof(int64_t)) : 0;
+    if (rows && record_rows_elements <
+                    lsf_state_run_rows_elements(g, iterations, (n_interior ? 1 : 0) + ((n_boundary || !n_interior) ? 1 : 0)))
         return LSF_ERR_BAD_ARGUMENT;
     hipStream_t s = as_stream(stream);
     const int32_t* lists[2];
@@ -105,7 +197,7 @@
     }
     const bool sparse = run->sparse_reach > 0;
     const int n_slots = iterations * LSF_RECORD_SLOTS;
-    const bool fixed = !loop || loop->min_iterations >= iterations;
+    unsigned rows_per_iteration = 0u;
     int32_t it = 0, n_exec = fixed ? iterations : 0;
     while (it < iterations) {
         const int32_t batch = fixed ? iterations : (loop->check_interval < iterations - it ? loop->check_interval : iterations - it);
@@ -113,18 +205,32 @@
             lsf_gate gate_i{records + (i > 0 ? i - 1 : 0), LSF_GATE_SLAVCHEVA, loop ? loop->lower_threshold : 0.0f,
                             loop ? loop->upper_threshold : 0.0f};
             const lsf_gate* gate = (fixed || i < loop->min_iterations) ? nullptr : &gate_i;
+            int64_t row = (int64_t)i * rows_per_iteration;
             for (int k = 0; k < n_lists; ++k) {
                 int e;
+                unsigned written = 0u;
+                const unsigned room = rows ? (unsigned)(rows_capacity - row < 0x7fffffffll ? rows_capacity - row : 0x7fffffffll) : 0u;
                 if (n_boxes > 0 && subsets[k] == LSF_BAND_INTERIOR)
-                    e = lsf_slavcheva_state_iteration_boxes(run->state[i % 2], box_canonical, run->state[(i + 1) % 2], g, params,
-                                                            gate, records + i, boxes, n_boxes, stream);
+                    e = state_iteration_boxes_launch(run->state[i % 2], box_canonical, run->state[(i + 1) % 2], g, params, gate,
+                                                     records + i, boxes, n_boxes, rows ? rows + row : nullptr, room, &written,
+                                                     stream);
                 else
-                    e = lsf_slavcheva_state_iteration(run->state[i % 2], run->canonical, run->state[(i + 1) % 2], g, params,
-                                                      gate, records + i, lists[k], counts[k], subsets[k], stream);
+                    e = state_iteration_launch(run->state[i % 2], run->canonical, run->state[(i + 1) % 2], g, params, gate,
+                                               records + i, lists[k], counts[k], subsets[k], rows ? rows + row : nullptr, room,
+                                               &written, stream);
                 if (e) return e;
+                row += written;
             }
+            if (i == 0) rows_per_iteration = (unsigned)row;
+            else if (rows && row != (int64_t)(i + 1) * rows_per_iteration) return LSF_ERR_BAD_ARGUMENT;
         }
         it += batch;
+        if (rows) {
+            if (rows_per_iteration == 0u) return LSF_ERR_BAD_ARGUMENT;
+            hipLaunchKernelGGL(records_from_rows_kernel, dim3((unsigned)iterations), dim3(kBlock), 0, s, rows, rows_per_iteration,
+                               records);
+            if (int e = launch_status()) return e;
+        }
         if (fixed) break;
         const int first_slot = (it - batch) * LSF_RECORD_SLOTS, batch_slots = batch * LSF_RECORD_SLOTS;
         hipLaunchKernelGGL(records_used_words_kernel, dim3((batch_slots * 4 + kBlock - 1) / kBlock), dim3(kBlock), 0, s,
@@ -150,15 +256,11 @@
     int n_listed = 0;
     for (int k = 0; k < n_lists; ++k)
         if (counts[k]) { listed[n_listed] = lists[k]; listed_counts[n_listed++] = counts[k]; }
-    if (int e = lsf_state_finalize_listed(final_state, run->canonical, live_out, nullptr, g, listed, listed_counts, n_listed,
+    if (int e = finalize_and_gather_words(final_state, run->canonical, live_out, g, listed, listed_counts, n_listed,
                                           run->totals_host[2], run->totals_host[3], lower_threshold, statistics16,
-                                          finalize_scratch, nullptr, sparse ? records : nullptr, sparse ? iterations : 0,
-                                          (float)run->sparse_reach, stream))
-        return e;
-    hipLaunchKernelGGL(records_used_words_kernel, dim3((n_slots * 4 + 16 + kBlock - 1) / kBlock), dim3(kBlock), 0, s,
-                       reinterpret_cast<const long long*>(records), reinterpret_cast<const long long*>(statistics16),
-                       reinterpret_cast<long long*>(words_device), n_slots, 1);
-    if (int e = launch_status()) return e;
+                                          finalize_scratch, sparse ? records : nullptr, sparse ? iterations : 0,
+                                          (float)run->sparse_reach, records, n_slots, words_device, s))
+        return e;
     if (hipMemcpyAsync(words_host, words_device, ((size_t)n_slots * 4 + 16) * sizeof(int64_t), hipMemcpyDeviceToHost, s) !=
         hipSuccess)
         return (int)hipGetLastError();
@@ -170,6 +272,7 @@
     result->n_lists = n_lists;
     result->reach_exceeded = 0;
     result->compact_faces = -1;
+    if (rows_taken) *rows_taken = rows ? 1 : 0;
     for (int32_t i = 0; i < iterations && sparse; ++i)
         if (result->executed[i] && !(result->max_value[i] < (float)run->sparse_reach)) result->reach_exceeded = 1;
     return 0;
@@ -259,15 +362,11 @@
     int n_listed = 0;
     if (n_interior) { listed[n_listed] = list_interior; listed_counts[n_listed++] = n_interior; }
     if (n_boundary) { listed[n_listed] = list_boundary; listed_counts[n_listed++] = n_boundary; }
-    if (int e = lsf_state_finalize_listed(run->state[n_exec % 2], run->canonical, live_out, nullptr, g, listed, listed_counts,
-                                          n_listed, run->totals_host[2], run->totals_host[3], lower_threshold, statistics16,
-                                          finalize_scratch, nullptr, sparse ? records : nullptr, sparse ? iterations : 0,
-                                          (float)run->sparse_reach, stream))
-        return e;
-    hipLaunchKernelGGL(records_used_words_kernel, dim3((n_slots * 4 + 16 + kBlock - 1) / kBlock), dim3(kBlock), 0, s,
-                       reinterpret_cast<const long long*>(records), reinterpret_cast<const long long*>(statistics16),
-                       reinterpret_cast<long long*>(words_device), n_slots, 1);
-    if (int e = launch_status()) return e;
+    if (int e = finalize_and_gather_words(run->state[n_exec % 2], run->canonical, live_out, g, listed, listed_counts, n_listed,
+                                          run->totals_host[2], run->totals_host[3], lower_threshold, statistics16,
+                                          finalize_scratch, sparse ? records : nullptr, sparse ? iterations : 0,
+                                          (float)run->sparse_reach, records, n_slots, words_device, s))
+        return e;
     if (hipMemcpyAsync(words_host, words_device, ((size_t)n_slots * 4 + 16) * sizeof(int64_t), hipMemcpyDeviceToHost, s) !=
         hipSuccess)
         return (int)hipGetLastError();
diff --git a/levelsetfusion-python_amd/csrc/lsf_slavcheva_state.hip b/levelsetfusion-python_amd/csrc/lsf_slavcheva_state.hip
--- a/levelsetfusion-python_amd/csrc/lsf_slavcheva_state.hip
+++ b/levelsetfusion-python_amd/csrc/lsf_slavcheva_state.hip
@@ -30,7 +30,7 @@
                                                                  vf4* __restrict__ state_out, Grid g, Params p,
                                                                  lsf_gate gate, lsf_iteration_record* record,
                                                                  const int* __restrict__ band_list,
-                                                                 unsigned band_count) {
+                                                                 unsigned band_count, RecordRow* __restrict__ rows) {
     constexpr int WALK = walk_of(WALK_CODE);
     if (WALK_CODE == WALK) {
         g.y_global_offset = 0;
@@ -254,7 +254,8 @@
     double* dst[3] = {ENERGY != LSF_ENERGY_NONE ? &record_slot(record)->data_energy : nullptr,
                       ENERGY != LSF_ENERGY_NONE ? &record_slot(record)->smoothing_energy : nullptr,
                       ENERGY != LSF_ENERGY_NONE ? &record_slot(record)->level_set_energy : nullptr};
-    block_reduce_commit<3>(best, en, record_max(record), dst);
+    if (rows) wave_reduce_store_row(best, en, rows);
+    else block_reduce_commit<3>(best, en, record_max(record), dst);
 #ifdef LSF_STATE_TRACE
     if (wave_row && (threadIdx.x & 63) == 0) wave_row[3] = __builtin_amdgcn_s_memrealtime();
 #endif
@@ -434,7 +435,12 @@
                                                                         unsigned rows, double voxels,
                                                                         double* __restrict__ out16, double unlisted,
                                                                         double opposite, long long first_opposite,
-                                                                        long long first_voxel) {
+                                                                        long long first_voxel,
+                                                                        const long long* __restrict__ word_records,
+                                                                        int n_word_slots, long long* __restrict__ words_out) {
+    if (words_out)
+        for (int k = threadIdx.x; k < n_word_slots * 4; k += kBlock)
+            words_out[k] = word_records[(long long)(k >> 2) * (sizeof(lsf_record_slot) / 8) + (k & 3)];
     unsigned long long best_w = 0ull, best_d = 0ull;
     double sums[6] = {0.0, 0.0, 0.0, 0.0, 0.0, 0.0};
     double mn = __longlong_as_double(0x7ff0000000000000ll);
@@ -491,6 +497,8 @@
     out16[11] = t[4]; out16[12] = t[5];
     out16[13] = d ? (double)(~(unsigned)d) : -1.0;
     out16[14] = 0.0; out16[15] = 0.0;
+    if (words_out)
+        for (int j = 0; j < 16; ++j) words_out[n_word_slots * 4 + j] = __double_as_longlong(out16[j]);
 }
 
 struct LaunchArgs {
@@ -505,6 +513,7 @@
     lsf_iteration_record* record;
     const int* band_list;
     unsigned band_count;
+    RecordRow* rows;
 };
 
 template <int D, int SMOOTH, bool LEVELSET, int DATA, int ENERGY, int WALK>
@@ -514,13 +523,13 @@
             hipLaunchKernelGGL((slavcheva_state_kernel<D, SMOOTH, LEVELSET, DATA, ENERGY,
                                                        WALK == kWalkList ? kWalkListYCut : kWalkListInteriorYCut>),
                                dim3(a.blocks), dim3(a.threads), 0, a.s, a.state_in, a.canonical, a.state_out, a.g, a.p, a.gate,
-                               a.record, a.band_list, a.band_count);
+                               a.record, a.band_list, a.band_count, a.rows);
             return;
         }
     }
     hipLaunchKernelGGL((slavcheva_state_kernel<D, SMOOTH, LEVELSET, DATA, ENERGY, WALK>), dim3(a.blocks),
                        dim3(a.threads), 0, a.s, a.state_in, a.canonical, a.state_out, a.g, a.p, a.gate,
-                       a.record, a.band_list, a.band_count);
+                       a.record, a.band_list, a.band_count, a.rows);
 }
 
 template <int D, int SMOOTH, bool LEVELSET, int DATA, int WALK>
@@ -644,7 +653,7 @@
                        slice * grid->z_global_offset, lower_threshold, statistics16 ? scratch : (double*)nullptr);
     if (statistics16)
         hipLaunchKernelGGL(state_finalize_combine_kernel, dim3(1), dim3(kBlock), 0, as_stream(stream), scratch, blocks,
-                           (double)n, statistics16, 0.0, 0.0, 0ll, 0ll);
+                           (double)n, statistics16, 0.0, 0.0, 0ll, 0ll, (const long long*)nullptr, 0, (long long*)nullptr);
     return launch_status();
 }
 
@@ -664,7 +673,7 @@
                        statistics16 ? scratch : (double*)nullptr);
     if (statistics16)
         hipLaunchKernelGGL(state_finalize_combine_kernel, dim3(1), dim3(kBlock), 0, as_stream(stream), scratch, blocks,
-                           (double)n, statistics16, 0.0, 0.0, 0ll, 0ll);
+                           (double)n, statistics16, 0.0, 0.0, 0ll, 0ll, (const long long*)nullptr, 0, (long long*)nullptr);
     return launch_status();
 }
 
@@ -675,7 +684,20 @@
                                          double* statistics16, double* scratch, const int32_t* skip_flag,
                                          const lsf_iteration_record* guard_records, int32_t guard_count, float guard_limit,
                                          void* stream) {
+    return state_finalize_listed_launch(state, canonical, live_out, warp_interleaved_out, grid, band_lists, band_counts, n_lists,
+                                        opposite_count, first_opposite, lower_threshold, statistics16, scratch, skip_flag,
+                                        guard_records, guard_count, guard_limit, nullptr, 0, nullptr, stream);
+}
+
+int lsf::state_finalize_listed_launch(const float* state, const float* canonical, float* live_out, float* warp_interleaved_out,
+                                      const lsf_grid* grid, const int32_t* const* band_lists, const int64_t* band_counts,
+                                      int32_t n_lists, int64_t opposite_count, int64_t first_opposite, float lower_threshold,
+                                      double* statistics16, double* scratch, const int32_t* skip_flag,
+                                      const lsf_iteration_record* guard_records, int32_t guard_count, float guard_limit,
+                                      const lsf_iteration_record* word_records, int32_t n_word_slots, int64_t* words_out,
+                                      void* stream) {
     if (int e = check_grid(grid, true)) return e;
+    if (words_out && (!statistics16 || !word_records || n_word_slots < 0)) return LSF_ERR_BAD_ARGUMENT;
     if (statistics16 && grid_is_y_cut(grid)) return LSF_ERR_BAD_ARGUMENT;
     if (!state || n_lists < 0 || n_lists > 2 || (n_lists && (!band_lists || !band_counts)) ||
         (statistics16 && (!canonical || !scratch)) || grid->z_begin != 0 || grid->z_end != grid->nz)
@@ -701,7 +723,9 @@
         const long long first_voxel = (long long)grid->ny * grid->nx * grid->z_global_offset;
         hipLaunchKernelGGL(state_finalize_combine_kernel, dim3(1), dim3(kBlock), 0, as_stream(stream), scratch, rows,
                            (double)n, statistics16, (double)(n - listed), (double)opposite_count,
-                           (long long)first_opposite + first_voxel, first_voxel);
+                           (long long)first_opposite + first_voxel, first_voxel,
+                           reinterpret_cast<const long long*>(word_records), (int)n_word_slots,
+                           reinterpret_cast<long long*>(words_out));
     }
     return launch_status();
 }
@@ -711,6 +735,23 @@
                                              const lsf_gate* gate, lsf_iteration_record* record,
                                              const int32_t* band_list, int64_t band_count, int32_t band_subset,
                                              void* stream) {
+    return state_iteration_launch(state_in, canonical, state_out, grid, params, gate, record, band_list, band_count,
+                                  band_subset, nullptr, 0u, nullptr, stream);
+}
+
+unsigned lsf::state_iteration_rows_max(const lsf_grid* grid) {
+    const long long n = (long long)grid->nz * grid->ny * grid->nx;
+    const unsigned count = (unsigned)(n < 0x7fffffffll ? n : 0x7fffffffll);
+    const unsigned interior = launch_rows(cu_list_blocks(count, compute_units()), kCuBlock);
+    const unsigned general = launch_rows(band_list_blocks_max(count, 128u), kBlock);
+    return interior > general ? interior : general;
+}
+
+int lsf::state_iteration_launch(const float* state_in, const float* canonical, float* state_out, const lsf_grid* grid,
+                                const lsf_slavcheva_params* params, const lsf_gate* gate, lsf_iteration_record* record,
+                                const int32_t* band_list, int64_t band_count, int32_t band_subset, RecordRow* rows,
+                                unsigned rows_capacity, unsigned* rows_written, void* stream) {
+    if (rows_written) *rows_written = 0u;
     if (int e = check_grid(grid, true)) return e;
     if (!state_in || !canonical || !state_out || state_out == state_in || !params || !record)
         return LSF_ERR_BAD_ARGUMENT;
@@ -738,9 +779,14 @@
     g.list_group = LSF_LIST_GROUP;
 #endif
     g.list_store_nt = listed && band_count * 32ll > 200ll * 1000 * 1000;
-    LaunchArgs a{blocks, all_interior ? list_threads : (unsigned)(kTileX * tile_y), as_stream(stream), reinterpret_cast<const vf4*>(state_in), canonical,
+    const unsigned threads = all_interior ? list_threads : (unsigned)(kTileX * tile_y);
+    if (rows) {
+        if (!listed || gate || launch_rows(blocks, threads) > rows_capacity) return LSF_ERR_BAD_ARGUMENT;
+        if (rows_written) *rows_written = launch_rows(blocks, threads);
+    }
+    LaunchArgs a{blocks, threads, as_stream(stream), reinterpret_cast<const vf4*>(state_in), canonical,
                  reinterpret_cast<vf4*>(state_out), g, make_params(params), gate_or_open(gate), record, band_list,
-                 (unsigned)band_count};
+                 (unsigned)band_count, rows};
     if (grid->dims == 2) {
         if (all_interior) pick_terms<2, kWalkListInterior>(params, a);
         else if (listed) pick_terms<2, kWalkList>(params, a);
diff --git a/levelsetfusion-python_amd/engine_options.py b/levelsetfusion-python_amd/engine_options.py
--- a/levelsetfusion-python_amd/engine_options.py
+++ b/levelsetfusion-python_amd/engine_options.py
@@ -4,6 +4,7 @@
 SLAVCHEVA_DEFAULTS = dict(
     use_band_list=True,
     library_run=True,
+    record_rows=True,
     box_walk=None,
     sobolev_boxes=True,
     sparse_reach=None,
@@ -38,4 +39,4 @@
 
 def new_call_report():
     return types.SimpleNamespace(sparse_states=False, box_walk=False, sobolev_boxes=False, library_run=False,
-                                 blocked_levels=0)
+                                 blocked_levels=0, record_rows=False)
diff --git a/levelsetfusion-python_amd/engine_run.py b/levelsetfusion-python_amd/engine_run.py
--- a/levelsetfusion-python_amd/engine_run.py
+++ b/levelsetfusion-python_amd/engine_run.py
@@ -78,6 +78,11 @@
             boxes = torch.empty((n_boxes, 2), dtype=torch.int64, device=device)
             box_canonical = torch.empty(n_boxes * dev.BOX_EDGE ** 3, dtype=torch.float32, device=device)
         self.last_call.box_walk = boxes is not None and not sobolev
+        record_rows = None
+        if loop is None and not sobolev and self.record_rows:
+            n_launches = int(n_interior > 0) + int(n_boundary > 0 or n_interior == 0)
+            record_rows = torch.empty(int(_lib.lib.lsf_state_run_rows_elements(ctypes.byref(whole), iterations, n_launches)),
+                                      dtype=torch.int64, device=device)
         records = dev.new_records(iterations, device)
         n_words = iterations * _lib.RECORD_SLOTS * dev.USED_SLOT_WORDS
         words = torch.empty(n_words + 16, dtype=torch.int64, device=device)
@@ -115,7 +120,7 @@
                 ctypes.c_void_p(words_host.data_ptr()), ctypes.byref(result), stream), "lsf_sobolev_run_finish")
         else:
             self._run_finish(run, p_lists, n_interior, boxes, box_canonical, records, iterations, loop, target, n,
-                             lower_threshold, stats, stats_scratch, statistics, words, words_host, result, stream)
+                             lower_threshold, stats, stats_scratch, statistics, words, words_host, result, stream, record_rows)
         return self._after_run(result, executed, iterations, f, max_value, argmax, energies, weights, states, canonical, grid,
                                bands, outcome, statistics, words_host, n_words, g4[1] if sobolev else None)
 
@@ -135,9 +140,10 @@
         return g4
 
     def _run_finish(self, run, p_lists, n_interior, boxes, box_canonical, records, iterations, loop, target, n,
-                    lower_threshold, stats, stats_scratch, statistics, words, words_host, result, stream):
+                    lower_threshold, stats, stats_scratch, statistics, words, words_host, result, stream, record_rows=None):
         none = ctypes.c_void_p(0)
-        _lib.check(_lib.lib.lsf_state_run_finish(
+        rows_taken = ctypes.c_int32(0)
+        _lib.check(_lib.lib.lsf_state_run_finish_rows(
             ctypes.byref(run), ctypes.byref(self.params), ctypes.c_void_p(p_lists),
             ctypes.c_void_p(p_lists + 4 * n_interior), ctypes.c_void_p(boxes.data_ptr() if boxes is not None else 0),
             ctypes.c_void_p(box_canonical.data_ptr() if boxes is not None else 0),
@@ -145,7 +151,11 @@
             dev._ptr(target, n, "live_out"), float(lower_threshold),
             ctypes.c_void_p(stats.data_ptr()) if statistics else none,
             ctypes.c_void_p(stats_scratch.data_ptr()) if statistics else none, ctypes.c_void_p(words.data_ptr()),
-            ctypes.c_void_p(words_host.data_ptr()), ctypes.byref(result), stream), "lsf_state_run_finish")
+            ctypes.c_void_p(words_host.data_ptr()), ctypes.byref(result),
+            ctypes.c_void_p(record_rows.data_ptr()) if record_rows is not None else none,
+            record_rows.numel() if record_rows is not None else 0, ctypes.byref(rows_taken), stream),
+            "lsf_state_run_finish_rows")
+        self.last_call.record_rows = bool(rows_taken.value)
 
     def _after_run(self, result, executed, iterations, f, max_value, argmax, energies, weights, states, canonical, grid, bands,
                    outcome, statistics, words_host, n_words, sobolev_gradient):
```

Measured after the change: 530.9 billion, median of 6. +1.9%, better.
